# jacobkrantz/VLN-CE

Measured on AMD Instinct MI355X. Metric: policy-steps/sec (fwd+bwd), higher is better.
Workload: dtype f32

## Files before the change

### include/vlnce_hip.h

```cpp
#ifndef VLNCE_HIP_H
#define VLNCE_HIP_H

#include <stddef.h>
#include <stdint.h>

#ifdef __cplusplus
extern "C" {
#endif

typedef void* vlnce_stream_t;

enum { VLNCE_ACT_NONE = 0, VLNCE_ACT_RELU = 1, VLNCE_ACT_SIGMOID = 2, VLNCE_ACT_TANH = 3 };

int vlnce_version(void);
int vlnce_option_count(void);
int vlnce_option_index(const char* name);
const char* vlnce_last_error(void);

int vlnce_set_option(const char* name, int value);
int vlnce_get_option(const char* name, int* value);
int vlnce_option_default(const char* name, int* value);

typedef struct {
  int N, H, W, Cin;
  int Cout, KH, KW;
  int stride, pad;
  int Ho, Wo;
  int ldx, ldy;
} vlnce_conv_desc;

typedef struct {
  const float* in_scale;
  const float* in_shift;
  const float* in_center;
  int in_relu;
  const float* x2;
  const float* in2_scale;
  const float* in2_shift;
  const float* in2_center;
  float* side_out;
  const void* w_split;
  const void* w_frag;
  const int* options;
  int w_format;
} vlnce_prologue;

#define VLNCE_BN_SHARDS 16
typedef struct {
  double* acc;
  void* workspace;
  long workspace_bytes;
} vlnce_bn_sums;

typedef struct {
  const float* scale;
  const float* shift;
  const float* residual;
  int ldr;
  int act;
  int accumulate;
  float* stat_partial;
  const vlnce_bn_sums* bn;
} vlnce_epilogue;

long vlnce_conv2d_bn_workspace_bytes(const vlnce_conv_desc* d);
int vlnce_bn_finalize_sums(double* acc, int M, int C, const float* gamma, const float* beta,
                           float eps, float momentum, float* running_mean, float* running_var,
                           float* scale_out, float* shift_out, float* mean_out, float* rstd_out,
                           vlnce_stream_t stream);

int vlnce_conv2d_tiles_m(const vlnce_conv_desc* d);
int vlnce_conv2d_tile_rows(const vlnce_conv_desc* d);

int vlnce_conv2d_split_weights(const float* w, void* planes, long count, int format,
                               vlnce_stream_t stream);

long vlnce_conv2d_pack_bytes(const vlnce_conv_desc* d);
int vlnce_conv2d_pack_weights(const float* w_ohwi, void* frag, const vlnce_conv_desc* d,
                              int format , vlnce_stream_t stream);

typedef struct vlnce_weight_job {
  const float* w_oihw;
  void* dst;
  int Cout, Cin, T;
  int kind;
  int transposed;
  int format;
} vlnce_weight_job;
long vlnce_weight_job_items(const vlnce_weight_job* job);
int vlnce_conv2d_prepare_weights(const vlnce_weight_job* jobs_dev, const long* first_item_dev,
                                 int njobs, long total_items, vlnce_stream_t stream);

#define VLNCE_CONV_PATH_F32 0
#define VLNCE_CONV_PATH_X3 1
#define VLNCE_CONV_PATH_P3 2
#define VLNCE_CONV_PATH_M3 3
int vlnce_conv2d_last_path(void);

#define VLNCE_CONV_KERNEL(family, format, kernel, a, b, c) \
  ((family) | ((format) << 2) | ((kernel) << 4) | ((a) << 8) | ((b) << 16) | ((c) << 24))
#define VLNCE_CONV_KERNEL_FAMILY(v) ((v) & 3)
#define VLNCE_CONV_KERNEL_FORMAT(v) (((v) >> 2) & 3)
#define VLNCE_CONV_KERNEL_KIND(v) (((v) >> 4) & 15)
#define VLNCE_CONV_KERNEL_A(v) (((v) >> 8) & 255)
#define VLNCE_CONV_KERNEL_B(v) (((v) >> 16) & 255)
#define VLNCE_CONV_KERNEL_C(v) (((v) >> 24) & 127)
#define VLNCE_CONV_KERNEL_P3 0
#define VLNCE_CONV_KERNEL_U3 1
#define VLNCE_CONV_KERNEL_S3 2
#define VLNCE_CONV_P3_DENSE 0
#define VLNCE_CONV_P3_GATHER 1
#define VLNCE_CONV_P3_DUAL 2
#define VLNCE_CONV_KERNEL_F32_BUF 0
#define VLNCE_CONV_KERNEL_F32_SPLITK 1
#define VLNCE_CONV_KERNEL_F32_V4 2
#define VLNCE_CONV_KERNEL_F32_S 3
#define VLNCE_CONV_KERNEL_F32_STEM3 4
#define VLNCE_CONV_KERNEL_F32_STEM1 5
#define VLNCE_CONV_KERNEL_F32_DUAL 6
int vlnce_conv2d_last_kernel(void);

int vlnce_conv2d_fwd(const float* x, const float* w_ohwi, float* y,
                     const vlnce_conv_desc* d, const vlnce_prologue* pro,
                     const vlnce_epilogue* epi, vlnce_stream_t stream);

int vlnce_gemm(const float* A, int lda, int transA, const float* B, int ldb, int transB,
               float* C, int ldc, int M, int N, int K,
               const vlnce_epilogue* epi, vlnce_stream_t stream);

int vlnce_linear_rows_supported(int M, int N, int K);
int vlnce_linear_rows_fwd(const float* x, int ldx, const float* w, int ldw, const float* bias,
                          int act, float* y, int ldy, int M, int N, int K, vlnce_stream_t stream);
int vlnce_linear_rows_bwd(const float* x, int ldx, const float* w, int ldw, const float* dy,
                          int lddy, const float* y, int ldy, int act, float* dx, float* dw,
                          float* db, int M, int N, int K, vlnce_stream_t stream);

int vlnce_colsum(const float* x, int ldx, int M, int N, float* out, int accumulate,
                 vlnce_stream_t stream);

size_t vlnce_bn_finalize_workspace_bytes(int tiles_m, int C);
int vlnce_bn_finalize(const float* stat_partial, int tiles_m, int tile_rows, int M, int C,
                      const float* gamma, const float* beta, float eps, float momentum,
                      float* running_mean, float* running_var,
                      float* scale_out, float* shift_out,
                      float* mean_out, float* rstd_out,
                      void* workspace, size_t workspace_bytes,
                      vlnce_stream_t stream);

int vlnce_scale_shift_act(const float* x, const float* scale, const float* shift,
                          const float* center, int rows_per_sample, const float* residual,
                          float* y, long M, int C, int act, vlnce_stream_t stream);

int vlnce_scale_shift_add_act(const float* x1, const float* scale1, const float* shift1,
                              const float* center1, const float* x2, const float* scale2,
                              const float* shift2, const float* center2, float* y, long M, int C,
                              int act, vlnce_stream_t stream);

int vlnce_gn_chunks(int HW);
int vlnce_gn_partial(const float* x, int Nimg, int HW, int C, float* partial ,
                     vlnce_stream_t stream);
int vlnce_gn_finalize(const float* partial, int Nimg, int HW, int C, int groups,
                      const float* gamma, const float* beta, float eps,
                      float* scale_out, float* shift_out,
                      float* center_out,
                      float* mean_out, float* rstd_out,
                      vlnce_stream_t stream);
int vlnce_gn_finalize_tiles(const float* stat_partial, int tile_rows, int Nimg, int HW, int C,
                            int groups, const float* gamma, const float* beta, float eps,
                            float* scale_out, float* shift_out, float* center_out,
                            float* mean_out, float* rstd_out, vlnce_stream_t stream);
int vlnce_group_norm_small(const float* x, int Nimg, int HW, int C, int groups, const float* gamma,
                           const float* beta, float eps, const float* residual, int act, float* y,
                           vlnce_stream_t stream);

int vlnce_maxpool3x3s2(const float* x, float* y, int N, int H, int W, int C, int Ho, int Wo,
                       const float* in_scale, const float* in_shift, const float* in_center,
                       int in_relu, vlnce_stream_t stream);
int vlnce_avgpool2x2(const float* x, float* y, int N, int H, int W, int C, vlnce_stream_t stream);

int vlnce_space_to_depth2(const float* x, float* y, int N, int H, int W, int C, int pad_lo,
                          int pad_hi, const float* scale, const float* shift,
                          vlnce_stream_t stream);
#define VLNCE_DT_F32 0
#define VLNCE_DT_U8 1
typedef struct {
  const void* x;
  const void* x2;
  const unsigned char* mask2;
  int dtype;
  int N, F, Hs, Ws, C;
  int y0, x0, H, W;
} vlnce_frames;
int vlnce_frames_s2d(const vlnce_frames* frames, float* y, int pad_lo, int pad_hi,
                     const float* scale, const float* shift, vlnce_stream_t stream);
int vlnce_stem7_fwd(const vlnce_frames* frames, const float* in_scale, const float* in_shift,
                    const void* w_frag, int w_format, float* y, int Cout, const vlnce_epilogue* epi,
                    vlnce_stream_t stream);
int vlnce_frames_avgpool2(const vlnce_frames* frames, float* y, vlnce_stream_t stream);
int vlnce_frames_f32(const vlnce_frames* frames, float* y, const float* scale, const float* shift,
                     vlnce_stream_t stream);
int vlnce_frames_gather(const void* const* srcs, int F, int elem_bytes, int N, int Hs, int Ws,
                        int C, int y0, int x0, int H, int W, void* out, vlnce_stream_t stream);

int vlnce_frames_resize_area(const void* x, int dtype, int NF, int Hs, int Ws, int C, int OH, int OW,
                             int y0, int x0, int H, int W, void* out, vlnce_stream_t stream);

int vlnce_adaptive_avgpool(const float* x, float* y, int N, int H, int W, int C, int OH, int OW,
                           int ldy, vlnce_stream_t stream);

int vlnce_conv2d_wgrad(const float* x, const float* dy, float* dw_ohwi, const vlnce_conv_desc* d,
                       const float* dy_pow2, int P, int accumulate, vlnce_stream_t stream);
#define VLNCE_WGRAD_PATH_F32 0
#define VLNCE_WGRAD_PATH_X6_BF16 1
#define VLNCE_WGRAD_PATH_X6_F16 2
int vlnce_conv2d_wgrad_last_path(void);
#define VLNCE_WGRAD_KERNEL(path, tm, split) ((path) | ((tm) << 4) | ((split) ? 1 << 12 : 0))
#define VLNCE_WGRAD_KERNEL_PATH(v) ((v) & 15)
#define VLNCE_WGRAD_KERNEL_TM(v) (((v) >> 4) & 255)
#define VLNCE_WGRAD_KERNEL_SPLIT(v) (((v) >> 12) & 1)
int vlnce_conv2d_wgrad_last_kernel(void);
size_t vlnce_bn_bwd_workspace_floats(long M, int C);
int vlnce_bn_bwd(const float* dy, const float* y, const float* x, const float* mean,
                 const float* rstd, const float* gamma, long M, int C, int relu,
                 int use_batch_stats, float* dx, float* dres, float* dgamma, float* dbeta,
                 float* workspace, float* pow2, int P, vlnce_stream_t stream);
size_t vlnce_gn_bwd_workspace_floats(int Nimg, int HW, int C, int groups);
int vlnce_gn_bwd(const float* dy, const float* y, const float* x, const float* mean,
                 const float* rstd, const float* gamma, int Nimg, int HW, int C, int groups,
                 int relu, float* dx, float* dres, float* dgamma, float* dbeta, float* workspace,
                 float* pow2, int P, vlnce_stream_t stream);
int vlnce_maxpool3x3s2_argmax(const float* x, float* y, uint8_t* argmax, int N, int H, int W,
                              int C, int Ho, int Wo, vlnce_stream_t stream);
int vlnce_maxpool3x3s2_bwd(const float* dy, const uint8_t* argmax, float* dx, int N, int H, int W,
                           int C, int Ho, int Wo, vlnce_stream_t stream);
int vlnce_adaptive_avgpool_bwd(const float* dy, float* dx, int N, int H, int W, int C, int OH,
                               int OW, vlnce_stream_t stream);

int vlnce_action_head_fwd(const float* x, int ldx, const float* w, const float* b, int M, int K,
                          int A, float* logits_out, int* nan_count, vlnce_stream_t stream);
int vlnce_action_head_bwd(const float* x, int ldx, const float* w, const float* logits,
                          const float* dlogits, int M, int K, int A, float* dx, float* dw,
                          float* db, vlnce_stream_t stream);

int vlnce_attn_fwd(const float* q, const float* K, int ldk, const float* V, int ldv,
                   const uint8_t* mask, int mask_mode, float scale,
                   float* out, float* attn_out, int B, int P, int Dk, int Dv,
                   vlnce_stream_t stream);
int vlnce_attn_bwd(const float* dout, const float* q, const float* K, int ldk,
                   const float* V, int ldv, const uint8_t* mask, int mask_mode, float scale,
                   const float* attn, float* dq, float* dK, int lddk, float* dV, int lddv,
                   int B, int P, int Dk, int Dv, vlnce_stream_t stream);

int vlnce_attn_fwd_shared(const float* q, const float* K, int ldk, const float* V, int ldv,
                          const uint8_t* mask, int mask_mode, float scale, const int64_t* kv_index,
                          float* out, float* attn_out, int B, int P, int Dk, int Dv,
                          vlnce_stream_t stream);
int vlnce_attn_bwd_shared(const float* dout, const float* q, const float* K, int ldk,
                          const float* V, int ldv, const uint8_t* mask, int mask_mode, float scale,
                          const int64_t* kv_index, const float* attn, float* dq, float* dK,
                          int lddk, float* dV, int lddv, int B, int P, int Dk, int Dv,
                          vlnce_stream_t stream);
int vlnce_segment_sum(const float* x, const int64_t* index, int B, int U, long row_elems,
// ... 129 lines not shown
```

### vln-ce_amd/_lib.py

```python
import collections
import ctypes as C
import os
import threading

import torch

_HERE = os.path.dirname(os.path.abspath(__file__))
LIB_PATH = os.environ.get("VLNCE_HIP_LIB") or os.path.join(_HERE, "libvlnce_hip.so")

_P = C.c_void_p
_I = C.c_int
_F = C.c_float
_L = C.c_long


def _buffer_format(explicit, *bufs):
    tags = {getattr(b, "_vlnce_fmt", None) for b in bufs if b is not None} - {None}
    if explicit:
        tags.add(int(explicit))
    if len(tags) > 1:
        raise RuntimeError(f"weight buffers / w_format disagree on the plane format: {sorted(tags)}")
    return tags.pop() if tags else 1


ConvKernel = collections.namedtuple("ConvKernel", "family kernel fmt a b c")
ConvKernel.__doc__ = """family: "f32" | "x3" | "p3" | "m3" (= conv2d_last_path()); kernel: the kernel within it
("conv_p3" | "conv_u3" | "conv_s3", "conv_m3", "conv_x3", "buf" | "splitk" | "v4" | "s" | "stem3" |
"stem1" | "dual" of igemm_kernel); fmt: plane format 1 / 2 (0: fp32); a, b, c per kernel:
  conv_p3: tile 1..6, mode "dense" | "gather" | "dual", 0      conv_u3: rows, kind 0..2, waves
  conv_s3: Cin, 0, 0      conv_m3: NT, KSPLIT, RB      conv_x3: tile 1..4, dual 0 / 1, 0
  splitk: the split factor, 0, 0"""
WgradKernel = collections.namedtuple("WgradKernel", "path tm split")

_FAMILIES = ("f32", "x3", "p3", "m3")
_KERNELS = {"f32": ("buf", "splitk", "v4", "s", "stem3", "stem1", "dual"), "x3": ("conv_x3",),
            "p3": ("conv_p3", "conv_u3", "conv_s3"), "m3": ("conv_m3",)}
_P3_MODES = ("dense", "gather", "dual")


def decode_conv_kernel(v):
    if v < 0:
        return None
    family = _FAMILIES[v & 3]
    kernel = _KERNELS[family][(v >> 4) & 15]
    a, b, c = (v >> 8) & 255, (v >> 16) & 255, (v >> 24) & 127
    if kernel == "conv_p3":
        b = _P3_MODES[b]
    return ConvKernel(family, kernel, (v >> 2) & 3, a, b, c)


def decode_wgrad_kernel(v):
    return None if v < 0 else WgradKernel(v & 15, (v >> 4) & 255, bool((v >> 12) & 1))


class ConvDesc(C.Structure):
    _fields_ = [(n, _I) for n in
                ("N", "H", "W", "Cin", "Cout", "KH", "KW", "stride", "pad", "Ho", "Wo", "ldx", "ldy")]


class WeightJob(C.Structure):
    _fields_ = [("w_oihw", _P), ("dst", _P), ("Cout", _I), ("Cin", _I), ("T", _I), ("kind", _I),
                ("transposed", _I), ("format", _I)]


class WeightPrepPlan:
    __slots__ = ("table", "first_item", "njobs", "total", "keep")


class Prologue(C.Structure):
    _fields_ = [("in_scale", _P), ("in_shift", _P), ("in_center", _P), ("in_relu", _I),
                ("x2", _P), ("in2_scale", _P), ("in2_shift", _P), ("in2_center", _P),
                ("side_out", _P), ("w_split", _P), ("w_frag", _P), ("options", _P), ("w_format", _I)]


class Frames(C.Structure):
    _fields_ = [("x", _P), ("x2", _P), ("mask2", _P), ("dtype", _I), ("N", _I), ("F", _I),
                ("Hs", _I), ("Ws", _I), ("C", _I), ("y0", _I), ("x0", _I), ("H", _I), ("W", _I)]


class BnSums(C.Structure):
    _fields_ = [("acc", _P), ("workspace", _P), ("workspace_bytes", _L)]


class TrajSensor(C.Structure):
    _fields_ = [("src", _P), ("dst", _P), ("row_stride", _L), ("c_stride", _L), ("p_stride", _L),
                ("C", _I), ("P", _I), ("src_dtype", _I), ("dst_dtype", _I)]


class Epilogue(C.Structure):
    _fields_ = [("scale", _P), ("shift", _P), ("residual", _P), ("ldr", _I), ("act", _I),
                ("accumulate", _I), ("stat_partial", _P), ("bn", C.POINTER(BnSums))]


_SIGNATURES = {
    "vlnce_version": (_I, []),
    "vlnce_last_error": (C.c_char_p, []),
    "vlnce_set_option": (_I, [C.c_char_p, _I]),
    "vlnce_get_option": (_I, [C.c_char_p, C.POINTER(_I)]),
    "vlnce_option_default": (_I, [C.c_char_p, C.POINTER(_I)]),
    "vlnce_conv2d_split_weights": (_I, [_P, _P, C.c_long, _I, _P]),
    "vlnce_conv2d_last_path": (_I, []),
    "vlnce_conv2d_wgrad_last_path": (_I, []),
    "vlnce_conv2d_last_kernel": (_I, []),
    "vlnce_conv2d_wgrad_last_kernel": (_I, []),
    "vlnce_embedding_bwd": (_I, [_P, _P, _P, _L, _I, _L, _L, _P]),
    "vlnce_conv2d_pack_bytes": (C.c_long, [C.POINTER(ConvDesc)]),
    "vlnce_conv2d_pack_weights": (_I, [_P, _P, C.POINTER(ConvDesc), _I, _P]),
    "vlnce_weight_job_items": (C.c_long, [C.POINTER(WeightJob)]),
    "vlnce_conv2d_prepare_weights": (_I, [_P, _P, _I, C.c_long, _P]),
    "vlnce_conv2d_tiles_m": (_I, [C.POINTER(ConvDesc)]),
    "vlnce_conv2d_tile_rows": (_I, [C.POINTER(ConvDesc)]),
    "vlnce_conv2d_bn_workspace_bytes": (C.c_long, [C.POINTER(ConvDesc)]),
    "vlnce_bn_finalize_sums": (_I, [_P, _I, _I, _P, _P, _F, _F, _P, _P, _P, _P, _P, _P, _P]),
    "vlnce_conv2d_fwd": (_I, [_P, _P, _P, C.POINTER(ConvDesc), C.POINTER(Prologue),
                              C.POINTER(Epilogue), _P]),
    "vlnce_gemm": (_I, [_P, _I, _I, _P, _I, _I, _P, _I, _I, _I, _I, C.POINTER(Epilogue), _P]),
    "vlnce_colsum": (_I, [_P, _I, _I, _I, _P, _I, _P]),
    "vlnce_bn_finalize_workspace_bytes": (C.c_size_t, [_I, _I]),
    "vlnce_bn_finalize": (_I, [_P, _I, _I, _I, _I, _P, _P, _F, _F, _P, _P, _P, _P, _P, _P, _P,
                               C.c_size_t, _P]),
    "vlnce_scale_shift_act": (_I, [_P, _P, _P, _P, _I, _P, _P, _L, _I, _I, _P]),
    "vlnce_gn_chunks": (_I, [_I]),
    "vlnce_gn_partial": (_I, [_P, _I, _I, _I, _P, _P]),
    "vlnce_gn_finalize": (_I, [_P, _I, _I, _I, _I, _P, _P, _F, _P, _P, _P, _P, _P, _P]),
    "vlnce_gn_finalize_tiles": (_I, [_P, _I, _I, _I, _I, _I, _P, _P, _F, _P, _P, _P, _P, _P, _P]),
    "vlnce_maxpool3x3s2": (_I, [_P, _P, _I, _I, _I, _I, _I, _I, _P, _P, _P, _I, _P]),
    "vlnce_scale_shift_add_act": (_I, [_P, _P, _P, _P, _P, _P, _P, _P, _P, _L, _I, _I, _P]),
    "vlnce_avgpool2x2": (_I, [_P, _P, _I, _I, _I, _I, _P]),
    "vlnce_ragged_pad_rows": (_I, [_P, _I, _P, _I, _I, _L, _F, _P, _P]),
    "vlnce_ragged_pad_rows_i64": (_I, [_P, _P, _I, _I, _L, _L, _P, _P]),
    "vlnce_dagger_targets": (_I, [_P, _P, _I, _I, _F, _P, _P, _P, _P]),
    "vlnce_traj_append": (_I, [C.POINTER(TrajSensor), _I, C.POINTER(_I), C.POINTER(_I), _I, _L, _P]),
    "vlnce_dagger_mix_actions": (_I, [_P, _P, _I, _P, _F, _I, _P, _P, _P]),
    "vlnce_ppo_loss": (_I, [_P, _P, _P, _P, _P, _P, _P, _P, _P, _P, _I, _F, _F, _F, _F, _F, _F, _F, _I,
                            _P, _P, _P]),
    "vlnce_ppo_returns": (_I, [_P, _P, _P, _P, _P, _I, _I, _F, _F, _I, _P]),
    "vlnce_space_to_depth2": (_I, [_P, _P, _I, _I, _I, _I, _I, _I, _P, _P, _P]),
    "vlnce_frames_s2d": (_I, [C.POINTER(Frames), _P, _I, _I, _P, _P, _P]),
    "vlnce_frames_avgpool2": (_I, [C.POINTER(Frames), _P, _P]),
    "vlnce_stem7_fwd": (_I, [C.POINTER(Frames), _P, _P, _P, _I, _P, _I, C.POINTER(Epilogue), _P]),
    "vlnce_frames_f32": (_I, [C.POINTER(Frames), _P, _P, _P, _P]),
    "vlnce_frames_gather": (_I, [_P, _I, _I, _I, _I, _I, _I, _I, _I, _I, _I, _P, _P]),
    "vlnce_frames_resize_area": (_I, [_P] + [_I] * 11 + [_P, _P]),
    "vlnce_adaptive_avgpool": (_I, [_P, _P, _I, _I, _I, _I, _I, _I, _I, _P]),
    "vlnce_attn_fwd": (_I, [_P, _P, _I, _P, _I, _P, _I, _F, _P, _P, _I, _I, _I, _I, _P]),
    "vlnce_attn_bwd": (_I, [_P, _P, _P, _I, _P, _I, _P, _I, _F, _P, _P, _P, _I, _P, _I,
                            _I, _I, _I, _I, _P]),
    "vlnce_rowzero_mask": (_I, [_P, _I, _L, _I, _P, _P]),
    "vlnce_attn_fwd_shared": (_I, [_P, _P, _I, _P, _I, _P, _I, _F, _P, _P, _P, _I, _I, _I, _I, _P]),
    "vlnce_attn_bwd_shared": (_I, [_P, _P, _P, _I, _P, _I, _P, _I, _F, _P, _P, _P, _P, _I, _P, _I,
                                   _I, _I, _I, _I, _P]),
    "vlnce_segment_sum": (_I, [_P, _P, _I, _I, _L, _P, _P]),
    "vlnce_action_head_fwd": (_I, [_P, _I, _P, _P, _I, _I, _I, _P, _P, _P]),
    "vlnce_action_head_bwd": (_I, [_P, _I, _P, _P, _P, _I, _I, _I, _P, _P, _P, _P]),
    "vlnce_gru_gates_fwd": (_I, [_P, _P, _P, _P, _P, _P, _P, _I, _I, _P]),
    "vlnce_gru_gates_bwd": (_I, [_P, _P, _P, _P, _P, _P, _P, _P, _I, _I, _P]),
    "vlnce_lstm_gates_fwd": (_I, [_P, _P, _P, _P, _P, _P, _P, _I, _I, _P]),
    "vlnce_lstm_gates_bwd": (_I, [_P, _P, _P, _P, _P, _P, _P, _P, _I, _I, _P]),
    "vlnce_mean_rows": (_I, [_P, _P, _I, _I, _I, _P]),
    "vlnce_mask_rows": (_I, [_P, _P, _P, _I, _I, _P]),
    "vlnce_conv2d_wgrad": (_I, [_P, _P, _P, C.POINTER(ConvDesc), _P, _I, _I, _P]),
    "vlnce_bn_bwd": (_I, [_P, _P, _P, _P, _P, _P, _L, _I, _I, _I, _P, _P, _P, _P, _P, _P, _I, _P]),
    "vlnce_bn_bwd_workspace_floats": (C.c_size_t, [_L, _I]),
    "vlnce_gn_bwd_workspace_floats": (C.c_size_t, [_I, _I, _I, _I]),
    "vlnce_gn_bwd": (_I, [_P, _P, _P, _P, _P, _P, _I, _I, _I, _I, _I, _P, _P, _P, _P, _P, _P, _I, _P]),
    "vlnce_maxpool3x3s2_argmax": (_I, [_P, _P, _P, _I, _I, _I, _I, _I, _I, _P]),
    "vlnce_maxpool3x3s2_bwd": (_I, [_P, _P, _P, _I, _I, _I, _I, _I, _I, _P]),
    "vlnce_adaptive_avgpool_bwd": (_I, [_P, _P, _I, _I, _I, _I, _I, _I, _P]),
    "vlnce_rnn_seq_supported": (_I, [_I, _I]),
    "vlnce_rnn_seq_fwd": (_I, [_I, _I, _P, _P, _P, _P, _P, _P, _P, _P, _I, _I, _I, _P]),
    "vlnce_rnn_seq_bwd": (_I, [_I, _I, _P, _P, _P, _P, _P, _P, _P, _P, _P, _I, _I, _I, _P]),
    "vlnce_option_count": (_I, []),
    "vlnce_option_index": (_I, [C.c_char_p]),
    "vlnce_linear_rows_supported": (_I, [_I, _I, _I]),
    "vlnce_linear_rows_fwd": (_I, [_P, _I, _P, _I, _P, _I, _P, _I, _I, _I, _I, _P]),
    "vlnce_linear_rows_bwd": (_I, [_P, _I, _P, _I, _P, _I, _P, _I, _I, _P, _P, _P, _I, _I, _I, _P]),
    "vlnce_rnn_seq_fwd2": (_I, [_I, _I, _P, _P, _P, _P, _P, _P, _L, _L, _P, _P, _P, _I, _I, _I, _P]),
    "vlnce_rnn_seq_bwd2": (_I, [_I, _I, _P, _P, _P, _P, _P, _P, _L, _L, _P, _P, _P, _P, _I, _I, _I, _P]),
    "vlnce_rnn_seq_wgrad": (_I, [_I, _I, _I, _P, _P, _P, _P, _I, _I, _P, _P, _P, _P, _P, _P, _I, _I, _I, _P]),
    "vlnce_group_norm_small": (_I, [_P, _I, _I, _I, _I, _P, _P, _F, _P, _I, _P, _P]),
    "vlnce_gru_rollout_supported": (_I, [_I, _I]),
    "vlnce_gru_rollout_workspace_bytes": (C.c_long, [_I, _I]),
    "vlnce_gru_rollout_fwd": (_I, [_P, _P, _P, _P, _P, _P, _P, _P, _P, _P, _I, _I, _I, _P]),
    "vlnce_gru_rollout_bwd": (_I, [_P, _P, _P, _P, _P, _P, _P, _P, _P, _P, _P, _I, _I, _I, _P]),
    "vlnce_lstm_rollout_supported": (_I, [_I, _I]),
    "vlnce_lstm_rollout_workspace_bytes": (C.c_long, [_I, _I]),
    "vlnce_lstm_rollout_fwd": (_I, [_P, _P, _P, _P, _P, _P, _P, _P, _P, _P, _P, _I, _I, _I, _P]),
    "vlnce_lstm_rollout_bwd": (_I, [_P, _P, _P, _P, _P, _P, _P, _P, _P, _P, _P, _P, _P, _I, _I, _I, _P]),
    "vlnce_rnn_step_supported": (_I, [_I, _I, _I]),
    "vlnce_rnn_step_fwd": (_I, [_I, _P, _P, _P, _P, _P, _P, _P, _P, _P, _P, _I, _I, _P]),
    "vlnce_rnn_step_bwd": (_I, [_I, _P, _P, _P, _P, _P, _P, _P, _P, _P, _P, _P, _P, _P, _I, _I, _P]),
    "vlnce_select_rows": (_I, [_P, _P, _P, _P, _I, _I, _P]),
    "vlnce_act_bwd": (_I, [_P, _P, _P, _L, _I, _P]),
}


def collapse_rows(t):
    while True:
        groups = []
        for n, st in zip(t.shape[1:], t.stride()[1:]):
            if n == 1:
                continue
            if groups and groups[-1][1] == st * n:
                groups[-1] = (groups[-1][0] * n, int(st))
            else:
                groups.append((int(n), int(st)))
        if len(groups) <= 2:
            break
        t = t.contiguous()
    row_stride = int(t.stride(0)) if t.size(0) > 1 else 0
    if not groups:
        return t, row_stride, 1, 0, 1, 0
    if len(groups) == 1:
        return t, row_stride, groups[0][0], groups[0][1], 1, 0
    return t, row_stride, groups[0][0], groups[0][1], groups[1][0], groups[1][1]


def exported_symbols():
    return sorted(_SIGNATURES)


def load_cdll(path=LIB_PATH):
    if not os.path.exists(path):
        raise RuntimeError(
            f"{path} not found: build it with `python __graft_entry__.py` (hipcc, gfx950). "
            "The VLN-CE policy path has no CPU fallback."
        )
    dll = C.CDLL(path)
    for name, (res, args) in _SIGNATURES.items():
        fn = getattr(dll, name)
        fn.restype = res
        fn.argtypes = args
    return dll


class _CallState(threading.local):
    dev = None
    restore = None


_CALL = _CallState()


def _ptr(t):
    if t is None:
        return None
    if not t.is_cuda:
        raise RuntimeError("libvlnce_hip: tensor is not on a GPU (no CPU fallback)")
    idx = t.device.index
    if _CALL.dev is None:
        _CALL.dev = idx
    elif _CALL.dev != idx:
        first, _CALL.dev = _CALL.dev, None
        raise RuntimeError(f"libvlnce_hip: tensors of one call live on cuda:{first} and "
                           f"cuda:{idx}")
    return t.data_ptr()


def _stream():
    dev, _CALL.dev = _CALL.dev, None
    if dev is None:
        return torch.cuda.current_stream().cuda_stream
    cur = torch.cuda.current_device()
    if dev != cur:
        _CALL.restore = cur
        torch.cuda.set_device(dev)
    return torch.cuda.current_stream(dev).cuda_stream


def _leave_device():
    if _CALL.restore is not None:
        cur, _CALL.restore = _CALL.restore, None
        torch.cuda.set_device(cur)


class HipLib:

    name = "hip"

    ABI = 147

    def __init__(self, path=LIB_PATH):
        self.dll = load_cdll(path)
        have = int(self.dll.vlnce_version())
        if have != self.ABI:
            raise RuntimeError(f"{path} has ABI {have}, this package binds ABI {self.ABI}: "
                               "rebuild it (python __graft_entry__.py)")

        self._conv_math = None
        self._tls = threading.local()
        self._options_from_env()

    OPTION_NAMES = ("conv_math", "p3", "p3_tile", "s3", "u3", "u3_waves", "x3_tile", "igemm_tile",
                    "igemm_nobuf", "igemm_no_splitk", "wgrad_tile", "rollout_one_xcd", "m3")

    def _options_from_env(self):
        for name in self.OPTION_NAMES:
            v = os.environ.get("VLNCE_" + name.upper())
            if v is None:
                continue
            if name == "conv_math":
                v = {"f32": 0, "0": 0, "bf16": 1, "1": 1, "f16": 2, "2": 2}.get(v.strip().lower(), v)
            elif name in ("igemm_nobuf", "igemm_no_splitk"):
                v = 0 if v in ("", "0") else 1
            try:
                v = int(v)
            except ValueError:
                import warnings
                warnings.warn(f"VLNCE_{name.upper()}={v!r} is not an integer: ignored "
                              f"(the option keeps its default)")
                continue
            self.set_option(name, v)

    def set_option(self, name, value):
        self._check(self.dll.vlnce_set_option(name.encode(), int(value)), "vlnce_set_option")
        if name == "conv_math":
            self._conv_math = int(value)

    def plane_format(self, options=None):
        v = None
        if options:
            v = options.get("conv_math")
        if v is None:
            sc = getattr(self._tls, "scoped", None)
            if sc:
                v = sc.get("conv_math")
        if v is None or v < 0:
            v = self._conv_math
            if v is None:
                v = self._conv_math = self.get_option("conv_math")
        return 2 if v == 2 else 1

    def get_option(self, name):
        v = _I(0)
        self._check(self.dll.vlnce_get_option(name.encode(), C.byref(v)), "vlnce_get_option")
        return v.value

    def option_default(self, name):
        v = _I(0)
        self._check(self.dll.vlnce_option_default(name.encode(), C.byref(v)), "vlnce_option_default")
        return v.value

    PER_LAUNCH = ("conv_math", "p3", "p3_tile", "s3", "u3", "u3_waves", "x3_tile", "m3")

    def _launch_options(self, overrides):
        if not overrides:
            return None
        arr = (C.c_int * int(self.dll.vlnce_option_count()))(*([-1] * int(self.dll.vlnce_option_count())))
        for name, v in overrides.items():
            i = int(self.dll.vlnce_option_index(name.encode()))
            if i < 0:
                raise RuntimeError(f"unknown dispatch option {name!r}")
            arr[i] = int(v)
        return arr

    def options(self, **kw):
        lib = self
        unknown = [k for k in kw if k not in self.OPTION_NAMES]
        if unknown:
            raise RuntimeError(f"unknown dispatch option(s) {unknown}")

        class _Scope:
            def __enter__(self_inner):
                self_inner.prev = getattr(lib._tls, "scoped", None)
                scoped = dict(self_inner.prev or {})
                scoped.update({k: v for k, v in kw.items() if k in lib.PER_LAUNCH})
                lib._tls.scoped = scoped or None
                self_inner.old = {k: lib.get_option(k) for k in kw if k not in lib.PER_LAUNCH}
                for k in self_inner.old:
                    lib.set_option(k, kw[k])
                return lib

            def __exit__(self_inner, *exc):
                lib._tls.scoped = self_inner.prev
                for k, v in self_inner.old.items():
                    lib.set_option(k, v)
                return False

        return _Scope()

    def _check(self, rc, what):
        _leave_device()
        if rc != 0:
            raise RuntimeError(f"{what} failed (rc={rc}): {self.dll.vlnce_last_error().decode()}")

    @staticmethod
    def _desc(g):
        return ConvDesc(*[int(g[k]) for k, _ in ConvDesc._fields_])

    def conv2d_tiles(self, g):
        d = self._desc(g)
        return self.dll.vlnce_conv2d_tiles_m(C.byref(d)), self.dll.vlnce_conv2d_tile_rows(C.byref(d))

    def conv2d_fwd(self, x, w, y, g, in_scale=None, in_shift=None, in_relu=0, scale=None,
                   shift=None, residual=None, ldr=0, act=0, accumulate=0, stat_partial=None,
                   in_center=None, x2=None, in2_scale=None, in2_shift=None, in2_center=None,
                   side_out=None, w_split=None, w_frag=None, bn=None, options=None, w_format=None):
        d = self._desc(g)
        w_format = _buffer_format(w_format, w_split, w_frag)
        opts = self._launch_options(options if options is not None
                                    else getattr(self._tls, "scoped", None))
        pro = Prologue(_ptr(in_scale), _ptr(in_shift), _ptr(in_center), int(in_relu), _ptr(x2),
                       _ptr(in2_scale), _ptr(in2_shift), _ptr(in2_center), _ptr(side_out),
                       _ptr(w_split), _ptr(w_frag),
                       C.cast(opts, C.c_void_p) if opts is not None else None, int(w_format))
        bnp = None
        if bn is not None:
            acc, ws = bn
            bnp = C.pointer(BnSums(_ptr(acc), _ptr(ws), ws.numel() * ws.element_size()))
        epi = Epilogue(_ptr(scale), _ptr(shift), _ptr(residual), int(ldr), int(act),
                       int(accumulate), _ptr(stat_partial), bnp)
        self._check(self.dll.vlnce_conv2d_fwd(_ptr(x), _ptr(w), _ptr(y), C.byref(d), C.byref(pro),
                                              C.byref(epi), _stream()), "vlnce_conv2d_fwd")

    def bn_finalize_sums(self, acc, M, gamma, beta, eps, momentum, running_mean, running_var,
                         scale_out, mean_out, shift_out=None, rstd_out=None):
        Cc = scale_out.numel()
        self._check(self.dll.vlnce_bn_finalize_sums(
            _ptr(acc), int(M), Cc, _ptr(gamma), _ptr(beta), float(eps), float(momentum),
            _ptr(running_mean), _ptr(running_var), _ptr(scale_out), _ptr(shift_out),
            _ptr(mean_out), _ptr(rstd_out), _stream()), "vlnce_bn_finalize_sums")

    def conv2d_bn_workspace_bytes(self, g):
        d = self._desc(g)
        return int(self.dll.vlnce_conv2d_bn_workspace_bytes(C.byref(d)))

    def conv2d_split_weights(self, w, planes, fmt=1):
        self._check(self.dll.vlnce_conv2d_split_weights(_ptr(w), _ptr(planes), w.numel(), int(fmt),
                                                        _stream()), "vlnce_conv2d_split_weights")

    def conv2d_last_path(self):
        return int(self.dll.vlnce_conv2d_last_path())

    def conv2d_wgrad_last_path(self):
        return int(self.dll.vlnce_conv2d_wgrad_last_path())

    def conv2d_last_kernel(self):
        return decode_conv_kernel(int(self.dll.vlnce_conv2d_last_kernel()))

    def conv2d_wgrad_last_kernel(self):
        return decode_wgrad_kernel(int(self.dll.vlnce_conv2d_wgrad_last_kernel()))

    def conv2d_pack_bytes(self, g):
        d = self._desc(g)
        return int(self.dll.vlnce_conv2d_pack_bytes(C.byref(d)))

    def conv2d_pack_weights(self, w, frag, g, fmt=1):
        d = self._desc(g)
        self._check(self.dll.vlnce_conv2d_pack_weights(_ptr(w), _ptr(frag), C.byref(d), int(fmt),
                                                       _stream()), "vlnce_conv2d_pack_weights")

    WP_F32, WP_PLANES, WP_FRAGMENTS = 0, 1, 2

    def weight_prep_plan(self, jobs):
        arr = (WeightJob * len(jobs))()
        first = [0]
        for j, (w, dst, kind, transposed, fmt) in zip(arr, jobs):
            assert w.is_cuda and w.is_contiguous() and w.dtype == torch.float32 and w.dim() == 4
            j.w_oihw, j.dst = w.data_ptr(), dst.data_ptr()
            j.Cout, j.Cin, j.T = w.size(0), w.size(1), w.size(2) * w.size(3)
            j.kind, j.transposed, j.format = int(kind), int(bool(transposed)), int(fmt or 0)
            items = int(self.dll.vlnce_weight_job_items(C.byref(j)))
            if items <= 0:
                raise ValueError(f"weight_prep_plan: job not eligible: {tuple(w.shape)} kind={kind} "
                                 f"transposed={transposed} format={fmt}")
            first.append(first[-1] + items)
        plan = WeightPrepPlan()
        dev = jobs[0][1].device
        plan.table = torch.frombuffer(bytearray(bytes(arr)), dtype=torch.uint8).to(dev)
        plan.first_item = torch.tensor(first, dtype=torch.int64).to(dev)
        plan.njobs, plan.total = len(jobs), first[-1]
        plan.keep = [(w, dst) for w, dst, *_ in jobs]
        return plan

    def conv2d_prepare_weights(self, plan):
        self._check(self.dll.vlnce_conv2d_prepare_weights(_ptr(plan.table), _ptr(plan.first_item),
                                                          plan.njobs, plan.total, _stream()),
                    "vlnce_conv2d_prepare_weights")

    def gemm(self, A, lda, transA, B, ldb, transB, Cm, ldc, M, N, K, scale=None, shift=None,
             residual=None, ldr=0, act=0, accumulate=0):
        epi = Epilogue(_ptr(scale), _ptr(shift), _ptr(residual), int(ldr), int(act),
                       int(accumulate), None)
        self._check(self.dll.vlnce_gemm(_ptr(A), lda, transA, _ptr(B), ldb, transB, _ptr(Cm), ldc,
                                        M, N, K, C.byref(epi), _stream()), "vlnce_gemm")

    def colsum(self, x, ldx, M, N, out, accumulate=0):
        self._check(self.dll.vlnce_colsum(_ptr(x), ldx, M, N, _ptr(out), accumulate, _stream()),
                    "vlnce_colsum")

    def bn_finalize_workspace_bytes(self, tiles_m, Cc):
        return int(self.dll.vlnce_bn_finalize_workspace_bytes(tiles_m, Cc))

    def bn_finalize(self, partial, tiles_m, tile_rows, M, Cc, gamma, beta, eps, momentum,
                    running_mean, running_var, scale_out, shift_out, mean_out=None, rstd_out=None,
                    workspace=None):
        wb = workspace.numel() * workspace.element_size() if workspace is not None else 0
        self._check(self.dll.vlnce_bn_finalize(
            _ptr(partial), tiles_m, tile_rows, M, Cc, _ptr(gamma), _ptr(beta), eps, momentum,
            _ptr(running_mean), _ptr(running_var), _ptr(scale_out), _ptr(shift_out),
            _ptr(mean_out), _ptr(rstd_out), _ptr(workspace), wb, _stream()), "vlnce_bn_finalize")

    def scale_shift_act(self, x, scale, shift, rows_per_sample, residual, y, M, Cc, act,
                        center=None):
        self._check(self.dll.vlnce_scale_shift_act(
            _ptr(x), _ptr(scale), _ptr(shift), _ptr(center), rows_per_sample, _ptr(residual),
            _ptr(y), M, Cc, act, _stream()), "vlnce_scale_shift_act")

    def gn_chunks(self, HW):
        return self.dll.vlnce_gn_chunks(HW)

    def gn_partial(self, x, Nimg, HW, Cc, partial):
        self._check(self.dll.vlnce_gn_partial(_ptr(x), Nimg, HW, Cc, _ptr(partial), _stream()),
                    "vlnce_gn_partial")

    def gn_finalize(self, partial, Nimg, HW, Cc, groups, gamma, beta, eps, scale_out, shift_out,
                    mean_out=None, rstd_out=None, center_out=None):
        self._check(self.dll.vlnce_gn_finalize(
            _ptr(partial), Nimg, HW, Cc, groups, _ptr(gamma), _ptr(beta), eps, _ptr(scale_out),
            _ptr(shift_out), _ptr(center_out), _ptr(mean_out), _ptr(rstd_out), _stream()),
            "vlnce_gn_finalize")

    def gn_finalize_tiles(self, partial, tile_rows, Nimg, HW, Cc, groups, gamma, beta, eps,
                          scale_out, shift_out, mean_out=None, rstd_out=None, center_out=None):
        self._check(self.dll.vlnce_gn_finalize_tiles(
            _ptr(partial), tile_rows, Nimg, HW, Cc, groups, _ptr(gamma), _ptr(beta), eps,
            _ptr(scale_out), _ptr(shift_out), _ptr(center_out), _ptr(mean_out), _ptr(rstd_out),
            _stream()), "vlnce_gn_finalize_tiles")

    def maxpool3x3s2(self, x, y, N, H, W, Cc, Ho, Wo, in_scale=None, in_shift=None, in_relu=0,
                     in_center=None):
        self._check(self.dll.vlnce_maxpool3x3s2(_ptr(x), _ptr(y), N, H, W, Cc, Ho, Wo,
                                                _ptr(in_scale), _ptr(in_shift), _ptr(in_center),
                                                int(in_relu), _stream()), "vlnce_maxpool3x3s2")

    def scale_shift_add_act(self, x1, s1, t1, x2, s2, t2, y, M, Cc, act, c1=None, c2=None):
        self._check(self.dll.vlnce_scale_shift_add_act(
            _ptr(x1), _ptr(s1), _ptr(t1), _ptr(c1), _ptr(x2), _ptr(s2), _ptr(t2), _ptr(c2),
            _ptr(y), M, Cc, act, _stream()), "vlnce_scale_shift_add_act")

    _SRC = {torch.float32: 0, torch.float16: 1, torch.int64: 2}

    def ragged_pad_rows(self, src, offsets, B, Tmax, D, fill, dst):
        assert offsets.dtype == torch.int32 and dst.dtype == torch.float32
        self._check(self.dll.vlnce_ragged_pad_rows(
            _ptr(src), self._SRC[src.dtype], _ptr(offsets), B, Tmax, D, float(fill),
            _ptr(dst), _stream()), "vlnce_ragged_pad_rows")

    def ragged_pad_rows_i64(self, src, offsets, B, Tmax, D, fill, dst):
        assert src.dtype == torch.int64 and dst.dtype == torch.int64
        self._check(self.dll.vlnce_ragged_pad_rows_i64(
            _ptr(src), _ptr(offsets), B, Tmax, D, int(fill), _ptr(dst), _stream()),
            "vlnce_ragged_pad_rows_i64")

    def dagger_targets(self, oracle, offsets, B, Tmax, coef, corrected, weights, masks):
        self._check(self.dll.vlnce_dagger_targets(
            _ptr(oracle), _ptr(offsets), B, Tmax, float(coef), _ptr(corrected),
            _ptr(weights), _ptr(masks), _stream()), "vlnce_dagger_targets")

    _TRAJ = {torch.float32: 0, torch.float16: 1, torch.int64: 2, torch.uint8: 3}
    TRAJ_MAX_SENSORS, TRAJ_MAX_ROWS = 8, 128

    def traj_append(self, sources, arenas, slots, steps):
        n = len(slots)
# ... 386 lines not shown
```

### vln-ce_amd/csrc/api.cpp

```cpp
#include <stdarg.h>
#include <stdio.h>
#include <string.h>

#include <atomic>

#include "common_opts.h"

static thread_local char g_err[512] = "";

void vlnce_set_error(const char* fmt, ...) {
  va_list ap;
  va_start(ap, fmt);
  vsnprintf(g_err, sizeof(g_err), fmt, ap);
  va_end(ap);
}

extern "C" const char* vlnce_last_error(void) { return g_err; }
extern "C" int vlnce_version(void) { return 147; }

namespace {
struct OptDef {
  const char* name;
  int def;
};
const OptDef kOpts[VLNCE_OPT_COUNT] = {
    {"conv_math", 2},   {"p3", 2},          {"p3_tile", 0},         {"s3", 1},
    {"u3", 1},          {"u3_waves", 8},    {"x3_tile", 0},         {"igemm_tile", 0},
    {"igemm_nobuf", 0}, {"igemm_no_splitk", 0}, {"wgrad_tile", 64}, {"rollout_one_xcd", 0},
    {"m3", 1},
};
std::atomic<int> g_opt[VLNCE_OPT_COUNT] = {
    {2}, {2}, {0}, {1}, {1}, {8}, {0}, {0}, {0}, {0}, {64}, {0}, {1},
};
int opt_index(const char* name) {
  if (name)
    for (int i = 0; i < VLNCE_OPT_COUNT; ++i)
      if (strcmp(name, kOpts[i].name) == 0) return i;
  return -1;
}
}

namespace {
thread_local const int* t_call_opts = nullptr;
}
VlnceOptScope::VlnceOptScope(const int* per_call) : prev(t_call_opts) { t_call_opts = per_call; }
VlnceOptScope::~VlnceOptScope() { t_call_opts = prev; }

int vlnce_opt(int id) {
  if (t_call_opts && t_call_opts[id] >= 0) return t_call_opts[id];
  return g_opt[id].load(std::memory_order_relaxed);
}

extern "C" int vlnce_option_count(void) { return VLNCE_OPT_COUNT; }

extern "C" int vlnce_option_index(const char* name) { return opt_index(name); }

extern "C" int vlnce_set_option(const char* name, int value) {
  const int i = opt_index(name);
  if (i < 0) {
    vlnce_set_error("vlnce_set_option: unknown option '%s'", name ? name : "(null)");
    return 1;
  }
  g_opt[i].store(value, std::memory_order_relaxed);
  return 0;
}

extern "C" int vlnce_get_option(const char* name, int* value) {
  const int i = opt_index(name);
  if (i < 0 || !value) {
    vlnce_set_error("vlnce_get_option: unknown option '%s'", name ? name : "(null)");
    return 1;
  }
  *value = g_opt[i].load(std::memory_order_relaxed);
  return 0;
}

extern "C" int vlnce_option_default(const char* name, int* value) {
  const int i = opt_index(name);
  if (i < 0 || !value) {
    vlnce_set_error("vlnce_option_default: unknown option '%s'", name ? name : "(null)");
    return 1;
  }
  *value = kOpts[i].def;
  return 0;
}
```

### vln-ce_amd/csrc/common_opts.h

```cpp
#pragma once
#include "../../include/vlnce_hip.h"

void vlnce_set_error(const char* fmt, ...);

enum {
  VLNCE_OPT_CONV_MATH,
  VLNCE_OPT_P3,
  VLNCE_OPT_P3_TILE,
  VLNCE_OPT_S3,
  VLNCE_OPT_U3,
  VLNCE_OPT_U3_WAVES,
  VLNCE_OPT_X3_TILE,
  VLNCE_OPT_IGEMM_TILE,
  VLNCE_OPT_IGEMM_NOBUF,
  VLNCE_OPT_IGEMM_NO_SPLITK,
  VLNCE_OPT_WGRAD_TILE,
  VLNCE_OPT_ROLLOUT_ONE_XCD,
  VLNCE_OPT_M3,
  VLNCE_OPT_COUNT
};
int vlnce_opt(int id);

struct VlnceOptScope {
  explicit VlnceOptScope(const int* per_call);
  ~VlnceOptScope();
  const int* prev;
};
```

### vln-ce_amd/csrc/conv_s3.hip

```cpp
#include "igemm_shared.h"

using namespace vlnce_detail;

namespace vlnce_detail {
namespace {

template <int NCC, int MATH>
__global__ __launch_bounds__(512) void conv_s3_kernel(IgemmParams p) {
#if defined(__HIP_DEVICE_COMPILE__)
  typedef Planes<MATH> PL;
  constexpr int P3_ROW = PL::ROW, NA = PL::NA, NP = PL::NP;
  constexpr int BM = 64, MT = 2, KS = NCC * 2;
  constexpr int CBUF = BM * P3_ROW;
  constexpr int PBUF = NCC * CBUF;
  constexpr int SPS = 32 / KS;
  extern __shared__ __attribute__((aligned(16))) char xsm[];

  const int tid = threadIdx.x;
  const int lane = tid & 63;
  const int wave = __builtin_amdgcn_readfirstlane(tid >> 6);
  const int half = lane >> 5;
  const int l31 = lane & 31;
  const int trow = tid >> 3;
  const int lk4 = (tid & 7) * 4;

  const int n0 = ((int)blockIdx.x % p.tiles_n) * 256;
  const int wg = (int)blockIdx.x / p.tiles_n, nwg = (int)gridDim.x / p.tiles_n;
  const int my_tiles = (p.tiles_m - wg + nwg - 1) / nwg;

  const __amdgpu_buffer_rsrc_t rsrc_a = __builtin_amdgcn_make_buffer_rsrc(
      const_cast<char*>(reinterpret_cast<const char*>(p.A)), 0, (int)p.a_bytes, 0x00020000);
  const __amdgpu_buffer_rsrc_t rsrc_b = __builtin_amdgcn_make_buffer_rsrc(
      const_cast<char*>(reinterpret_cast<const char*>(p.Bfrag)), 0, (int)((long)p.N * p.K * 6),
      0x00020000);
  const __amdgpu_buffer_rsrc_t rsrc_c = __builtin_amdgcn_make_buffer_rsrc(
      reinterpret_cast<char*>(p.C), 0, (int)p.c_bytes, 0x00020000);
  const float relu_floor = p.in_relu ? 0.f : -__builtin_huge_valf();
  const bool relu_out = p.act == VLNCE_ACT_RELU;

  bf16x8 bres[KS][3];
  {
    const int vb = (n0 / 32 + wave) * KS * 3072 + lane * 16;
#pragma unroll
    for (int ks = 0; ks < KS; ++ks)
#pragma unroll
      for (int q = 0; q < 3; ++q)
        bres[ks][q] = __builtin_bit_cast(
            bf16x8, __builtin_amdgcn_raw_buffer_load_b128(rsrc_b, vb + q * 1024, ks * 3072, 0));
  }
  float* const vlds = reinterpret_cast<float*>(xsm + 2 * PBUF);
  if (tid < 8) {
    const f32x4 zero4 = {0.f, 0.f, 0.f, 0.f}, one4 = {1.f, 1.f, 1.f, 1.f};
#pragma unroll
    for (int c = 0; c < NCC; ++c) {
      f32x4 s_ = one4, t_ = zero4, c_ = zero4;
      if (p.in_scale != nullptr) {
        s_ = ldg4(p.in_scale + c * 32 + lk4);
        t_ = ldg4(p.in_shift + c * 32 + lk4);
        if (p.in_center) c_ = ldg4(p.in_center + c * 32 + lk4);
      }
      *reinterpret_cast<f32x4*>(vlds + c * 32 + lk4) = s_;
      *reinterpret_cast<f32x4*>(vlds + NCC * 32 + c * 32 + lk4) = t_;
      *reinterpret_cast<f32x4*>(vlds + 2 * NCC * 32 + c * 32 + lk4) = c_;
    }
  }
  __syncthreads();
  const int col = n0 + wave * 32 + l31;
  const float e_sc = (p.scale ? p.scale[col] : 1.f) * PL::POST;
  const float e_sh = p.shift ? p.shift[col] : 0.f;

  constexpr int RING = NCC > 2 ? 1 : 2;
  f32x4 raw[RING][NCC];
  auto load_raw = [&](f32x4 (&r)[NCC], int round) {
    const int m = (wg + round * nwg) * BM + trow;
    const int vo = (round < my_tiles && m < p.M) ? (m * p.lda + lk4) * 4 : BUF_OOB;
#pragma unroll
    for (int c = 0; c < NCC; ++c)
      r[c] = __builtin_bit_cast(f32x4, __builtin_amdgcn_raw_buffer_load_b128(rsrc_a, vo, c * 128, 0));
  };
#pragma unroll
  for (int k = 0; k < RING; ++k) load_raw(raw[k], k);
  f32x16 acc[2][MT];
#pragma unroll
  for (int b = 0; b < 2; ++b)
#pragma unroll
    for (int i = 0; i < MT; ++i)
#pragma unroll
      for (int r = 0; r < 16; ++r) acc[b][i][r] = 0.f;
  const int a_off = l31 * P3_ROW + half * 16;

  WaveBn<1> wbn;
  wave_bn_reset(wbn);
  auto stats = [&](const f32x16 (&a)[MT], int m0) {
    if (p.bn.acc != nullptr) {
      wave_bn_tile<MT, 1>(reinterpret_cast<const f32x16(&)[MT][1]>(a), wbn, p.bn.acc, n0 + wave * 32,
                          p.N, p.M - m0, half, l31, PL::POST);
    } else if (p.stat_partial != nullptr) {
#pragma unroll
      for (int i = 0; i < MT; ++i)
        wave_stats_block<1>(reinterpret_cast<const f32x16(&)[1]>(a[i]), p.stat_partial,
                            m0 / 32 + i, p.M - (m0 + i * 32), n0 + wave * 32, p.N, half, l31, PL::POST);
    }
  };
  auto stores = [&](f32x16 (&a)[MT], int m0, int first, int count) {
    const int rows_left = p.M - (m0 + 4 * half);
    const int e_voff = (int)((((long)(m0 + 4 * half)) * p.ldc + col) * 4);
#pragma unroll
    for (int k = first; k < first + count; ++k) {
      const int i = k >> 4, r2 = k & 15;
      const int rw = i * 32 + (r2 & 3) + 8 * (r2 >> 2);
      const float lin = a[i][r2] * e_sc + e_sh;
      const float v = relu_out ? (lin > 0.f ? lin : 0.f) : lin;
      __builtin_amdgcn_raw_buffer_store_b32(__builtin_bit_cast(unsigned, v), rsrc_c,
                                            rw < rows_left ? e_voff : BUF_OOB, rw * p.ldc * 4, 0);
      a[i][r2] = 0.f;
    }
  };

  auto tile = [&](int round, f32x4 (&r)[NCC], f32x16 (&cur)[MT], f32x16 (&prv)[MT]) {
    const int m0 = (wg + round * nwg) * BM;
    const int m0_prev = (wg + (round - 1) * nwg) * BM;
    const bool has_prev = round > 0;
    char* const pb = xsm + (round & 1) * PBUF;
    const bool row_ok = m0 + trow < p.M;
#pragma unroll
    for (int c = 0; c < NCC; ++c) {
      f32x4 v = r[c];
      const f32x4 s_ = *reinterpret_cast<const f32x4*>(vlds + c * 32 + lk4);
      const f32x4 t_ = *reinterpret_cast<const f32x4*>(vlds + NCC * 32 + c * 32 + lk4);
      const f32x4 c_ = *reinterpret_cast<const f32x4*>(vlds + 2 * NCC * 32 + c * 32 + lk4);
#pragma unroll
      for (int e = 0; e < 4; ++e) {
        v[e] = fmaxf(fmaf(v[e] - c_[e], s_[e], t_[e]), relu_floor);
        v[e] = row_ok ? v[e] : 0.f;
      }
      p3_split_store<MATH>(v, pb + c * CBUF + trow * P3_ROW + lk4 * 2);
    }
    load_raw(r, round + RING);
    asm volatile("s_waitcnt lgkmcnt(0)" ::: "memory");
    __builtin_amdgcn_s_barrier();
    if (has_prev) stats(prv, m0_prev);
#pragma unroll
    for (int c = 0; c < NCC; ++c)
#pragma unroll
      for (int s2 = 0; s2 < 2; ++s2) {
        bf16x8 f[MT][NA];
#pragma unroll
        for (int i = 0; i < MT; ++i)
#pragma unroll
          for (int q = 0; q < NA; ++q)
            f[i][q] = *reinterpret_cast<const bf16x8*>(pb + c * CBUF + a_off + i * 32 * P3_ROW +
                                                       q * 64 + s2 * 32);
#pragma unroll
        for (int q = 0; q < NP; ++q)
#pragma unroll
          for (int i = 0; i < MT; ++i)
            cur[i] = plane_mfma<MATH>(f[i][PL::PA[q]], bres[c * 2 + s2][PL::PB[q]], cur[i]);
        stores(prv, has_prev ? m0_prev : p.M, (c * 2 + s2) * SPS, SPS);
        if constexpr (MATH == MATH_F16X3) {
#pragma unroll
          for (int g = 0; g < 2; ++g) {
            if constexpr (SPS == 8) {
              __builtin_amdgcn_sched_group_barrier(0x008, 1, 0);
              __builtin_amdgcn_sched_group_barrier(0x040, 1, 0);
              __builtin_amdgcn_sched_group_barrier(0x008, 1, 0);
              __builtin_amdgcn_sched_group_barrier(0x040, 2, 0);
              __builtin_amdgcn_sched_group_barrier(0x008, 1, 0);
              __builtin_amdgcn_sched_group_barrier(0x040, 1, 0);
            } else {
              __builtin_amdgcn_sched_group_barrier(0x008, 3, 0);
              __builtin_amdgcn_sched_group_barrier(0x040, 2, 0);
            }
          }
        } else {
#pragma unroll
          for (int g = 0; g < 4; ++g) {
            if constexpr (SPS == 8) {
              __builtin_amdgcn_sched_group_barrier(0x008, 2, 0);
              __builtin_amdgcn_sched_group_barrier(0x040, 1, 0);
              __builtin_amdgcn_sched_group_barrier(0x008, 1, 0);
              __builtin_amdgcn_sched_group_barrier(0x040, 1, 0);
            } else {
              __builtin_amdgcn_sched_group_barrier(0x008, 3, 0);
              __builtin_amdgcn_sched_group_barrier(0x040, 1, 0);
            }
          }
        }
      }
  };
  if (my_tiles <= 0) return;
  tile(0, raw[0], acc[0], acc[1]);
  if (1 < my_tiles) tile(1, raw[RING - 1], acc[1], acc[0]);
  for (int round = 2; round < my_tiles; round += 2) {
    tile(round, raw[0], acc[0], acc[1]);
    if (round + 1 < my_tiles) tile(round + 1, raw[RING - 1], acc[1], acc[0]);
  }
  {
    const int m0 = (wg + (my_tiles - 1) * nwg) * BM;
    if ((my_tiles - 1) & 1) {
      stats(acc[1], m0);
      if (p.bn.acc != nullptr) wave_bn_flush(wbn, p.bn.acc, p.N, half, l31);
      stores(acc[1], m0, 0, 32);
    } else {
      stats(acc[0], m0);
      if (p.bn.acc != nullptr) wave_bn_flush(wbn, p.bn.acc, p.N, half, l31);
      stores(acc[0], m0, 0, 32);
    }
  }
#endif
}

template <int NCC, int MATH>
int launch_s3(const IgemmParams& p, hipStream_t stream) {
  constexpr int smem_bytes = 2 * NCC * 64 * Planes<MATH>::ROW + 3 * NCC * 32 * 4;
  auto kern = conv_s3_kernel<NCC, MATH>;
  static bool attr_set = false;
  if (!attr_set) {
    hipError_t e = hipFuncSetAttribute(reinterpret_cast<const void*>(kern),
                                       hipFuncAttributeMaxDynamicSharedMemorySize, smem_bytes);
    if (e != hipSuccess) {
      vlnce_set_error("conv_s3: hipFuncSetAttribute failed: %s", hipGetErrorString(e));
      return 2;
    }
    attr_set = true;
  }
  IgemmParams q = p;
  q.tiles_m = ceil_div(p.M, 64);
  q.tiles_n = p.N / 256;
  q.splitk = 1;
  const int cus = x3_cus();
  long grid = (long)q.tiles_m * q.tiles_n;
  if (grid > cus) grid = cus - cus % q.tiles_n;
  hipLaunchKernelGGL(kern, dim3((unsigned)grid), dim3(512), smem_bytes, stream, q);
  VLNCE_CHECK_LAUNCH("conv_s3");
  return 0;
}

}

int s3_launch(const IgemmParams& p, hipStream_t stream) {
  note_conv_kernel(VLNCE_CONV_KERNEL(VLNCE_CONV_PATH_P3, p.math, VLNCE_CONV_KERNEL_S3, p.Cin == 64 ? 64 : 128, 0, 0));
  if (p.math == MATH_F16X3)
    return p.Cin == 64 ? launch_s3<2, MATH_F16X3>(p, stream) : launch_s3<4, MATH_F16X3>(p, stream);
  return p.Cin == 64 ? launch_s3<2, MATH_BF16X6>(p, stream) : launch_s3<4, MATH_BF16X6>(p, stream);
}

}
```

### vln-ce_amd/csrc/igemm.hip

```cpp
#include "igemm_shared.h"

using namespace vlnce_detail;

namespace {


template <int BM, int BN, int WM, int WN, int AMODE, int BMODE, int CIN_C = 0, int KW_C = 0,
          int DUAL = 0>
__global__ __launch_bounds__(256, 2) void igemm_kernel(IgemmParams p) {
  static_assert(!DUAL || AMODE == A_BUF, "dual-input prologue: buffer-loader path only");
  constexpr int WTM = BM / WM;
  constexpr int WTN = BN / WN;
  constexpr int MT = WTM / 32;
  constexpr int NT = WTN / 32;
  constexpr bool A_KMAJOR = AMODE == A_TRANS;
  constexpr bool B_KMAJOR = BMODE == B_KN || BMODE == B_IM2COL;
  constexpr int LDT_A = BM + 8, LDT_B = BN + 8;
  constexpr int A_TILE = BM * LDP;
  constexpr int B_TILE = BN * LDP;
  static_assert(BK * LDT_A <= A_TILE && BK * LDT_B <= B_TILE, "k-major LDS image");
  constexpr int STAGE = A_TILE + B_TILE;
  static_assert(WM * WN == 4, "4 waves");
  static_assert(MT >= 1 && NT >= 1, "tile");

// ... 944 lines not shown
      const long long c = clock64() - d_c0, w = wall_clock64() - d_w0;
      printf("x3 tiles %d KT %d: first K-tile after %lld cycles; total %lld cycles = %lld ticks of 100 MHz "
             "(%.2f GHz); waiting for producers %lld\n", my_tiles, KT, d_c1 - d_c0, c, w,
             (double)c / (double)w * 0.1, d_wait);
    }
#endif
  }
#endif
}

__global__ __launch_bounds__(256) void rows_stats_kernel(const float* __restrict__ y, int ldc, int M,
                                                         int N, int rows,
                                                         float* __restrict__ partial) {
  const int col = blockIdx.y * 64 + (threadIdx.x & 63);
  const int blk = blockIdx.x * 4 + (threadIdx.x >> 6);
  const int r0 = blk * rows;
  if (col >= N || r0 >= M) return;
  const int n = min(rows, M - r0);
  const float* q = y + (long)r0 * ldc + col;
  float v[32];
  float s = 0.f;
#pragma unroll
  for (int i = 0; i < 32; ++i) {
    v[i] = i < n ? q[(long)i * ldc] : 0.f;
    s += v[i];
  }
  const float mean = s / (float)n;
  float m2 = 0.f;
#pragma unroll
  for (int i = 0; i < 32; ++i) {
    const float d = v[i] - mean;
    if (i < n) m2 += d * d;
  }
  float* dst = partial + ((long)blk * N + col) * 2;
  dst[0] = s;
  dst[1] = m2;
}

__global__ __launch_bounds__(256) void bias_act_kernel(float* __restrict__ c, int ldc, int M, int N,
                                                       const float* __restrict__ shift, int act) {
  const long total = (long)M * N;
  for (long i = (long)blockIdx.x * blockDim.x + threadIdx.x; i < total;
       i += (long)gridDim.x * blockDim.x) {
    const long row = i / N;
    const int col = (int)(i - row * N);
    float* q = c + row * ldc + col;
    *q = apply_act(*q + (shift ? shift[col] : 0.f), act);
  }
}

template <int BM, int BN, int WM, int WN, int AMODE, int BMODE, int CIN_C = 0, int KW_C = 0,
          int DUAL = 0>
int launch(const IgemmParams& p, hipStream_t stream) {
  constexpr int smem_bytes = 2 * (BM + BN) * LDP * (int)sizeof(float);
  static_assert(BM * (BN + 4) * (int)sizeof(float) <= smem_bytes, "epilogue tile must fit");
  auto kern = igemm_kernel<BM, BN, WM, WN, AMODE, BMODE, CIN_C, KW_C, DUAL>;
  static bool attr_set = false;
  if (!attr_set) {
    hipError_t e = hipFuncSetAttribute(reinterpret_cast<const void*>(kern),
                                       hipFuncAttributeMaxDynamicSharedMemorySize, smem_bytes);
    if (e != hipSuccess) {
      vlnce_set_error("igemm: hipFuncSetAttribute failed: %s", hipGetErrorString(e));
      return 2;
    }
    attr_set = true;
  }
  IgemmParams q = p;
  q.tiles_m = ceil_div(p.M, BM);
  q.tiles_n = ceil_div(p.N, BN);
  if (q.splitk < 1) q.splitk = 1;
  const long nwg = (long)q.tiles_m * q.tiles_n;
  if (nwg <= 0 || nwg > 0x7fffffffL) {
    vlnce_set_error("igemm: bad grid %ld", nwg);
    return 1;
  }
  hipLaunchKernelGGL(kern, dim3((unsigned)nwg, (unsigned)q.splitk), dim3(256), smem_bytes, stream,
                     q);
  VLNCE_CHECK_LAUNCH("igemm");
  return 0;
}

struct TileChoice {
  int bm, bn;
};
TileChoice choose_tile(long M, int N) {
  const int force = vlnce_opt(VLNCE_OPT_IGEMM_TILE);
  if (force == 1) return {128, 128};
  if (force == 2) return {128, 64};
  if (force == 3) return {64, 64};
  const long want = 512;
  auto tiles = [&](int bm, int bn) { return (long)ceil_div(M, bm) * ceil_div(N, bn); };
  if (N > 64 && M > 64 && tiles(128, 128) >= want) return {128, 128};
  if (N > 64 && M > 64 && tiles(128, 64) >= want) return {128, 64};
  return {64, 64};
}

template <int AMODE, int BMODE>
int dispatch_tiles(const IgemmParams& p, hipStream_t s) {
  const TileChoice t = choose_tile(p.M, p.N);
  if (t.bm == 128 && t.bn == 128) return launch<128, 128, 2, 2, AMODE, BMODE>(p, s);
  if (t.bm == 128 && t.bn == 64) return launch<128, 64, 2, 2, AMODE, BMODE>(p, s);
  return launch<64, 64, 2, 2, AMODE, BMODE>(p, s);
}
int dispatch_dual(const IgemmParams& p, hipStream_t s) {
  const TileChoice t = choose_tile(p.M, p.N);
  if (t.bm == 128 && t.bn == 128) return launch<128, 128, 2, 2, A_BUF, B_BUF, 0, 0, 1>(p, s);
  if (t.bm == 128 && t.bn == 64) return launch<128, 64, 2, 2, A_BUF, B_BUF, 0, 0, 1>(p, s);
  return launch<64, 64, 2, 2, A_BUF, B_BUF, 0, 0, 1>(p, s);
}
template <int AMODE, int BMODE>
int dispatch_small(const IgemmParams& p, hipStream_t s) {
  return launch<64, 64, 2, 2, AMODE, BMODE>(p, s);
}
bool buf_ok(const IgemmParams& p) {
  const bool off = vlnce_opt(VLNCE_OPT_IGEMM_NOBUF) != 0;
  const long bias = ((long)p.pad * p.W + p.pad) * p.lda * 4;
  return !off && (p.Cin % 32 == 0) && (p.K % 32 == 0) && (p.lda % 4 == 0) && (p.ldb % 4 == 0) &&
         p.KH * p.KW <= 32 && p.a_bytes + bias < 0x7fffffffL && p.b_bytes < 0x7fffffffL;
}
template <int CIN_C>
int dispatch_stem(const IgemmParams& p, hipStream_t s) {
  const TileChoice t = choose_tile(p.M, p.N);
  if (t.bm == 128) return launch<128, 64, 2, 2, A_IM2COL_S, B_NK_S, CIN_C, 7>(p, s);
  return launch<64, 64, 2, 2, A_IM2COL_S, B_NK_S, CIN_C, 7>(p, s);
}

int choose_splitk(const IgemmParams& p, bool long_reduction_form = false) {
  const bool off = vlnce_opt(VLNCE_OPT_IGEMM_NO_SPLITK) != 0;
  if (off) return 1;
  const long tiles = (long)ceil_div(p.M, 64) * ceil_div(p.N, 64);
  const int KT = ceil_div(p.K, BK);
  if (long_reduction_form && KT >= 32 && tiles >= 128 && tiles < 1024) {
    long s = (1024 + tiles - 1) / tiles;
    if (s > KT / 4) s = KT / 4;
    return s < 2 ? 1 : (int)s;
  }
  if (tiles >= 128 || KT < 8) return 1;
  long s = (256 + tiles - 1) / tiles;
  if (s > KT / 2) s = KT / 2;
  if (s > 64) s = 64;
  return s < 2 ? 1 : (int)s;
}

void fill_epilogue(IgemmParams& p, const vlnce_epilogue* e) {
  p.scale = e ? e->scale : nullptr;
  p.shift = e ? e->shift : nullptr;
  p.residual = e ? e->residual : nullptr;
  p.ldr = e ? e->ldr : 0;
  p.act = e ? e->act : 0;
  p.accumulate = e ? e->accumulate : 0;
  p.stat_partial = e ? e->stat_partial : nullptr;
  p.bn = vlnce_bn_sums{};
  if (e && e->bn) p.bn = *e->bn;
}

bool aligned16(const void* q) { return (reinterpret_cast<uintptr_t>(q) & 15) == 0; }

template <int BM, int BN, int WM, int WN, int DUAL, int MATH>
int launch_x3(const IgemmParams& p, hipStream_t stream) {
  constexpr int smem_bytes = 2 * (Planes<MATH>::NA * BM + 3 * BN) * X3_PITCH + 16;
  constexpr int threads = (WM * WN + X3_PRODUCERS) * 64;
  auto kern = conv_x3_kernel<BM, BN, WM, WN, DUAL, MATH>;
  static bool attr_set = false;
  if (!attr_set) {
    hipError_t e = hipFuncSetAttribute(reinterpret_cast<const void*>(kern),
                                       hipFuncAttributeMaxDynamicSharedMemorySize, smem_bytes);
    if (e != hipSuccess) {
      vlnce_set_error("conv_x3: hipFuncSetAttribute failed: %s", hipGetErrorString(e));
      return 2;
    }
    attr_set = true;
  }
  IgemmParams q = p;
  q.tiles_m = ceil_div(p.M, BM);
  q.tiles_n = ceil_div(p.N, BN);
  q.splitk = 1;
  const long nwg = (long)q.tiles_m * q.tiles_n;
  if (nwg <= 0 || nwg > 0x7fffffffL) {
    vlnce_set_error("conv_x3: bad grid %ld", nwg);
    return 1;
  }
  const int cus = x3_cus();
  const unsigned grid = nwg <= cus ? (unsigned)nwg : (unsigned)cus;
  hipLaunchKernelGGL(kern, dim3(grid), dim3(threads), smem_bytes, stream, q);
  VLNCE_CHECK_LAUNCH("conv_x3");
  return 0;
}

struct X3Plan {
  int bm, bn;
};
bool x3_plan(const IgemmParams& p, X3Plan* out) {
  if (!conv_math() || !p.Bsplit || !buf_ok(p) || p.splitk > 1) return false;
  if (p.accumulate || p.c_bytes >= 0x7fffffffL) return false;
  if (p.residual && (p.ldr != p.ldc || p.stat_partial || p.bn.acc)) return false;
  const int force = vlnce_opt(VLNCE_OPT_X3_TILE);
  const X3Plan cand[4] = {{128, 128}, {64, 128}, {128, 64}, {64, 64}};
  if (force >= 1 && force <= 4) {
    *out = cand[force - 1];
    return true;
  }
  const int cus = x3_cus();
  double best = 0.0;
  for (const X3Plan& c : cand) {
    if (c.bn == 128 && p.N <= 64) continue;
    const long tiles = (long)ceil_div(p.M, c.bm) * ceil_div(p.N, c.bn);
    const long rounds = (tiles + cus - 1) / cus;
    const double eff = (double)tiles / (double)(rounds * cus);
    if (eff >= 0.8) {
      *out = c;
      return true;
    }
    if (eff > best) {
      best = eff;
      *out = c;
    }
  }
  return best >= 0.4;
}
template <int DUAL, int MATH>
int dispatch_x3_(const IgemmParams& p, const X3Plan& t, hipStream_t s) {
  const int tile = t.bm == 128 ? (t.bn == 128 ? 1 : 3) : (t.bn == 128 ? 2 : 4);
  note_conv_kernel(VLNCE_CONV_KERNEL(VLNCE_CONV_PATH_X3, MATH, 0, tile, DUAL, 0));
  if (t.bm == 128 && t.bn == 128) return launch_x3<128, 128, 2, 4, DUAL, MATH>(p, s);
  if (t.bm == 64 && t.bn == 128) return launch_x3<64, 128, 2, 4, DUAL, MATH>(p, s);
  if (t.bm == 128 && t.bn == 64) return launch_x3<128, 64, 4, 2, DUAL, MATH>(p, s);
  return launch_x3<64, 64, 2, 2, DUAL, MATH>(p, s);
}
template <int DUAL>
int dispatch_x3(const IgemmParams& p, const X3Plan& t, hipStream_t s) {
  return p.math == MATH_F16X3 ? dispatch_x3_<DUAL, MATH_F16X3>(p, t, s)
                              : dispatch_x3_<DUAL, MATH_BF16X6>(p, t, s);
}

}

static int stat_rows_for(const vlnce_conv_desc* d) {
  const int hw = d->Ho * d->Wo;
  return hw % 32 == 0 ? 32 : 16;
}

extern "C" int vlnce_conv2d_tile_rows(const vlnce_conv_desc* d) { return stat_rows_for(d); }

extern "C" int vlnce_conv2d_tiles_m(const vlnce_conv_desc* d) {
  const long M = (long)d->N * d->Ho * d->Wo;
  return ceil_div(M, stat_rows_for(d));
}

template <int MATH>
__global__ __launch_bounds__(256) void split_weights_kernel(const float* __restrict__ w,
                                                            unsigned short* __restrict__ planes,
                                                            long count) {
  for (long i = blockIdx.x * 256L + threadIdx.x; i < count; i += gridDim.x * 256L) {
    unsigned short o[3];
    split_weight<MATH>(w[i], o);
#pragma unroll
    for (int q = 0; q < 3; ++q) planes[q * count + i] = o[q];
  }
}

extern "C" int vlnce_conv2d_split_weights(const float* w, void* planes, long count, int format,
                                          vlnce_stream_t stream) {
  VLNCE_CHECK_ARG(w && planes && count > 0, "conv2d_split_weights: bad argument");
  VLNCE_CHECK_ARG(format == MATH_BF16X6 || format == MATH_F16X3,
                  "conv2d_split_weights: format must be 1 (three bf16 planes) or 2 (fp16 planes)");
  const long blocks = (count + 255) / 256;
  hipLaunchKernelGGL(format == MATH_F16X3 ? split_weights_kernel<MATH_F16X3>
                                          : split_weights_kernel<MATH_BF16X6>,
                     dim3((unsigned)(blocks > 4096 ? 4096 : blocks)),
                     dim3(256), 0, reinterpret_cast<hipStream_t>(stream), w,
                     reinterpret_cast<unsigned short*>(planes), count);
  VLNCE_CHECK_LAUNCH("conv2d_split_weights");
  return 0;
}

__global__ __launch_bounds__(256) void bn_sums_finalize_kernel(
    double* __restrict__ acc, int M, int N, const float* __restrict__ gamma,
    const float* __restrict__ beta, float eps, float momentum, float* running_mean,
    float* running_var, float* scale_out, float* shift_out, float* mean_out, float* rstd_out) {
  const int c = blockIdx.x * 256 + threadIdx.x;
  if (c >= N) return;
  double S = 0.0, Q = 0.0;
#pragma unroll
  for (int k = 0; k < VLNCE_BN_SHARDS; ++k) {
    double* q = acc + ((long)k * N + c) * 2;
    S += q[0];
    Q += q[1];
    q[0] = 0.0;
    q[1] = 0.0;
  }
  const double mean = S / (double)M;
  double m2 = Q - S * mean;
  if (m2 < 0.0) m2 = 0.0;
  const double var = m2 / (double)M;
  const float rstd = (float)(1.0 / sqrt(var + (double)eps));
  const float g = gamma ? gamma[c] : 1.f;
  const float sc = g * rstd;
  scale_out[c] = sc;
  if (shift_out) shift_out[c] = (beta ? beta[c] : 0.f) - (float)mean * sc;
  if (mean_out) mean_out[c] = (float)mean;
  if (rstd_out) rstd_out[c] = rstd;
  if (running_mean) {
    const double unbiased = M > 1 ? m2 / (double)(M - 1) : var;
    running_mean[c] = (1.f - momentum) * running_mean[c] + momentum * (float)mean;
    running_var[c] = (1.f - momentum) * running_var[c] + momentum * (float)unbiased;
  }
}

__global__ __launch_bounds__(256) void bn_partials_to_sums_kernel(const float* __restrict__ partial,
                                                                  int tiles_m, int tile_rows, int M,
                                                                  int N, double* __restrict__ acc) {
  const int c = blockIdx.y * 64 + (threadIdx.x & 63);
  const int t0 = (blockIdx.x * 4 + (threadIdx.x >> 6)) * 32;
  if (c >= N || t0 >= tiles_m) return;
  double S = 0.0, Q = 0.0;
  for (int t = t0; t < min(t0 + 32, tiles_m); ++t) {
    const float2 v = *reinterpret_cast<const float2*>(partial + ((long)t * N + c) * 2);
    const int nt = min(tile_rows, M - t * tile_rows);
    S += (double)v.x;
    Q += (double)v.y + (double)v.x * (double)v.x / (double)nt;
  }
  double* q = acc + ((long)(blockIdx.x % VLNCE_BN_SHARDS) * N + c) * 2;
  unsafeAtomicAdd(q, S);
  unsafeAtomicAdd(q + 1, Q);
}

extern "C" long vlnce_conv2d_bn_workspace_bytes(const vlnce_conv_desc* d) {
  if (!d || d->Cout <= 0) return 0;
  return (((long)vlnce_conv2d_tiles_m(d) * d->Cout * 2 * 4) + 255) / 256 * 256;
}

extern "C" int vlnce_bn_finalize_sums(double* acc, int M, int C, const float* gamma, const float* beta,
                                      float eps, float momentum, float* running_mean,
                                      float* running_var, float* scale_out, float* shift_out,
                                      float* mean_out, float* rstd_out, vlnce_stream_t stream) {
  VLNCE_CHECK_ARG(acc && scale_out && M > 0 && C > 0, "bn_finalize_sums: bad argument");
  VLNCE_CHECK_ARG((running_mean == nullptr) == (running_var == nullptr),
                  "bn_finalize_sums: running stats must come together");
  hipLaunchKernelGGL(bn_sums_finalize_kernel, dim3(ceil_div(C, 256)), dim3(256), 0,
                     reinterpret_cast<hipStream_t>(stream), acc, M, C, gamma, beta, eps, momentum,
                     running_mean, running_var, scale_out, shift_out, mean_out, rstd_out);
  VLNCE_CHECK_LAUNCH("bn_finalize_sums");
  return 0;
}

static thread_local int g_last_path = -1;
extern "C" int vlnce_conv2d_last_path(void) { return g_last_path; }
static thread_local int g_last_kernel = -1;
extern "C" int vlnce_conv2d_last_kernel(void) { return g_last_kernel; }
void vlnce_detail::note_conv_kernel(int value) { g_last_kernel = value; }
static void note_f32_kernel(int kernel, int a = 0) {
  g_last_kernel = VLNCE_CONV_KERNEL(VLNCE_CONV_PATH_F32, 0, kernel, a, 0, 0);
}

extern "C" int vlnce_conv2d_fwd(const float* x, const float* w, float* y, const vlnce_conv_desc* d,
                                const vlnce_prologue* pro, const vlnce_epilogue* epi,
                                vlnce_stream_t stream) {
  VLNCE_CHECK_ARG(x && w && y && d, "conv2d_fwd: null argument");
  VLNCE_CHECK_ARG(d->N > 0 && d->H > 0 && d->W > 0 && d->Cin > 0 && d->Cout > 0,
                  "conv2d_fwd: bad shape");
  const VlnceOptScope opt_scope(pro ? pro->options : nullptr);
  VLNCE_CHECK_ARG(d->H < 32768 && d->W < 32768, "conv2d_fwd: H/W must be < 32768");
  const int ho = (d->H + 2 * d->pad - d->KH) / d->stride + 1;
  const int wo = (d->W + 2 * d->pad - d->KW) / d->stride + 1;
  VLNCE_CHECK_ARG(ho == d->Ho && wo == d->Wo, "conv2d_fwd: Ho/Wo mismatch (%d,%d) vs (%d,%d)", ho,
                  wo, d->Ho, d->Wo);
  const long M = (long)d->N * d->Ho * d->Wo;
  VLNCE_CHECK_ARG(M < 0x7fffffffL && (long)d->N * d->H * d->W < 0x7fffffffL,
                  "conv2d_fwd: too many pixels for 32-bit row indices");
  IgemmParams p{};
  p.A = x;
  p.B = w;
  p.C = y;
  p.M = (int)M;
  p.N = d->Cout;
  p.K = d->KH * d->KW * d->Cin;
  p.H = d->H;
  p.W = d->W;
  p.Cin = d->Cin;
  p.KH = d->KH;
  p.KW = d->KW;
  p.stride = d->stride;
  p.pad = d->pad;
  p.Ho = d->Ho;
  p.Wo = d->Wo;
  p.lda = d->ldx ? d->ldx : d->Cin;
  p.ldb = p.K;
  p.ldc = d->ldy ? d->ldy : d->Cout;
  p.in_scale = pro ? pro->in_scale : nullptr;
  p.in_shift = pro ? pro->in_shift : nullptr;
  p.in_center = pro ? pro->in_center : nullptr;
  p.in_relu = pro ? pro->in_relu : 0;
  p.A2 = pro ? pro->x2 : nullptr;
  p.in2_scale = pro ? pro->in2_scale : nullptr;
  p.in2_shift = pro ? pro->in2_shift : nullptr;
  p.in2_center = pro ? pro->in2_center : nullptr;
  p.side_out = pro ? pro->side_out : nullptr;
  p.Bsplit = pro ? pro->w_split : nullptr;
  p.Bfrag = pro ? pro->w_frag : nullptr;
  p.math = (pro && pro->w_format) ? pro->w_format : MATH_BF16X6;
  VLNCE_CHECK_ARG(p.math == MATH_BF16X6 || p.math == MATH_F16X3,
                  "conv2d_fwd: w_format must be 0 / 1 (three bf16 planes) or 2 (fp16 planes)");
  VLNCE_CHECK_ARG((p.in_scale == nullptr) == (p.in_shift == nullptr),
                  "conv2d_fwd: in_scale and in_shift must come together");
  fill_epilogue(p, epi);
  const vlnce_bn_sums* const bnf = epi ? epi->bn : nullptr;
  if (bnf != nullptr) {
    VLNCE_CHECK_ARG(bnf->acc != nullptr, "conv2d_fwd: bn needs acc");
    VLNCE_CHECK_ARG(!p.stat_partial && !p.scale && !p.shift && !p.residual && !p.act && !p.accumulate,
                    "conv2d_fwd: bn excludes stat_partial / scale / shift / residual / act / accumulate");
    VLNCE_CHECK_ARG(bnf->workspace && bnf->workspace_bytes >= vlnce_conv2d_bn_workspace_bytes(d) &&
                        aligned16(bnf->workspace),
                    "conv2d_fwd: bn workspace too small (vlnce_conv2d_bn_workspace_bytes)");
  }
  auto bn_to_partials = [&]() {
    if (bnf != nullptr) {
      p.bn = vlnce_bn_sums{};
      p.stat_partial = static_cast<float*>(bnf->workspace);
    }
  };
  auto bn_sums_behind = [&](int rc) -> int { return rc; };
  auto bn_finalize_behind = [&](int rc) -> int {
    if (rc != 0 || bnf == nullptr) return rc;
    const int tiles = vlnce_conv2d_tiles_m(d);
    hipLaunchKernelGGL(bn_partials_to_sums_kernel, dim3(ceil_div(tiles, 128), ceil_div(d->Cout, 64)),
                       dim3(256), 0, reinterpret_cast<hipStream_t>(stream),
                       static_cast<const float*>(bnf->workspace), tiles, stat_rows_for(d), (int)M,
                       d->Cout, bnf->acc);
    VLNCE_CHECK_LAUNCH("conv2d_fwd bn moments -> sums");
    return 0;
  };
  const bool v4 = (d->Cin % 4 == 0) && (p.lda % 4 == 0) && aligned16(x) && aligned16(w) &&
                  (!p.in_scale || (aligned16(p.in_scale) && aligned16(p.in_shift))) &&
                  (!p.in_center || aligned16(p.in_center));
  p.splitk = 1;
  p.a_bytes = (((long)d->N * d->H * d->W - 1) * p.lda + d->Cin) * 4;
  p.b_bytes = (long)d->Cout * p.K * 4;
  p.c_bytes = ((M - 1) * p.ldc + d->Cout) * 4;
  p.stat_rows = stat_rows_for(d);
  hipStream_t s = reinterpret_cast<hipStream_t>(stream);
  g_last_path = VLNCE_CONV_PATH_F32;
  if (p.A2 != nullptr || p.side_out != nullptr) {
    VLNCE_CHECK_ARG(p.A2 && p.in_scale && d->KH == 1 && d->KW == 1 && d->stride == 1 &&
                        d->pad == 0 && v4 && buf_ok(p) && aligned16(p.A2) &&
                        (!p.side_out || aligned16(p.side_out)) &&
                        ((p.in2_scale == nullptr) == (p.in2_shift == nullptr)) &&
                        (!p.in2_scale || (aligned16(p.in2_scale) && aligned16(p.in2_shift))) &&
                        (!p.in2_center || (p.in2_scale && aligned16(p.in2_center))),
                    "conv2d_fwd: the dual-input prologue needs x2 + in_scale on a 1x1/stride-1/"
                    "pad-0 convolution with Cin %% 32 == 0 and 16-byte aligned operands");
    g_last_path = VLNCE_CONV_PATH_P3;
    if (const int rc = p3_try_launch(p, s); rc >= 0) return bn_sums_behind(rc);
    g_last_path = VLNCE_CONV_PATH_X3;
    if (X3Plan t; x3_plan(p, &t)) return bn_sums_behind(dispatch_x3<1>(p, t, s));
    g_last_path = VLNCE_CONV_PATH_F32;
    note_f32_kernel(VLNCE_CONV_KERNEL_F32_DUAL);
    bn_to_partials();
    return bn_finalize_behind(dispatch_dual(p, s));
  }
  if (v4 && buf_ok(p)) {
    g_last_path = VLNCE_CONV_PATH_M3;
    if (const int rc = m3_try_launch(p, s); rc >= 0) return bn_sums_behind(rc);
    g_last_path = VLNCE_CONV_PATH_F32;
    const int sk = (!p.accumulate && p.ldc == p.N && p.stat_rows <= 32 &&
                    ((p.scale && p.shift) || (!p.scale && !p.residual)))
                       ? choose_splitk(p)
                       : 1;
    if (sk > 1) {
      bn_to_partials();
      const float* scale = p.scale;
      const float* shift = p.shift;
      const float* residual = p.residual;
      float* stat_partial = p.stat_partial;
      const int act = p.act, ldr = p.ldr;
      p.scale = p.shift = p.residual = nullptr;
      p.stat_partial = nullptr;
      p.act = 0;
      p.splitk = sk;
      note_f32_kernel(VLNCE_CONV_KERNEL_F32_SPLITK, sk);
      vlnce_zero(y, M, p.N, p.ldc, s);
      if (int rc = dispatch_small<A_BUF, B_BUF>(p, s)) return rc;
      if (stat_partial) {
        const int nblk = ceil_div((int)M, p.stat_rows);
        hipLaunchKernelGGL(rows_stats_kernel, dim3(ceil_div(nblk, 4), ceil_div(p.N, 64)), dim3(256),
                           0, s, y, p.ldc, (int)M, p.N, p.stat_rows, stat_partial);
        VLNCE_CHECK_LAUNCH("conv2d_fwd split-K statistics");
      }
      if (bnf != nullptr) return bn_finalize_behind(0);
      if (scale) {
        VLNCE_CHECK_ARG(!residual || ldr == p.N, "conv2d_fwd: split-K needs a contiguous residual");
        return vlnce_scale_shift_act(y, scale, shift, nullptr, 0, residual, y, M, p.N, act, stream);
      }
      if (shift || act) {
        const long work = M * p.N;
        const int grid = (int)((work + 255) / 256 > 2048 ? 2048 : (work + 255) / 256);
        hipLaunchKernelGGL(bias_act_kernel, dim3(grid), dim3(256), 0, s, y, p.ldc, (int)M, p.N, shift, act);
        VLNCE_CHECK_LAUNCH("conv2d_fwd bias/act");
      }
      return 0;
    }
    g_last_path = VLNCE_CONV_PATH_P3;
    if (const int rc = p3_try_launch(p, s); rc >= 0) return bn_sums_behind(rc);
    g_last_path = VLNCE_CONV_PATH_X3;
    if (X3Plan t; x3_plan(p, &t)) return bn_sums_behind(dispatch_x3<0>(p, t, s));
    g_last_path = VLNCE_CONV_PATH_F32;
    note_f32_kernel(VLNCE_CONV_KERNEL_F32_BUF);
    bn_to_partials();
    return bn_finalize_behind(dispatch_tiles<A_BUF, B_BUF>(p, s));
  }
  bn_to_partials();
  note_f32_kernel(v4 ? VLNCE_CONV_KERNEL_F32_V4
                  : d->KW == 7 && d->Cin == 3 ? VLNCE_CONV_KERNEL_F32_STEM3
                  : d->KW == 7 && d->Cin == 1 ? VLNCE_CONV_KERNEL_F32_STEM1
                                              : VLNCE_CONV_KERNEL_F32_S);
  if (v4) return bn_finalize_behind(dispatch_tiles<A_IM2COL_V4, B_NK_V4>(p, s));
  if (d->KW == 7 && d->Cin == 3) return bn_finalize_behind(dispatch_stem<3>(p, s));
  if (d->KW == 7 && d->Cin == 1) return bn_finalize_behind(dispatch_stem<1>(p, s));
  return bn_finalize_behind(dispatch_tiles<A_IM2COL_S, B_NK_S>(p, s));
}

extern "C" int vlnce_gemm(const float* A, int lda, int transA, const float* B, int ldb, int transB,
                          float* C, int ldc, int M, int N, int K, const vlnce_epilogue* epi,
                          vlnce_stream_t stream) {
  VLNCE_CHECK_ARG(A && B && C, "gemm: null argument");
  VLNCE_CHECK_ARG(M > 0 && N > 0 && K > 0, "gemm: bad shape %d %d %d", M, N, K);
  VLNCE_CHECK_ARG(!(epi && epi->stat_partial), "gemm: stat_partial is a conv-only option");
  IgemmParams p{};
  p.A = A;
  p.B = B;
  p.C = C;
  p.M = M;
  p.N = N;
  p.K = K;
  VLNCE_CHECK_ARG((long)M < 32767L * 1024L, "gemm: M too large");
  p.W = M < 1024 ? M : 1024;
  p.H = ceil_div(M, p.W);
  p.Cin = K;
  p.KH = p.KW = 1;
  p.stride = 1;
  p.pad = 0;
  p.Ho = p.H;
  p.Wo = p.W;
  p.lda = lda;
  p.ldb = ldb;
  p.ldc = ldc;
  fill_epilogue(p, epi);
  hipStream_t s = reinterpret_cast<hipStream_t>(stream);
  p.splitk = 1;
  const bool plain = !p.scale && !p.residual && !(p.accumulate && p.act);
  if (plain) p.splitk = choose_splitk(p, transA != 0);
  const float* bias2 = nullptr;
  int act2 = 0;
  if (p.splitk > 1) {
    bias2 = p.shift;
    act2 = p.act;
    p.shift = nullptr;
    p.act = 0;
    if (!p.accumulate) vlnce_zero(C, M, N, ldc, s);
    p.accumulate = 0;
  }
  int rc;
  if (!transA) {
    const bool av4 = (K % 4 == 0) && (lda % 4 == 0) && aligned16(A);
    if (!transB) {
      const bool bv4 = (K % 4 == 0) && (ldb % 4 == 0) && aligned16(B);
      p.a_bytes = (((long)M - 1) * lda + K) * 4;
      p.b_bytes = (((long)N - 1) * ldb + K) * 4;
      if (av4 && bv4 && buf_ok(p))
        rc = p.splitk > 1 ? dispatch_small<A_BUF, B_BUF>(p, s) : dispatch_tiles<A_BUF, B_BUF>(p, s);
      else if (av4 && bv4)
        rc = p.splitk > 1 ? dispatch_small<A_IM2COL_V4, B_NK_V4>(p, s)
                          : dispatch_tiles<A_IM2COL_V4, B_NK_V4>(p, s);
      else
        rc = dispatch_small<A_IM2COL_S, B_NK_S>(p, s);
    } else {
      VLNCE_CHECK_ARG(aligned16(B), "gemm: B must be 16-byte aligned");
      if (av4)
        rc = p.splitk > 1 ? dispatch_small<A_IM2COL_V4, B_KN>(p, s)
                          : dispatch_tiles<A_IM2COL_V4, B_KN>(p, s);
      else
        rc = dispatch_small<A_IM2COL_S, B_KN>(p, s);
    }
  } else {
    VLNCE_CHECK_ARG(transB, "gemm: transA requires transB (only A^T * B^T-stored form is built)");
    VLNCE_CHECK_ARG(aligned16(A) && aligned16(B), "gemm: operands must be 16-byte aligned");
    rc = p.splitk > 1 ? dispatch_small<A_TRANS, B_KN>(p, s) : dispatch_tiles<A_TRANS, B_KN>(p, s);
  }
  if (rc != 0) return rc;
  if (p.splitk > 1 && (bias2 || act2)) {
    const long work = (long)M * N;
    const int grid = (int)((work + 255) / 256 > 2048 ? 2048 : (work + 255) / 256);
    hipLaunchKernelGGL(bias_act_kernel, dim3(grid), dim3(256), 0, s, C, ldc, M, N, bias2, act2);
    VLNCE_CHECK_LAUNCH("gemm bias/act");
  }
// ... 70 lines not shown
```

### vln-ce_amd/csrc/igemm_shared.h

```cpp
#pragma once
#include "common.h"
#include <stdlib.h>
#include <type_traits>

namespace vlnce_detail {

constexpr int BK = 32;
constexpr int LDP = 36;

enum { A_IM2COL_V4 = 0, A_IM2COL_S = 1, A_TRANS = 2, A_BUF = 3 };
enum { B_NK_V4 = 0, B_NK_S = 1, B_KN = 2, B_BUF = 3, B_IM2COL = 4 };

typedef unsigned int u32x4 __attribute__((ext_vector_type(4)));
typedef unsigned u32x2 __attribute__((ext_vector_type(2)));
constexpr int BUF_OOB = (int)0x80000000;

#ifdef VLNCE_DBG_TIME
#define DBG_T(...) __VA_ARGS__
#else
#define DBG_T(...)
#endif

struct IgemmParams {
  const float* A;
  const float* B;
  float* C;
  int M, N, K;
  int H, W, Cin, KH, KW, stride, pad, Ho, Wo;
  int lda, ldb, ldc;
  const float* in_scale;
  const float* in_shift;
  const float* in_center;
  int in_relu;
  const float* A2;
  const float* in2_scale;
  const float* in2_shift;
  const float* in2_center;
  float* side_out;
  const void* Bsplit;
  const void* Bfrag;
  int math;
  int p3_rows;
  const float* scale;
  const float* shift;
  const float* residual;
  int ldr;
  int act;
  int accumulate;
  float* stat_partial;
  vlnce_bn_sums bn;
  int tiles_m, tiles_n;
  int splitk;
  int stat_rows;
  long a_bytes, b_bytes, c_bytes;
};

__device__ __forceinline__ f32x4 ldg4(const float* p) { return *reinterpret_cast<const f32x4*>(p); }

template <int MT, int NT>
__device__ __forceinline__ void wave_stats(const f32x16 (&acc)[MT][NT], float* stat_partial,
                                           int part_row, int rows_left, int rows_full, int col0,
                                           int N, int half, int l31, float post = 1.f) {
  const int rows_valid = min(rows_full, rows_left);
#pragma unroll
  for (int j = 0; j < NT; ++j) {
    float s = 0.f;
#pragma unroll
    for (int i = 0; i < MT; ++i)
#pragma unroll
      for (int r = 0; r < 16; ++r) {
        const int row = i * 32 + (r & 3) + 8 * (r >> 2) + 4 * half;
        if (row < rows_valid) s += acc[i][j][r];
      }
    s += __shfl_xor(s, 32, 64);
    const float mean = rows_valid > 0 ? s / (float)rows_valid : 0.f;
    float m2 = 0.f;
#pragma unroll
    for (int i = 0; i < MT; ++i)
#pragma unroll
      for (int r = 0; r < 16; ++r) {
        const int row = i * 32 + (r & 3) + 8 * (r >> 2) + 4 * half;
        const float d = acc[i][j][r] - mean;
        if (row < rows_valid) m2 += d * d;
      }
    m2 += __shfl_xor(m2, 32, 64);
    const int col = col0 + j * 32 + l31;
    if (half == 0 && col < N && rows_left > 0) {
      float* dst = stat_partial + ((long)part_row * N + col) * 2;
      dst[0] = s * post;
      dst[1] = m2 * post * post;
    }
  }
}

template <int MT, int NT>
__device__ __forceinline__ void wave_stats_fine(const f32x16 (&acc)[MT][NT], float* stat_partial,
                                                int rows, int row0, int M, int col0, int N,
                                                int half, int l31, float post = 1.f) {
  const int nblk = MT * 32 / rows;
  for (int b = 0; b < nblk; ++b) {
    const int r_first = b * rows;
    const int left = M - (row0 + r_first);
    const int valid = min(rows, left);
#pragma unroll
    for (int j = 0; j < NT; ++j) {
      float s = 0.f;
#pragma unroll
      for (int i = 0; i < MT; ++i)
#pragma unroll
        for (int r = 0; r < 16; ++r) {
          const int row = i * 32 + (r & 3) + 8 * (r >> 2) + 4 * half;
          if (row >= r_first && row < r_first + valid) s += acc[i][j][r];
        }
      s += __shfl_xor(s, 32, 64);
      const float mean = valid > 0 ? s / (float)valid : 0.f;
      float m2 = 0.f;
#pragma unroll
      for (int i = 0; i < MT; ++i)
#pragma unroll
        for (int r = 0; r < 16; ++r) {
          const int row = i * 32 + (r & 3) + 8 * (r >> 2) + 4 * half;
          const float d = acc[i][j][r] - mean;
          if (row >= r_first && row < r_first + valid) m2 += d * d;
        }
      m2 += __shfl_xor(m2, 32, 64);
      const int col = col0 + j * 32 + l31;
      if (half == 0 && col < N && left > 0) {
        float* dst = stat_partial + ((long)((row0 + r_first) / rows) * N + col) * 2;
        dst[0] = s * post;
        dst[1] = m2 * post * post;
      }
    }
  }
}

template <int NT>
__device__ __forceinline__ void wave_stats_block(const f32x16 (&acc)[NT], float* stat_partial,
                                                 int part_row, int rows_left, int col0, int N,
                                                 int half, int l31, float post = 1.f) {
  const int rows_valid = min(32, rows_left);
#pragma unroll
  for (int j = 0; j < NT; ++j) {
    float s = 0.f;
#pragma unroll
    for (int r = 0; r < 16; ++r)
      if ((r & 3) + 8 * (r >> 2) + 4 * half < rows_valid) s += acc[j][r];
    s += __shfl_xor(s, 32, 64);
    const float mean = rows_valid > 0 ? s / (float)rows_valid : 0.f;
    float m2 = 0.f;
#pragma unroll
    for (int r = 0; r < 16; ++r) {
      const float d = acc[j][r] - mean;
      if ((r & 3) + 8 * (r >> 2) + 4 * half < rows_valid) m2 += d * d;
    }
    m2 += __shfl_xor(m2, 32, 64);
    const int col = col0 + j * 32 + l31;
    if (half == 0 && col < N && rows_left > 0) {
      float* dst = stat_partial + ((long)part_row * N + col) * 2;
      dst[0] = s * post;
      dst[1] = m2 * post * post;
    }
  }
}

template <int NT>
struct WaveBn {
  double s[NT], q[NT];
  int col0;
};
template <int NT>
__device__ __forceinline__ void wave_bn_reset(WaveBn<NT>& w) {
#pragma unroll
  for (int j = 0; j < NT; ++j) w.s[j] = w.q[j] = 0.0;
  w.col0 = -1;
}
template <int NT>
__device__ __forceinline__ void wave_bn_flush(WaveBn<NT>& w, double* acc, int N, int half, int l31) {
  acc += (long)(blockIdx.x % VLNCE_BN_SHARDS) * N * 2;
  if (w.col0 >= 0 && half == 0) {
#pragma unroll
    for (int j = 0; j < NT; ++j) {
      const int col = w.col0 + j * 32 + l31;
      if (col < N) {
        unsafeAtomicAdd(acc + 2 * col, w.s[j]);
        unsafeAtomicAdd(acc + 2 * col + 1, w.q[j]);
      }
    }
  }
  wave_bn_reset(w);
}
template <int NT>
__device__ __forceinline__ void wave_bn_block(const f32x16 (&acc)[NT], WaveBn<NT>& w, int rows_left,
                                              int half, float post = 1.f) {
  const int rows_valid = min(32, rows_left);
  if (rows_valid <= 0) return;
  const double inv_n = 1.0 / (double)rows_valid;
#pragma unroll
  for (int j = 0; j < NT; ++j) {
    float s = 0.f;
#pragma unroll
    for (int r = 0; r < 16; ++r)
      if ((r & 3) + 8 * (r >> 2) + 4 * half < rows_valid) s += acc[j][r];
    s += __shfl_xor(s, 32, 64);
    const float mean = s / (float)rows_valid;
    float m2 = 0.f;
#pragma unroll
    for (int r = 0; r < 16; ++r) {
// ... 38 lines not shown
#pragma unroll
      for (int r = 0; r < 16; ++r) {
        const int rw = i * 32 + (r & 3) + 8 * (r >> 2);
#pragma unroll
        for (int j = 0; j < NT; ++j) {
          const float v = apply_act(acc[i][j][r] * e_sc[j] + e_sh[j] + rv[j][r], act);
          __builtin_amdgcn_raw_buffer_store_b32(__builtin_bit_cast(unsigned, v), rsrc_c,
                                                rw < rows_left ? e_voff[j] : BUF_OOB, rw * ldc * 4, 0);
          if (clear) acc[i][j][r] = 0.f;
        }
      }
    }
    return;
  }
#pragma unroll
  for (int i = 0; i < MT; ++i)
#pragma unroll
    for (int r = 0; r < 16; ++r) {
      const int rw = i * 32 + (r & 3) + 8 * (r >> 2);
#pragma unroll
      for (int j = 0; j < NT; ++j) {
        const float v = apply_act(acc[i][j][r] * e_sc[j] + e_sh[j], act);
        __builtin_amdgcn_raw_buffer_store_b32(__builtin_bit_cast(unsigned, v), rsrc_c,
                                              rw < rows_left ? e_voff[j] : BUF_OOB, rw * ldc * 4, 0);
        if (clear) acc[i][j][r] = 0.f;
      }
    }
}

typedef __bf16 bf16x8 __attribute__((ext_vector_type(8)));
typedef _Float16 f16x8 __attribute__((ext_vector_type(8)));

enum { MATH_F32 = 0, MATH_BF16X6 = 1, MATH_F16X3 = 2 };
template <int MATH>
struct Planes;
template <>
struct Planes<MATH_BF16X6> {
  static constexpr int NA = 3, NB = 3, NP = 6;
  static constexpr int ROW = 208;
  static constexpr float POST = 1.f;
  static constexpr int PA[6] = {2, 1, 0, 1, 0, 0};
  static constexpr int PB[6] = {0, 1, 2, 0, 1, 0};
};
template <>
struct Planes<MATH_F16X3> {
  static constexpr int NA = 2, NB = 3, NP = 3;
  static constexpr int ROW = 144;
  static constexpr float POST = 1.f / 2048.f;
  static constexpr int PA[6] = {1, 0, 0, 0, 0, 0};
  static constexpr int PB[6] = {2, 1, 0, 0, 0, 0};
};
template <int MATH>
__device__ __forceinline__ f32x16 plane_mfma(bf16x8 a, bf16x8 b, f32x16 c) {
  if constexpr (MATH == MATH_F16X3)
    return __builtin_amdgcn_mfma_f32_32x32x16_f16(__builtin_bit_cast(f16x8, a),
                                                  __builtin_bit_cast(f16x8, b), c, 0, 0, 0);
  else
    return __builtin_amdgcn_mfma_f32_32x32x16_bf16(a, b, c, 0, 0, 0);
}
template <int MATH>
__device__ __forceinline__ void split_pair(float v0, float v1, unsigned (&w)[Planes<MATH>::NA]) {
  typedef float f32x2_ __attribute__((ext_vector_type(2)));
  if constexpr (MATH == MATH_F16X3) {
    typedef _Float16 f16x2_ __attribute__((ext_vector_type(2)));
    const f32x2_ v = {v0, v1};
    const f16x2_ h = __builtin_convertvector(v, f16x2_);
    w[0] = __builtin_bit_cast(unsigned, h);
    const f32x2_ r = {(v0 - (float)h[0]) * 2048.f, (v1 - (float)h[1]) * 2048.f};
    w[1] = __builtin_bit_cast(unsigned, __builtin_convertvector(r, f16x2_));
  } else {
    typedef __bf16 bf16x2_ __attribute__((ext_vector_type(2)));
    f32x2_ v = {v0, v1};
#pragma unroll
    for (int q = 0; q < 3; ++q) {
      const unsigned hb = __builtin_bit_cast(unsigned, __builtin_convertvector(v, bf16x2_));
      w[q] = hb;
      if (q < 2) {
        v[0] -= __builtin_bit_cast(float, hb << 16);
        v[1] -= __builtin_bit_cast(float, hb & 0xffff0000u);
      }
    }
  }
}
template <int MATH>
__device__ __forceinline__ void p3_split_store(f32x4 x, char* row_ptr) {
  constexpr int NA = Planes<MATH>::NA;
  unsigned w0[NA], w1[NA];
  split_pair<MATH>(x[0], x[1], w0);
  split_pair<MATH>(x[2], x[3], w1);
#pragma unroll
  for (int q = 0; q < NA; ++q) *reinterpret_cast<u32x2*>(row_ptr + q * 64) = u32x2{w0[q], w1[q]};
}
template <int MATH>
__device__ __forceinline__ void split_weight(float v, unsigned short (&o)[3]) {
  if constexpr (MATH == MATH_F16X3) {
    const _Float16 h = (_Float16)v;
    o[0] = __builtin_bit_cast(unsigned short, (_Float16)((float)h * 2048.f));
    o[1] = __builtin_bit_cast(unsigned short, (_Float16)((v - (float)h) * 2048.f));
    o[2] = __builtin_bit_cast(unsigned short, h);
  } else {
#pragma unroll
    for (int q = 0; q < 3; ++q) {
      const __bf16 hb = (__bf16)v;
      o[q] = __builtin_bit_cast(unsigned short, hb);
      v -= (float)hb;
    }
  }
}

__device__ __forceinline__ int x3_peek(const int* flag) {
  return __hip_atomic_load(flag, __ATOMIC_RELAXED, __HIP_MEMORY_SCOPE_WORKGROUP);
}
__device__ __forceinline__ void x3_wait(const int* flag, int seen, int need) {
  while (seen < need) {
    __builtin_amdgcn_s_sleep(1);
    seen = x3_peek(flag);
  }
  asm volatile("" ::: "memory");
}
__device__ __forceinline__ void x3_signal(int* flag) {
  typedef __attribute__((address_space(3))) int lds_int;
  const unsigned addr = (unsigned)(__UINTPTR_TYPE__)(lds_int*)flag;
  asm volatile("ds_add_u32 %0, %1" ::"v"(addr), "v"(1) : "memory");
}

static inline int x3_cus() {
  static const int cus = [] {
    int dev = 0, n = 256;
    if (hipGetDevice(&dev) != hipSuccess ||
        hipDeviceGetAttribute(&n, hipDeviceAttributeMultiprocessorCount, dev) != hipSuccess)
      n = 256;
    return n >= 8 ? (n / 8) * 8 : 8;
  }();
  return cus;
}

static inline int x3_lds_max() {
  static const int v = [] {
    int dev = 0, n = 0;
    if (hipGetDevice(&dev) != hipSuccess ||
        hipDeviceGetAttribute(&n, hipDeviceAttributeMaxSharedMemoryPerBlock, dev) != hipSuccess || n <= 0)
      n = 65536;
    return n;
  }();
  return v;
}

static inline int conv_math() { return vlnce_opt(VLNCE_OPT_CONV_MATH) != 0; }

int p3_try_launch(const IgemmParams& p, hipStream_t stream);
constexpr int U3_MAX_CIN = 4096;
int u3_launch(const IgemmParams& p, int bm, int dual_kind, int waves, hipStream_t stream);
int s3_launch(const IgemmParams& p, hipStream_t stream);
int m3_try_launch(const IgemmParams& p, hipStream_t stream);
int wgrad_x6_try_launch(const float* x, const float* dy, float* dw, const vlnce_conv_desc* d,
                        const float* dy_up, const float* dy_down, int accumulate,
                        hipStream_t stream);

void note_conv_kernel(int value);
void note_wgrad_kernel(int tm, bool split);

}
```

### vln-ce_amd/encoders/resnet_encoders.py

```python
import os
import warnings
from collections import OrderedDict

import numpy as np
import torch
import torch.nn as nn

from .. import ops
from ..config import Box, Dict
from ..streams import DropsGraphsOnApply, capture_guard, wait_ready
from . import trunk_backward as tb


class _WeightCache:

    def __init__(self):
        self._packed = {}
        self._folded = {}
        self._prep = None
        self._convs = None

    @staticmethod
    def _key(*ts):
        return tuple((t.data_ptr(), t._version, t.device) for t in ts)

    def conv(self, conv):
        k = self._key(conv.weight)
        hit = self._packed.get(id(conv))
        if hit is None or hit[0] != k:
            w = conv.weight.detach().permute(0, 2, 3, 1).contiguous()
            if not conv.weight.requires_grad:
                ops.check_weight_range(w)
            hit = (k, w)
            self._packed[id(conv)] = hit
        return hit[1]

    def prepare_trainable(self, trunk):
        if self._convs is None:
            self._convs = [m for m in trunk.modules() if isinstance(m, nn.Conv2d)]
        convs = [c for c in self._convs if c.weight.is_cuda and c.weight.is_contiguous()
                 and c.weight.size(0) % 32 == 0 and c.weight.size(1) % 32 == 0]
        if not convs or os.environ.get("VLNCE_WEIGHT_PREP", "1") == "0":
            return
        lib = ops.L()
        fmt = ops.plane_format()
        gfmt = ops.GRAD_PLANES if fmt == ops.PLANES_F16X3 else ops.PLANES_BF16X6
        sig = (fmt, gfmt) + tuple((id(c), c.weight.data_ptr()) for c in convs)
        st = self._prep
        if st is None or st["sig"] != sig:
            st = dict(sig=sig, key=None, rows=[], plan=None)
            jobs = []
            for c in convs:
                p = c.weight
                Cout, Cin, KH, KW = p.shape
                dev = p.device

                def i16(*shape):
                    return torch.empty(shape, device=dev, dtype=torch.int16)
                row = dict(conv=c,
                           w=(torch.empty((Cout, KH, KW, Cin), device=dev) if KH * KW > 1 else None),
                           split=i16(3, p.numel()), frag=i16(p.numel() * 3),
                           wt=torch.empty((Cin, KH, KW, Cout), device=dev),
                           split_t=i16(3, p.numel()), frag_t=i16(p.numel() * 3))
                row["split"]._vlnce_fmt = row["frag"]._vlnce_fmt = fmt
                row["split_t"]._vlnce_fmt = row["frag_t"]._vlnce_fmt = gfmt
                if row["w"] is not None:
                    jobs.append((p, row["w"], lib.WP_F32, 0, 0))
                jobs += [(p, row["split"], lib.WP_PLANES, 0, fmt),
                         (p, row["frag"], lib.WP_FRAGMENTS, 0, fmt),
                         (p, row["wt"], lib.WP_F32, 1, 0),
                         (p, row["split_t"], lib.WP_PLANES, 1, gfmt),
                         (p, row["frag_t"], lib.WP_FRAGMENTS, 1, gfmt)]
                st["rows"].append(row)
            st["plan"] = lib.weight_prep_plan(jobs)
            self._prep = st
        key = tuple(c.weight._version for c in convs)
        if st["key"] == key:
            return
        lib.conv2d_prepare_weights(st["plan"])
        st["key"] = key
        for row in st["rows"]:
            c = row["conv"]
            w = row["w"] if row["w"] is not None else c.weight.detach().permute(0, 2, 3, 1)
            wt = row["wt"]
            w.__dict__["_vlnce_split"] = {fmt: (w._version, row["split"])}
            w.__dict__["_vlnce_frag"] = {fmt: (w._version, row["frag"])}
            wt.__dict__["_vlnce_split"] = {gfmt: (wt._version, row["split_t"])}
            wt.__dict__["_vlnce_frag"] = {gfmt: (wt._version, row["frag_t"])}
            w._vlnce_dgrad = wt
            self._packed[id(c)] = (self._key(c.weight), w)

    def stem_s2d(self, conv):
        k = self._key(conv.weight)
        hit = self._packed.get(("s2d", id(conv)))
        if hit is None or hit[0] != k:
            hit = (k, ops.stem_weight_s2d(self.conv(conv)))
            self._packed[("s2d", id(conv))] = hit
        return hit[1]

    def stem7(self, conv):
        fmt = ops.plane_format(None, self.conv(conv))
        k = self._key(conv.weight) + (fmt,)
        hit = self._packed.get(("stem7", id(conv)))
        if hit is None or hit[0] != k:
            hit = (k, ops.stem7_pack_weights(self.conv(conv), fmt))
            self._packed[("stem7", id(conv))] = hit
        return hit[1], fmt

    def bn_eval(self, bn, gen=0):
        k = self._key(bn.weight, bn.bias, bn.running_mean, bn.running_var) + (gen,)
        hit = self._folded.get(id(bn))
        if hit is None or hit[0] != k:
            scale = bn.weight.detach() / torch.sqrt(bn.running_var + bn.eps)
            shift = bn.bias.detach() - bn.running_mean * scale
            hit = (k, scale.contiguous(), shift.contiguous())
            self._folded[id(bn)] = hit
        return hit[1], hit[2]


class _GraphRunner:

    MAX_GRAPHS = 6

    def __init__(self, fn):
        self.fn = fn
        self.entries = OrderedDict()

    @staticmethod
    def enabled():
        return os.environ.get("VLNCE_HIP_GRAPHS", "1") != "0"

    def captured(self, key):
        return not self.enabled() or isinstance(self.entries.get(key), list)

    @staticmethod
    def _parts(x):
        return tuple(x) if isinstance(x, (tuple, list)) else (x,)

    def __call__(self, x, key):
        parts = self._parts(x)
        probe = parts[0]
        if (not self.enabled() or not probe.is_cuda or torch.cuda.is_current_stream_capturing()):
            return self.fn(x)
        ent = self.entries.get(key)
        if ent is None:
            while len(self.entries) >= self.MAX_GRAPHS:
                self.entries.popitem(last=False)
            self.entries[key] = "seen"
            return self.fn(x)
        self.entries.move_to_end(key)
        cur = torch.cuda.current_stream(probe.device)
        if ent == "seen":
            static_in = tuple(None if t is None else t.clone() for t in parts)
            graph = torch.cuda.CUDAGraph()
            with capture_guard(), torch.cuda.graph(graph):
                static_out = self.fn(static_in if isinstance(x, (tuple, list)) else static_in[0])
            ent = [graph, static_in, static_out, None]
            self.entries[key] = ent
        else:
            if ent[3] is not None:
                cur.wait_event(ent[3])
            for dst, src in zip(ent[1], parts):
                if dst is not None:
                    dst.copy_(src)
        ent[0].replay()
        out = ent[2].clone()
        ent[3] = torch.cuda.Event()
        ent[3].record(cur)
        return out


def _stem_is_s2d(conv, H, W=None):
    if W is None:
        H, W = H.size(1), H.size(2)
    return (conv.kernel_size == (7, 7) and conv.stride == (2, 2) and conv.padding == (3, 3)
            and H % 2 == 0 and W % 2 == 0 and os.environ.get("VLNCE_STEM_S2D", "1") != "0")


def _as_nhwc(t_nchw_logical):
    return t_nchw_logical.permute(0, 2, 3, 1).contiguous()


def _grid_embedding_nhwc(emb, b, h, w):
    e = emb.weight.view(1, emb.embedding_dim, h, w).permute(0, 2, 3, 1)
    return e.expand(b, h, w, emb.embedding_dim)


def _c3(cin, cout, stride=1):
    return nn.Conv2d(cin, cout, 3, stride=stride, padding=1, bias=False)


def _c1(cin, cout, stride=1):
    return nn.Conv2d(cin, cout, 1, stride=stride, bias=False)


class BasicBlock(nn.Module):
    expansion = 1

    def __init__(self, inplanes, planes, stride=1, downsample=None):
        super().__init__()
        self.conv1 = _c3(inplanes, planes, stride)
        self.bn1 = nn.BatchNorm2d(planes)
        self.relu = nn.ReLU(inplace=True)
        self.conv2 = _c3(planes, planes)
        self.bn2 = nn.BatchNorm2d(planes)
        self.downsample = downsample
        self.stride = stride

    def stages(self):
        return [(self.conv1, self.bn1), (self.conv2, self.bn2)]


class Bottleneck(nn.Module):
    expansion = 4

    def __init__(self, inplanes, planes, stride=1, downsample=None):
        super().__init__()
        self.conv1 = _c1(inplanes, planes)
        self.bn1 = nn.BatchNorm2d(planes)
        self.conv2 = _c3(planes, planes, stride)
        self.bn2 = nn.BatchNorm2d(planes)
        self.conv3 = _c1(planes, planes * 4)
        self.bn3 = nn.BatchNorm2d(planes * 4)
        self.relu = nn.ReLU(inplace=True)
        self.downsample = downsample
        self.stride = stride

    def stages(self):
        return [(self.conv1, self.bn1), (self.conv2, self.bn2), (self.conv3, self.bn3)]


class _GlobalAvgPool(nn.Module):
    out_hw = (1, 1)


class SpatialAvgPool(nn.Module):
    out_hw = (4, 4)


class HipResNetTrunk(DropsGraphsOnApply, nn.Sequential):

    def __init__(self, block, layers):
        inplanes = 64
        mods = [nn.Conv2d(3, 64, 7, stride=2, padding=3, bias=False), nn.BatchNorm2d(64),
                nn.ReLU(inplace=True), nn.MaxPool2d(kernel_size=3, stride=2, padding=1)]
        for planes, n, stride in zip((64, 128, 256, 512), layers, (1, 2, 2, 2)):
            down = None
            if stride != 1 or inplanes != planes * block.expansion:
                down = nn.Sequential(_c1(inplanes, planes * block.expansion, stride),
                                     nn.BatchNorm2d(planes * block.expansion))
            blocks = [block(inplanes, planes, stride, down)]
            inplanes = planes * block.expansion
            blocks += [block(inplanes, planes) for _ in range(1, n)]
            mods.append(nn.Sequential(*blocks))
        mods.append(_GlobalAvgPool())
        super().__init__(*mods)
        self.final_channels = inplanes
        for m in self.modules():
            if isinstance(m, nn.Conv2d):
                nn.init.kaiming_normal_(m.weight, mode="fan_out", nonlinearity="relu")
        self._cache = _WeightCache()
        self.input_scale = None
        self._bn_gen = 0
        self._graphs = _GraphRunner(self._forward_impl)
        self._norms = [m for m in self.modules() if isinstance(m, nn.BatchNorm2d)]

    def _conv_bn_eval(self, x, conv, bn, relu, residual=None, prologue=None, s2d=False):
        pro = {} if prologue is None else dict(in_scale=prologue[0], in_shift=prologue[1])
        scale, shift = self._cache.bn_eval(bn, self._bn_gen)
        w, stride, pad = ((self._cache.stem_s2d(conv), 1, 0) if s2d else
                          (self._cache.conv(conv), conv.stride[0], conv.padding[0]))
        return ops.conv2d_nhwc(x, w, stride, pad, scale=scale, shift=shift, residual=residual,
                               act=ops.ACT_RELU if relu else ops.ACT_NONE, **pro)

    def _conv_stats(self, x, conv, bn, touched, prologue=None, in_relu=False, s2d=False,
                    dual=None):
        pro = {}
        if prologue is not None:
            pro = dict(in_scale=prologue[0], in_shift=prologue[1], in_relu=in_relu,
                       in_center=prologue[2] if len(prologue) > 2 else None)
        if dual is not None:
            x2, p2, side = dual
            pro.update(x2=x2, side_out=side)
            if p2 is not None:
                pro.update(in2_scale=p2[0], in2_shift=p2[1], in2_center=p2[2])
        w, stride, pad = ((self._cache.stem_s2d(conv), 1, 0) if s2d else
                          (self._cache.conv(conv), conv.stride[0], conv.padding[0]))
        assert bn.momentum is not None
        if os.environ.get("VLNCE_BN_FUSED", "1") == "0":
            y, stats = ops.conv2d_nhwc(x, w, stride, pad, want_stats=True, **pro)
            pend = ops.bn_finalize(stats, y.numel() // y.size(-1), bn.weight, bn.bias, bn.eps,
                                   bn.momentum, bn.running_mean, bn.running_var)
            touched.append(bn.num_batches_tracked)
            return y, pend
        y, pend = ops.conv2d_bn_train(x, w, stride, pad, bn, **pro)
        touched.append(bn.num_batches_tracked)
        return y, pend

    @staticmethod
    def _materialise(pending):
        raw, pend, skip, pskip = pending
        if pskip is not None:
            return ops.scale_shift_add_act(raw, pend[0], pend[1], skip, pskip[0], pskip[1],
                                           act=ops.ACT_RELU, out=raw, c1=pend[2], c2=pskip[2])
        return ops.scale_shift_act(raw, pend[0], pend[1], center=pend[2], residual=skip,
                                   act=ops.ACT_RELU, out=raw)

    @staticmethod
    def _takes_pending(blk, pending):
        conv = blk.stages()[0][0]
        return (conv.kernel_size == (1, 1) and conv.stride == (1, 1) and conv.padding == (0, 0)
                and conv.in_channels % 32 == 0 and pending[0].numel() * 4 < (1 << 31)
                and os.environ.get("VLNCE_FUSE_BLOCK_END", "1") != "0")

    def _block_train(self, x, pending, blk, touched):
        st = blk.stages()
        if pending is not None and self._takes_pending(blk, pending):
            raw3, pend3, skip, pskip = pending
            x = torch.empty_like(raw3)
            raw, pend = self._conv_stats(raw3, st[0][0], st[0][1], touched, prologue=pend3,
                                         in_relu=True, dual=(skip, pskip, x))
        else:
            if pending is not None:
                x = self._materialise(pending)
            raw, pend = self._conv_stats(x, st[0][0], st[0][1], touched)
        for conv, bn in st[1:]:
            raw, pend = self._conv_stats(raw, conv, bn, touched, prologue=pend, in_relu=True)
        if blk.downsample is not None:
            rd, pd = self._conv_stats(x, blk.downsample[0], blk.downsample[1], touched)
            return raw, pend, rd, pd
        return raw, pend, x, None

    def _block_eval(self, x, blk):
        identity = x
        if blk.downsample is not None:
            identity = self._conv_bn_eval(x, blk.downsample[0], blk.downsample[1], False)
        st = blk.stages()
        for conv, bn in st[:-1]:
            x = self._conv_bn_eval(x, conv, bn, True)
        return self._conv_bn_eval(x, st[-1][0], st[-1][1], True, residual=identity)

    def forward(self, x_nhwc_raw):
        if torch.is_grad_enabled() and any(p.requires_grad for p in self._plist()):
            x = ops.frames_f32(ops.frames(x_nhwc_raw))
            return tb.TrunkFn.apply(self, x, *tb.trainable_params(self)).permute(0, 3, 1, 2)
        key, train = self._graph_key(ops.frames_signature(x_nhwc_raw))
        y = self._graphs(x_nhwc_raw, key)
        if train:
            self._bn_gen += 1
        return y.permute(0, 3, 1, 2)

    def _graph_key(self, signature):
        modes = tuple(m.training for m in self._norms)
        if any(modes) and not all(modes):
            raise NotImplementedError("mixed train/eval BatchNorm modes inside one trunk")
        key = (signature, modes[0], tuple(p._version for p in self._plist(checked=False)),
               id(self.input_scale[0]), len(self._modules),
               0 if modes[0] else self._bn_gen, ops.plane_format())
        return key, modes[0]

    def graph_ready(self, x):
        return self._graphs.captured(self._graph_key(ops.frames_signature(x))[0])

    def _forward_impl(self, x):
        with torch.no_grad():
            kids = list(self.children())
            train = kids[1].training
            touched = []
            fr = ops.frames(x)
            s2d = _stem_is_s2d(kids[0], fr["H"], fr["W"])
            pro = self.input_scale
            stem7 = (s2d and fr["C"] == 3 and kids[0].out_channels in (32, 64)
                     and os.environ.get("VLNCE_STEM7", "1") != "0")
            if stem7:
                wf, wfmt = self._cache.stem7(kids[0])
                if train:
                    bn = kids[1]
                    acc = ops._bn_state(bn)
                    raw = ops.stem7(fr, wf, kids[0].out_channels, pro[0], pro[1], bn_acc=acc,
                                    w_format=wfmt)
                    pend = ops.bn_finalize_sums(acc, raw.numel() // raw.size(-1), bn)
                    touched.append(bn.num_batches_tracked)
                    x = ops.maxpool3x3s2(raw, pend[0], pend[1], in_relu=True, in_center=pend[2])
                else:
                    sc, sh = self._cache.bn_eval(kids[1], self._bn_gen)
                    x = ops.stem7(fr, wf, kids[0].out_channels, pro[0], pro[1], scale=sc, shift=sh,
                                  act=ops.ACT_RELU, w_format=wfmt)
                    x = ops.maxpool3x3s2(x)
            else:
                if s2d:
                    x = ops.frames_s2d(fr, 2, 1, self.input_scale[0], self.input_scale[1])
                    pro = None
                else:
                    x = ops.frames_f32(fr)
                if train:
                    raw, pend = self._conv_stats(x, kids[0], kids[1], touched, prologue=pro, s2d=s2d)
                    x = ops.maxpool3x3s2(raw, pend[0], pend[1], in_relu=True, in_center=pend[2])
                else:
                    x = self._conv_bn_eval(x, kids[0], kids[1], True, prologue=pro, s2d=s2d)
                    x = ops.maxpool3x3s2(x)
            pending = None
            for stage in kids[4:8]:
                for blk in stage:
                    if train:
                        pending = self._block_train(x, pending, blk, touched)
                        x = None
                    else:
                        x = self._block_eval(x, blk)
            if pending is not None:
                x = self._materialise(pending)
            for pool in kids[8:]:
                x = ops.adaptive_avgpool(x, *pool.out_hw)
            if touched:
                torch._foreach_add_(touched, 1)
        return x


    def run_recording(self, x):
        kids = list(self.children())
        self._cache.prepare_trainable(self)
        sc, sh = self.input_scale
        x = ops.scale_shift_act(x, sc, sh)
        blocks = [(None if blk.downsample is None else tuple(blk.downsample), blk.stages())
                  for stage in kids[4:8] for blk in stage]
        x, tape, touched = tb.record(x, self._cache.conv, (kids[0], kids[1]), blocks,
                                     [("avgpool", pool.out_hw) for pool in kids[8:]])
        if touched:
            torch._foreach_add_(touched, 1)
        if any(m.training for m in self._norms):
            self._bn_gen += 1
        return x, tape


_TV_CHILD_INDEX = {"conv1": "0", "bn1": "1", "layer1": "4", "layer2": "5", "layer3": "6",
                   "layer4": "7"}


def torchvision_trunk_state_dict(sd):
    out = {}
    for k, v in sd.items():
        head, _, rest = k.partition(".")
        if head == "fc":
            continue
        out[(_TV_CHILD_INDEX.get(head, head) + "." + rest) if rest else k] = v
    return out


class TorchVisionResNet(nn.Module):

    def __init__(self, output_size, resnet_version="resnet50", normalize_visual_inputs=False,
                 trainable=False, spatial_output=False, single_spatial_filter=True,
                 pretrained_weights=None):
        super().__init__()
        self.normalize_visual_inputs = normalize_visual_inputs
        self.spatial_output = spatial_output
        if resnet_version == "resnet50":
            self.cnn = HipResNetTrunk(Bottleneck, [3, 4, 6, 3])
        elif resnet_version == "resnet18":
            self.cnn = HipResNetTrunk(BasicBlock, [2, 2, 2, 2])
        else:
            raise ValueError(resnet_version)
        self.resnet_layer_size = self.cnn.final_channels
        pretrained_weights = pretrained_weights or os.environ.get("VLNCE_TORCHVISION_WEIGHTS")
        if pretrained_weights and pretrained_weights != "NONE":
            self.load_torchvision_weights(pretrained_weights)
        elif not trainable:
            warnings.warn(
                f"TorchVisionResNet({resnet_version}): the frozen RGB trunk is RANDOMLY initialised "
                "(the reference uses ImageNet weights, pretrained=True).  Set "
                "MODEL.RGB_ENCODER.pretrained_weights / VLNCE_TORCHVISION_WEIGHTS to a torchvision "
                "state_dict, or restore a full policy checkpoint before training.", stacklevel=2)
        for p in self.cnn.parameters():
            p.requires_grad_(trainable)
        self.cnn.train(trainable)
        if not spatial_output:
            self.output_shape = (output_size,)
            self.fc = nn.Sequential(nn.Flatten(), nn.Linear(self.resnet_layer_size, output_size),
                                    nn.ReLU())
        else:
            if single_spatial_filter:
                del self.cnn[8]
            self.cnn.avgpool = SpatialAvgPool()
            self.spatial_embeddings = nn.Embedding(4 * 4, 64)
            self.output_shape = (self.resnet_layer_size + 64, 4, 4)
        self._in_cache = None

    def load_torchvision_weights(self, path_or_state_dict):
        sd = path_or_state_dict
        if not isinstance(sd, dict):
            sd = torch.load(sd, map_location="cpu", weights_only=True)
        sd = sd.get("state_dict", sd)
        self.cnn.load_state_dict(torchvision_trunk_state_dict(sd), strict=True)

    def _input_transform(self, device):
        if self._in_cache is None or self._in_cache[0].device != device:
            if self.normalize_visual_inputs:
                mean = torch.tensor([0.485, 0.456, 0.406], device=device)
                std = torch.tensor([0.229, 0.224, 0.225], device=device)
                sc, sh = 1.0 / (255.0 * std), -mean / std
            else:
                sc = torch.full((3,), 1.0 / 255.0, device=device)
                sh = torch.zeros(3, device=device)
            self._in_cache = (sc.contiguous(), sh.contiguous())
        return self._in_cache

    def trunk_features(self, observations):
        rgb = observations["rgb"]
        self.cnn.input_scale = self._input_transform(_GraphRunner._parts(rgb)[0].device)
        return self.cnn(rgb)

    def trunk_parameters(self):
        return self.cnn._plist()

    def trunk_ready(self, observations):
        self.cnn.input_scale = self._input_transform(_GraphRunner._parts(observations["rgb"])[0].device)
        return self.cnn.graph_ready(observations["rgb"])

    def forward(self, observations):
        if "rgb_features" in observations:
            feats = wait_ready(observations["rgb_features"], observations, "rgb_features")
        else:
            feats = self.trunk_features(observations)
        if not self.spatial_output:
            return ops.linear(feats.reshape(feats.size(0), -1), self.fc[1].weight, self.fc[1].bias,
                              ops.ACT_RELU)
        b, _, h, w = feats.shape
        x = torch.cat([_as_nhwc(feats), _grid_embedding_nhwc(self.spatial_embeddings, b, h, w)],
                      dim=3)
        return x.permute(0, 3, 1, 2)


class TorchVisionResNet50(TorchVisionResNet):
    def __init__(self, *args, **kwargs):
        super().__init__(*args, resnet_version="resnet50", **kwargs)


class TorchVisionResNet18(TorchVisionResNet):
    def __init__(self, *args, **kwargs):
        super().__init__(*args, resnet_version="resnet18", **kwargs)


class _GNBlock(nn.Module):
    def stages(self):
        mods = [m for m in self.convs if not isinstance(m, nn.ReLU)]
        return list(zip(mods[0::2], mods[1::2]))


class GNBasicBlock(_GNBlock):
    expansion = 1

    def __init__(self, inplanes, planes, ngroups, stride=1, downsample=None):
        super().__init__()
        self.convs = nn.Sequential(_c3(inplanes, planes, stride), nn.GroupNorm(ngroups, planes),
                                   nn.ReLU(True), _c3(planes, planes),
                                   nn.GroupNorm(ngroups, planes))
        self.downsample = downsample
        self.relu = nn.ReLU(True)


class GNBottleneck(_GNBlock):
    expansion = 4
# ... 188 lines not shown
```

### vln-ce_amd/ops.py

```python
import os

import torch
import torch.nn.functional as F
from torch.autograd import Function

from . import _lib

ACT_NONE, ACT_RELU, ACT_SIGMOID, ACT_TANH = 0, 1, 2, 3


def L():
    return _lib.get_lib()


def _f32c(t):
    if t.dtype != torch.float32:
        t = t.float()
    return t if t.is_contiguous() else t.contiguous()


def _rows2d(t):
    if t.dim() != 2 or t.stride(1) != 1 or (t.size(0) > 1 and t.stride(0) < t.size(1)):
        t = t.reshape(-1, t.size(-1)).contiguous()
    ld = t.stride(0) if t.size(0) > 1 else t.size(1)
    return t, ld


PLANES_BF16X6, PLANES_F16X3 = 1, 2


def plane_format(w_format=None, w=None):
    if w_format:
        return int(w_format)
    forced = getattr(w, "_vlnce_force_fmt", None) if w is not None else None
    return forced or L().plane_format()


GRAD_PLANES = (PLANES_BF16X6 if os.environ.get("VLNCE_GRAD_PLANES", "f16") in ("bf16", "1")
               else PLANES_F16X3)
_ZEROS = {}


def zeros_vec(device, n):
    z = _ZEROS.get(device)
    if z is None or z.numel() < n:
        z = torch.zeros(max(4096, n), device=device, dtype=torch.float32)
        _ZEROS[device] = z
    return z[:n]


F16_PLANES_MAX_WEIGHT = 16.0


def check_weight_range(w_ohwi):
    if w_ohwi.is_cuda and not torch.cuda.is_current_stream_capturing():
        w_ohwi._vlnce_force_fmt = (PLANES_BF16X6 if float(w_ohwi.abs().max()) >= F16_PLANES_MAX_WEIGHT
                                   else None)
    return w_ohwi


def split_weights(w_ohwi, fmt=None):
    if not w_ohwi.is_cuda or w_ohwi.shape[-1] % 32 != 0 or w_ohwi.dtype != torch.float32:
        return None
    fmt = plane_format(fmt)
    cache = w_ohwi.__dict__.setdefault("_vlnce_split", {})
    hit = cache.get(fmt)
    if hit is None or hit[0] != w_ohwi._version:
        planes = torch.empty((3, w_ohwi.numel()), device=w_ohwi.device, dtype=torch.int16)
        L().conv2d_split_weights(w_ohwi, planes, fmt)
        planes._vlnce_fmt = fmt
        hit = (w_ohwi._version, planes)
        cache[fmt] = hit
    return hit[1]


def pack_weights(w_ohwi, fmt=None):
    if (not w_ohwi.is_cuda or w_ohwi.dtype != torch.float32 or w_ohwi.shape[-1] % 32 != 0
            or w_ohwi.shape[0] % 32 != 0):
        return None
    fmt = plane_format(fmt)
    cache = w_ohwi.__dict__.setdefault("_vlnce_frag", {})
    hit = cache.get(fmt)
    if hit is None or hit[0] != w_ohwi._version:
        Cout, KH, KW, Cin = w_ohwi.shape
        g = dict(N=1, H=KH, W=KW, Cin=Cin, Cout=Cout, KH=KH, KW=KW, stride=1, pad=0, Ho=1, Wo=1,
                 ldx=Cin, ldy=Cout)
        nbytes = L().conv2d_pack_bytes(g)
        if nbytes <= 0:
            return None
        frag = torch.empty((nbytes // 2,), device=w_ohwi.device, dtype=torch.int16)
        L().conv2d_pack_weights(w_ohwi, frag, g, fmt)
        frag._vlnce_fmt = fmt
        hit = (w_ohwi._version, frag)
        cache[fmt] = hit
    return hit[1]


def conv_geometry(x, w, stride, pad, ldx=None):
    N, H, W, Cin = x.shape
    Cout, KH, KW, Cin2 = w.shape
    assert Cin == Cin2, (x.shape, w.shape)
    Ho = (H + 2 * pad - KH) // stride + 1
    Wo = (W + 2 * pad - KW) // stride + 1
    return dict(N=N, H=H, W=W, Cin=Cin, Cout=Cout, KH=KH, KW=KW, stride=stride, pad=pad,
                Ho=Ho, Wo=Wo, ldx=ldx or Cin, ldy=Cout)


def conv2d_nhwc(x, w_ohwi, stride, pad, *, in_scale=None, in_shift=None, in_center=None,
                in_relu=False, scale=None, shift=None, residual=None, act=ACT_NONE,
                want_stats=False, x2=None, in2_scale=None, in2_shift=None, in2_center=None,
                side_out=None, w_format=None):
    assert x.is_contiguous() and w_ohwi.is_contiguous()
    g = conv_geometry(x, w_ohwi, stride, pad)
    y = torch.empty((g["N"], g["Ho"], g["Wo"], g["Cout"]), device=x.device, dtype=torch.float32)
    stats = None
    partial = None
    if want_stats:
        tiles_m, tile_rows = L().conv2d_tiles(g)
        partial = torch.empty((tiles_m, g["Cout"], 2), device=x.device, dtype=torch.float32)
        stats = (partial, tiles_m, tile_rows)
    if residual is not None:
        assert residual.is_contiguous() and residual.shape == y.shape
    dual = {}
    if x2 is not None:
        assert x2.is_contiguous() and x2.shape == x.shape
        assert side_out is None or (side_out.is_contiguous() and side_out.shape == x.shape)
        dual = dict(x2=x2, in2_scale=in2_scale, in2_shift=in2_shift, in2_center=in2_center,
                    side_out=side_out)
    fmt = plane_format(w_format, w_ohwi)
    L().conv2d_fwd(x, w_ohwi, y, g, in_scale=in_scale, in_shift=in_shift, in_center=in_center,
                   in_relu=int(in_relu), **dual, scale=scale, shift=shift, residual=residual, ldr=g["Cout"], act=act,
                   stat_partial=partial, w_split=split_weights(w_ohwi, fmt),
                   w_frag=pack_weights(w_ohwi, fmt), w_format=fmt)
    return (y, stats) if want_stats else y


BN_SHARDS = 16


def _bn_state(bn):
    w = bn.weight
    acc = bn.__dict__.get("_vlnce_acc")
    if acc is None or acc.device != w.device or acc.size(1) != w.numel():
        acc = torch.zeros((BN_SHARDS, w.numel(), 2), device=w.device, dtype=torch.float64)
        bn.__dict__["_vlnce_acc"] = acc
    return acc


def conv2d_bn_sums(x, w_ohwi, stride, pad, acc, **pro):
    assert x.is_contiguous() and w_ohwi.is_contiguous()
    g = conv_geometry(x, w_ohwi, stride, pad)
    y = torch.empty((g["N"], g["Ho"], g["Wo"], g["Cout"]), device=x.device, dtype=torch.float32)
    lib = L()
    ws = torch.empty(max(lib.conv2d_bn_workspace_bytes(g), 16), device=x.device, dtype=torch.uint8)
    if pro.get("x2") is not None:
        assert pro["x2"].is_contiguous() and pro["x2"].shape == x.shape
    if "in_relu" in pro:
        pro = dict(pro, in_relu=int(pro["in_relu"]))
    fmt = plane_format(None, w_ohwi)
    lib.conv2d_fwd(x, w_ohwi, y, g, **pro, ldr=g["Cout"], w_split=split_weights(w_ohwi, fmt),
                   w_frag=pack_weights(w_ohwi, fmt), bn=(acc, ws), w_format=fmt)
    return y


def bn_finalize_sums(acc, M, bn):
    Cc = bn.weight.numel()
    scale = torch.empty(Cc, device=acc.device, dtype=torch.float32)
    mean = torch.empty_like(scale)
    L().bn_finalize_sums(acc, M, bn.weight.detach(), bn.bias.detach(), bn.eps, bn.momentum,
                         bn.running_mean, bn.running_var, scale, mean)
    return scale, bn.bias.detach(), mean


def conv2d_bn_train(x, w_ohwi, stride, pad, bn, **pro):
    assert bn.momentum is not None
    acc = _bn_state(bn)
    try:
        y = conv2d_bn_sums(x, w_ohwi, stride, pad, acc, **pro)
        return y, bn_finalize_sums(acc, y.numel() // y.size(-1), bn)
    except Exception:
        if not (acc.is_cuda and torch.cuda.is_current_stream_capturing()):
            acc.zero_()
        raise


def bn_finalize(stats, M, gamma, beta, eps, momentum, running_mean, running_var):
    partial, tiles_m, tile_rows = stats
    Cc = partial.size(1)
    scale = torch.empty(Cc, device=partial.device, dtype=torch.float32)
    folded = torch.empty_like(scale)
    mean = torch.empty_like(scale)
    lib = L()
    wb = lib.bn_finalize_workspace_bytes(tiles_m, Cc)
    ws = torch.empty(wb // 8, device=partial.device, dtype=torch.float64) if wb else None
    lib.bn_finalize(partial, tiles_m, tile_rows, M, Cc, gamma, beta, float(eps), float(momentum),
                    running_mean, running_var, scale, folded, mean, None, workspace=ws)
    return scale, beta.detach(), mean


def scale_shift_act(x, scale, shift, *, center=None, rows_per_sample=0, residual=None,
                    act=ACT_NONE, out=None):
    assert x.is_contiguous()
    Cc = x.size(-1)
    M = x.numel() // Cc
    y = out if out is not None else torch.empty_like(x)
    L().scale_shift_act(x, scale, shift, rows_per_sample, residual, y, M, Cc, act, center=center)
    return y


GN_SMALL_ELEMENTS = 1 << 20


def _gn_small(x):
    return (x.is_cuda and x.numel() <= GN_SMALL_ELEMENTS
            and os.environ.get("VLNCE_GN_SMALL", "1") != "0")


def group_norm_act(x, groups, gamma, beta, eps, *, residual=None, act=ACT_NONE):
    assert x.is_contiguous()
    N, H, W, Cc = x.shape
    HW = H * W
    lib = L()
    if _gn_small(x):
        y = torch.empty_like(x)
        lib.group_norm_small(x, N, HW, Cc, groups, gamma, beta, float(eps), residual, act, y)
        return y
    chunks = lib.gn_chunks(HW)
    partial = torch.empty((N, chunks, Cc, 2), device=x.device, dtype=torch.float32)
    lib.gn_partial(x, N, HW, Cc, partial)
    scale = torch.empty((N, Cc), device=x.device, dtype=torch.float32)
    shift = torch.empty_like(scale)
    center = torch.empty_like(scale)
    lib.gn_finalize(partial, N, HW, Cc, groups, gamma, beta, float(eps), scale, shift,
                    center_out=center)
    return scale_shift_act(x, scale, shift, center=center, rows_per_sample=HW, residual=residual,
                           act=act)


def conv_group_norm_act(x, w_ohwi, stride, pad, groups, gamma, beta, eps, *, residual=None,
                        act=ACT_NONE):
    g = conv_geometry(x, w_ohwi, stride, pad)
    if x.is_cuda and g["N"] * g["Ho"] * g["Wo"] * g["Cout"] <= GN_SMALL_ELEMENTS and \
            os.environ.get("VLNCE_GN_SMALL", "1") != "0":
        return group_norm_act(conv2d_nhwc(x, w_ohwi, stride, pad), groups, gamma, beta, eps,
                              residual=residual, act=act)
    y, stats = conv2d_nhwc(x, w_ohwi, stride, pad, want_stats=True)
    partial, _tiles_m, tile_rows = stats
    N, Ho, Wo, Cc = y.shape
    HW = Ho * Wo
    if HW % tile_rows != 0:
        return group_norm_act(y, groups, gamma, beta, eps, residual=residual, act=act)
    scale = torch.empty((N, Cc), device=y.device, dtype=torch.float32)
    shift = torch.empty_like(scale)
    center = torch.empty_like(scale)
    L().gn_finalize_tiles(partial, tile_rows, N, HW, Cc, groups, gamma, beta, float(eps), scale,
                          shift, center_out=center)
    return scale_shift_act(y, scale, shift, center=center, rows_per_sample=HW, residual=residual,
                           act=act)


def maxpool3x3s2(x, in_scale=None, in_shift=None, in_relu=False, in_center=None):
    N, H, W, Cc = x.shape
    Ho, Wo = (H + 2 - 3) // 2 + 1, (W + 2 - 3) // 2 + 1
    y = torch.empty((N, Ho, Wo, Cc), device=x.device, dtype=torch.float32)
    L().maxpool3x3s2(x, y, N, H, W, Cc, Ho, Wo, in_scale, in_shift, int(in_relu),
                     in_center=in_center)
    return y


def scale_shift_add_act(x1, s1, t1, x2, s2, t2, act=ACT_NONE, out=None, c1=None, c2=None):
    assert x1.is_contiguous() and x2.is_contiguous() and x1.shape == x2.shape
    Cc = x1.size(-1)
    y = out if out is not None else torch.empty_like(x1)
    L().scale_shift_add_act(x1, s1, t1, x2, s2, t2, y, x1.numel() // Cc, Cc, act, c1=c1, c2=c2)
    return y


def space_to_depth2(x, pad_lo, pad_hi, scale=None, shift=None):
    assert x.is_contiguous()
    N, H, W, Cc = x.shape
    y = torch.empty((N, H // 2 + pad_lo + pad_hi, W // 2 + pad_lo + pad_hi, 4 * Cc),
                    device=x.device, dtype=torch.float32)
    L().space_to_depth2(x, y, N, H, W, Cc, pad_lo, pad_hi, scale, shift)
    return y


def stem_weight_s2d(w_ohwi):
    Cout, KH, KW, Cc = w_ohwi.shape
    assert KH == 7 and KW == 7
    w8 = torch.zeros((Cout, 8, 8, Cc), device=w_ohwi.device, dtype=w_ohwi.dtype)
    w8[:, 1:, 1:] = w_ohwi
    return (w8.view(Cout, 4, 2, 4, 2, Cc).permute(0, 1, 3, 2, 4, 5)
            .reshape(Cout, 4, 4, 4 * Cc).contiguous())


def _frame_view(t):
    if t.dtype not in (torch.uint8, torch.float32):
        t = t.float()
    imgs = t.numel() // (t.size(-3) * t.size(-2) * t.size(-1)) if t.numel() else 0
    H, W, Cc = t.shape[-3:]
    if t.is_contiguous():
        return t.reshape(imgs, H, W, Cc), H, W, 0, 0
    t4 = None
    if t.dim() == 4:
        t4 = t
    elif t.dim() == 5 and t.stride(0) == t.size(1) * t.stride(1):
        t4 = torch.as_strided(t, (imgs, H, W, Cc), t.stride()[1:], t.storage_offset())
    if t4 is not None and imgs > 1 and t4.stride(3) == 1 and t4.stride(2) == Cc:
        sN, sH = t4.stride(0), t4.stride(1)
        if sH % Cc == 0 and sH > 0 and sN > 0 and sN % sH == 0:
            Ws, Hs = sH // Cc, sN // sH
            off = t4.storage_offset() % sN
            y0, rem = divmod(off, sH)
            if rem % Cc == 0 and y0 + H <= Hs and rem // Cc + W <= Ws:
                x0 = rem // Cc
                try:
                    base = torch.as_strided(t4, (imgs, Hs, Ws, Cc), (sN, sH, Cc, 1),
                                            t4.storage_offset() - off)
                    return base, Hs, Ws, y0, x0
                except RuntimeError:
                    pass
    return t.contiguous().reshape(imgs, H, W, Cc), H, W, 0, 0


def frames(x):
    x2 = mask2 = None
    if isinstance(x, (tuple, list)):
        x, x2, mask2 = x
    F_ = x.size(1) if x.dim() == 5 else 1
    N = x.size(0)
    base, Hs, Ws, y0, x0 = _frame_view(x)
    H, W, Cc = x.shape[-3:]
# ... 773 lines not shown
```

Baseline: 7909.

## Regenerate bottleneck conv3 output inside next block's conv1 instead of storing it

Adds a conv_r3 kernel that recomputes the last 1x1 conv of a bottleneck block (with its BN/ReLU prologue) from the preceding activation inside the next block's first conv, fused with the skip add. The original last conv then runs in a statistics-only mode that only accumulates BN sums and never writes its output. The aim is to avoid writing and re-reading the large expanded-channel activation. In exchange it repeats that conv's FLOPs, and selection is gated by a measured-shape table and row-count threshold, defaulting on via the new r3 option.

New measurement: 8116, median of 6. +2.6%, better.

```diff
diff --git a/include/vlnce_hip.h b/include/vlnce_hip.h
--- a/include/vlnce_hip.h
+++ b/include/vlnce_hip.h
@@ -28,6 +28,16 @@
   int Ho, Wo;
   int ldx, ldy;
 } vlnce_conv_desc;
+
+typedef struct {
+  const float* x;
+  int Cin, ldx;
+  const void* w_frag;
+  const float* in_scale;
+  const float* in_shift;
+  const float* in_center;
+  int in_relu;
+} vlnce_regen;
 
 typedef struct {
   const float* in_scale;
@@ -43,6 +53,7 @@
   const void* w_frag;
   const int* options;
   int w_format;
+  const vlnce_regen* regen;
 } vlnce_prologue;
 
 #define VLNCE_BN_SHARDS 16
@@ -61,6 +72,7 @@
   int accumulate;
   float* stat_partial;
   const vlnce_bn_sums* bn;
+  int stats_only;
 } vlnce_epilogue;
 
 long vlnce_conv2d_bn_workspace_bytes(const vlnce_conv_desc* d);
@@ -108,6 +120,7 @@
 #define VLNCE_CONV_KERNEL_P3 0
 #define VLNCE_CONV_KERNEL_U3 1
 #define VLNCE_CONV_KERNEL_S3 2
+#define VLNCE_CONV_KERNEL_R3 3
 #define VLNCE_CONV_P3_DENSE 0
 #define VLNCE_CONV_P3_GATHER 1
 #define VLNCE_CONV_P3_DUAL 2
diff --git a/vln-ce_amd/_lib.py b/vln-ce_amd/_lib.py
--- a/vln-ce_amd/_lib.py
+++ b/vln-ce_amd/_lib.py
@@ -28,13 +28,14 @@
 ("conv_p3" | "conv_u3" | "conv_s3", "conv_m3", "conv_x3", "buf" | "splitk" | "v4" | "s" | "stem3" |
 "stem1" | "dual" of igemm_kernel); fmt: plane format 1 / 2 (0: fp32); a, b, c per kernel:
   conv_p3: tile 1..6, mode "dense" | "gather" | "dual", 0      conv_u3: rows, kind 0..2, waves
-  conv_s3: Cin, 0, 0      conv_m3: NT, KSPLIT, RB      conv_x3: tile 1..4, dual 0 / 1, 0
+  conv_s3: Cin, 1 = statistics only, 0      conv_r3: regenerated Cin, Cout / 32, skip kind 1 / 2
+  conv_m3: NT, KSPLIT, RB      conv_x3: tile 1..4, dual 0 / 1, 0
   splitk: the split factor, 0, 0"""
 WgradKernel = collections.namedtuple("WgradKernel", "path tm split")
 
 _FAMILIES = ("f32", "x3", "p3", "m3")
 _KERNELS = {"f32": ("buf", "splitk", "v4", "s", "stem3", "stem1", "dual"), "x3": ("conv_x3",),
-            "p3": ("conv_p3", "conv_u3", "conv_s3"), "m3": ("conv_m3",)}
+            "p3": ("conv_p3", "conv_u3", "conv_s3", "conv_r3"), "m3": ("conv_m3",)}
 _P3_MODES = ("dense", "gather", "dual")
 
 
@@ -70,7 +71,13 @@
 class Prologue(C.Structure):
     _fields_ = [("in_scale", _P), ("in_shift", _P), ("in_center", _P), ("in_relu", _I),
                 ("x2", _P), ("in2_scale", _P), ("in2_shift", _P), ("in2_center", _P),
-                ("side_out", _P), ("w_split", _P), ("w_frag", _P), ("options", _P), ("w_format", _I)]
+                ("side_out", _P), ("w_split", _P), ("w_frag", _P), ("options", _P), ("w_format", _I),
+                ("regen", _P)]
+
+
+class Regen(C.Structure):
+    _fields_ = [("x", _P), ("Cin", _I), ("ldx", _I), ("w_frag", _P), ("in_scale", _P), ("in_shift", _P),
+                ("in_center", _P), ("in_relu", _I)]
 
 
 class Frames(C.Structure):
@@ -89,7 +96,8 @@
 
 class Epilogue(C.Structure):
     _fields_ = [("scale", _P), ("shift", _P), ("residual", _P), ("ldr", _I), ("act", _I),
-                ("accumulate", _I), ("stat_partial", _P), ("bn", C.POINTER(BnSums))]
+                ("accumulate", _I), ("stat_partial", _P), ("bn", C.POINTER(BnSums)),
+                ("stats_only", _I)]
 
 
 _SIGNATURES = {
@@ -278,7 +286,7 @@
 
     name = "hip"
 
-    ABI = 147
+    ABI = 148
 
     def __init__(self, path=LIB_PATH):
         self.dll = load_cdll(path)
@@ -292,7 +300,8 @@
         self._options_from_env()
 
     OPTION_NAMES = ("conv_math", "p3", "p3_tile", "s3", "u3", "u3_waves", "x3_tile", "igemm_tile",
-                    "igemm_nobuf", "igemm_no_splitk", "wgrad_tile", "rollout_one_xcd", "m3")
+                    "igemm_nobuf", "igemm_no_splitk", "wgrad_tile", "rollout_one_xcd", "m3", "r3",
+                    "s3_wgs")
 
     def _options_from_env(self):
         for name in self.OPTION_NAMES:
@@ -331,6 +340,12 @@
                 v = self._conv_math = self.get_option("conv_math")
         return 2 if v == 2 else 1
 
+    def effective_option(self, name):
+        sc = getattr(self._tls, "scoped", None)
+        if sc and sc.get(name, -1) >= 0:
+            return int(sc[name])
+        return self.get_option(name)
+
     def get_option(self, name):
         v = _I(0)
         self._check(self.dll.vlnce_get_option(name.encode(), C.byref(v)), "vlnce_get_option")
@@ -341,7 +356,7 @@
         self._check(self.dll.vlnce_option_default(name.encode(), C.byref(v)), "vlnce_option_default")
         return v.value
 
-    PER_LAUNCH = ("conv_math", "p3", "p3_tile", "s3", "u3", "u3_waves", "x3_tile", "m3")
+    PER_LAUNCH = ("conv_math", "p3", "p3_tile", "s3", "u3", "u3_waves", "x3_tile", "m3", "r3", "s3_wgs")
 
     def _launch_options(self, overrides):
         if not overrides:
@@ -395,21 +410,29 @@
     def conv2d_fwd(self, x, w, y, g, in_scale=None, in_shift=None, in_relu=0, scale=None,
                    shift=None, residual=None, ldr=0, act=0, accumulate=0, stat_partial=None,
                    in_center=None, x2=None, in2_scale=None, in2_shift=None, in2_center=None,
-                   side_out=None, w_split=None, w_frag=None, bn=None, options=None, w_format=None):
+                   side_out=None, w_split=None, w_frag=None, bn=None, options=None, w_format=None,
+                   stats_only=False, regen=None):
         d = self._desc(g)
-        w_format = _buffer_format(w_format, w_split, w_frag)
+        w_format = _buffer_format(w_format, w_split, w_frag, regen["w_frag"] if regen else None)
+        rg = None
+        if regen is not None:
+            rx = regen["x"]
+            rg = Regen(_ptr(rx), rx.size(-1), rx.size(-1), _ptr(regen["w_frag"]),
+                       _ptr(regen.get("in_scale")), _ptr(regen.get("in_shift")),
+                       _ptr(regen.get("in_center")), int(regen.get("in_relu", 0)))
         opts = self._launch_options(options if options is not None
                                     else getattr(self._tls, "scoped", None))
         pro = Prologue(_ptr(in_scale), _ptr(in_shift), _ptr(in_center), int(in_relu), _ptr(x2),
                        _ptr(in2_scale), _ptr(in2_shift), _ptr(in2_center), _ptr(side_out),
                        _ptr(w_split), _ptr(w_frag),
-                       C.cast(opts, C.c_void_p) if opts is not None else None, int(w_format))
+                       C.cast(opts, C.c_void_p) if opts is not None else None, int(w_format),
+                       C.cast(C.pointer(rg), C.c_void_p) if rg is not None else None)
         bnp = None
         if bn is not None:
             acc, ws = bn
             bnp = C.pointer(BnSums(_ptr(acc), _ptr(ws), ws.numel() * ws.element_size()))
         epi = Epilogue(_ptr(scale), _ptr(shift), _ptr(residual), int(ldr), int(act),
-                       int(accumulate), _ptr(stat_partial), bnp)
+                       int(accumulate), _ptr(stat_partial), bnp, int(bool(stats_only)))
         self._check(self.dll.vlnce_conv2d_fwd(_ptr(x), _ptr(w), _ptr(y), C.byref(d), C.byref(pro),
                                               C.byref(epi), _stream()), "vlnce_conv2d_fwd")
 
diff --git a/vln-ce_amd/csrc/api.cpp b/vln-ce_amd/csrc/api.cpp
--- a/vln-ce_amd/csrc/api.cpp
+++ b/vln-ce_amd/csrc/api.cpp
@@ -16,7 +16,7 @@
 }
 
 extern "C" const char* vlnce_last_error(void) { return g_err; }
-extern "C" int vlnce_version(void) { return 147; }
+extern "C" int vlnce_version(void) { return 148; }
 
 namespace {
 struct OptDef {
@@ -27,10 +27,10 @@
     {"conv_math", 2},   {"p3", 2},          {"p3_tile", 0},         {"s3", 1},
     {"u3", 1},          {"u3_waves", 8},    {"x3_tile", 0},         {"igemm_tile", 0},
     {"igemm_nobuf", 0}, {"igemm_no_splitk", 0}, {"wgrad_tile", 64}, {"rollout_one_xcd", 0},
-    {"m3", 1},
+    {"m3", 1},          {"r3", 1},          {"s3_wgs", 0},
 };
 std::atomic<int> g_opt[VLNCE_OPT_COUNT] = {
-    {2}, {2}, {0}, {1}, {1}, {8}, {0}, {0}, {0}, {0}, {64}, {0}, {1},
+    {2}, {2}, {0}, {1}, {1}, {8}, {0}, {0}, {0}, {0}, {64}, {0}, {1}, {1}, {0},
 };
 int opt_index(const char* name) {
   if (name)
diff --git a/vln-ce_amd/csrc/common_opts.h b/vln-ce_amd/csrc/common_opts.h
--- a/vln-ce_amd/csrc/common_opts.h
+++ b/vln-ce_amd/csrc/common_opts.h
@@ -17,6 +17,8 @@
   VLNCE_OPT_WGRAD_TILE,
   VLNCE_OPT_ROLLOUT_ONE_XCD,
   VLNCE_OPT_M3,
+  VLNCE_OPT_R3,
+  VLNCE_OPT_S3_WGS,
   VLNCE_OPT_COUNT
 };
 int vlnce_opt(int id);
diff --git a/vln-ce_amd/csrc/conv_r3.hip b/vln-ce_amd/csrc/conv_r3.hip
--- /dev/null
+++ b/vln-ce_amd/csrc/conv_r3.hip
@@ -0,0 +1,373 @@
+#include "igemm_shared.h"
+
+using namespace vlnce_detail;
+
+namespace vlnce_detail {
+namespace {
+
+__device__ __forceinline__ float swap_odd_even(float v) {
+  return __builtin_bit_cast(
+      float, __builtin_amdgcn_update_dpp(0, __builtin_bit_cast(int, v), 0xB1, 0xF, 0xF, true));
+}
+
+template <int NCC, int N2B, int SKIP, int MATH>
+__global__ __launch_bounds__(512) void conv_r3_kernel(IgemmParams p, RegenParams g) {
+#if defined(__HIP_DEVICE_COMPILE__)
+  typedef Planes<MATH> PL;
+  constexpr int ROW = PL::ROW, NA = PL::NA, NP = PL::NP;
+  constexpr int BM = 64, MT = 2;
+  constexpr int KS1 = NCC * 2;
+  constexpr int NPASS = NCC / 2;
+  constexpr int KS2 = NCC * 8;
+  constexpr int CBUF = BM * ROW;
+  constexpr int P1 = NCC * CBUF;
+  constexpr int YB = 8 * CBUF;
+  constexpr int MT2 = N2B == 8 ? 2 : 1;
+  constexpr int AHEAD = (NCC == 2 && MATH == MATH_F16X3) ? 3 : 2;
+  constexpr bool EARLY_B2 = NCC == 2;
+  constexpr int AH1 = NCC == 2 ? 4 : 2;
+  constexpr bool FENCE_SLABS = NCC == 4 || MATH == MATH_BF16X6;
+  extern __shared__ __attribute__((aligned(16))) char xsm[];
+
+  const int tid = threadIdx.x;
+  const int lane = tid & 63;
+  const int wave = __builtin_amdgcn_readfirstlane(tid >> 6);
+  const int half = lane >> 5;
+  const int l31 = lane & 31;
+  const int trow = tid >> 3;
+  const int lk4 = (tid & 7) * 4;
+  const int wg = (int)blockIdx.x, nwg = (int)gridDim.x;
+  const int my_tiles = (p.tiles_m - wg + nwg - 1) / nwg;
+  if (my_tiles <= 0) return;
+
+  const __amdgpu_buffer_rsrc_t rsrc_a = __builtin_amdgcn_make_buffer_rsrc(
+      const_cast<char*>(reinterpret_cast<const char*>(g.x)), 0, (int)g.x_bytes, 0x00020000);
+  const __amdgpu_buffer_rsrc_t rsrc_b1 = __builtin_amdgcn_make_buffer_rsrc(
+      const_cast<char*>(reinterpret_cast<const char*>(g.w_frag)), 0, NCC * 128 * NCC * 32 * 6, 0x00020000);
+  const __amdgpu_buffer_rsrc_t rsrc_s = __builtin_amdgcn_make_buffer_rsrc(
+      const_cast<char*>(reinterpret_cast<const char*>(p.A2)), 0, (int)p.a_bytes, 0x00020000);
+  const __amdgpu_buffer_rsrc_t rsrc_y = __builtin_amdgcn_make_buffer_rsrc(
+      reinterpret_cast<char*>(p.side_out), 0, (int)p.a_bytes, 0x00020000);
+  const __amdgpu_buffer_rsrc_t rsrc_b2 = __builtin_amdgcn_make_buffer_rsrc(
+      const_cast<char*>(reinterpret_cast<const char*>(p.Bfrag)), 0, N2B * 32 * NCC * 128 * 6, 0x00020000);
+  const __amdgpu_buffer_rsrc_t rsrc_c = __builtin_amdgcn_make_buffer_rsrc(
+      reinterpret_cast<char*>(p.C), 0, (int)p.c_bytes, 0x00020000);
+  const float relu2 = g.relu ? 0.f : -__builtin_huge_valf();
+  const float relu3 = p.in_relu ? 0.f : -__builtin_huge_valf();
+
+  bf16x8 bres[AH1][3];
+  auto load_b1 = [&](bf16x8 (&f)[3], int pass, int ks) {
+    const int vb = (pass * 8 + wave) * KS1 * 3072 + lane * 16;
+#pragma unroll
+    for (int q = 0; q < 3; ++q)
+      f[q] = __builtin_bit_cast(
+          bf16x8, __builtin_amdgcn_raw_buffer_load_b128(rsrc_b1, vb + q * 1024, ks * 3072, 0));
+  };
+  auto preload_b1 = [&](int pass) {
+#pragma unroll
+    for (int k = 0; k < AH1; ++k) load_b1(bres[k], pass, k);
+  };
+  preload_b1(0);
+  float* const vlds = reinterpret_cast<float*>(xsm + P1 + YB);
+  if (tid < 8) {
+    const f32x4 zero4 = {0.f, 0.f, 0.f, 0.f}, one4 = {1.f, 1.f, 1.f, 1.f};
+#pragma unroll
+    for (int c = 0; c < NCC; ++c) {
+      f32x4 s_ = one4, t_ = zero4, c_ = zero4;
+      if (g.scale != nullptr) {
+        s_ = ldg4(g.scale + c * 32 + lk4);
+        t_ = ldg4(g.shift + c * 32 + lk4);
+        if (g.center) c_ = ldg4(g.center + c * 32 + lk4);
+      }
+      *reinterpret_cast<f32x4*>(vlds + c * 32 + lk4) = s_;
+      *reinterpret_cast<f32x4*>(vlds + NCC * 32 + c * 32 + lk4) = t_;
+      *reinterpret_cast<f32x4*>(vlds + 2 * NCC * 32 + c * 32 + lk4) = c_;
+    }
+  }
+  __syncthreads();
+  float s3[NPASS], t3[NPASS], c3[NPASS], s2[NPASS], c2[NPASS];
+#pragma unroll
+  for (int ps = 0; ps < NPASS; ++ps) {
+    const int col = ps * 256 + wave * 32 + l31;
+    s3[ps] = p.in_scale[col];
+    t3[ps] = p.in_shift[col];
+    c3[ps] = p.in_center ? p.in_center[col] : 0.f;
+    s2[ps] = c2[ps] = 0.f;
+    if constexpr (SKIP == 2) {
+      s2[ps] = p.in2_scale[col];
+      t3[ps] = t3[ps] + p.in2_shift[col];
+      c2[ps] = p.in2_center ? p.in2_center[col] : 0.f;
+    }
+  }
+
+  f32x4 raw[NCC];
+  auto load_raw = [&](int round) {
+    const int m = (wg + round * nwg) * BM + trow;
+    const int vo = (round < my_tiles && m < p.M) ? (m * g.ldx + lk4) * 4 : BUF_OOB;
+#pragma unroll
+    for (int c = 0; c < NCC; ++c)
+      raw[c] = __builtin_bit_cast(f32x4, __builtin_amdgcn_raw_buffer_load_b128(rsrc_a, vo, c * 128, 0));
+  };
+  float sk[MT][16];
+  auto load_skip = [&](int round, int pass) {
+    const int m0 = (wg + round * nwg) * BM;
+    const int rows_left = p.M - (m0 + 4 * half);
+    const int voff = round < my_tiles
+                         ? (int)((((long)(m0 + 4 * half)) * p.lda + pass * 256 + wave * 32 + l31) * 4)
+                         : BUF_OOB;
+#pragma unroll
+    for (int i = 0; i < MT; ++i)
+#pragma unroll
+      for (int r = 0; r < 16; ++r) {
+        const int rw = i * 32 + (r & 3) + 8 * (r >> 2);
+        sk[i][r] = __builtin_bit_cast(float, __builtin_amdgcn_raw_buffer_load_b32(
+                                                 rsrc_s, rw < rows_left ? voff : BUF_OOB, rw * p.lda * 4, 0));
+        if ((r & 7) == 7) __builtin_amdgcn_sched_barrier(0);
+      }
+  };
+  load_raw(0);
+  load_skip(0, 0);
+
+  const bool active2 = N2B == 2 ? wave < 4 : true;
+  const int cb = wave % N2B;
+  const int rb = N2B == 8 ? 0 : (wave / N2B) & 1;
+  const int vb2 = cb * KS2 * 3072 + lane * 16;
+  bf16x8 fb[AHEAD][3];
+  auto load_b2 = [&](bf16x8 (&f)[3], int slab) {
+#pragma unroll
+    for (int q = 0; q < 3; ++q)
+      f[q] = __builtin_bit_cast(
+          bf16x8, __builtin_amdgcn_raw_buffer_load_b128(rsrc_b2, vb2 + q * 1024, slab * 3072, 0));
+  };
+  auto preload_b2 = [&](int ps) {
+    if (active2) {
+#pragma unroll
+      for (int k = 0; k < AHEAD; ++k) load_b2(fb[k], ps * 16 + k);
+    }
+  };
+  if constexpr (EARLY_B2) preload_b2(0);
+  WaveBn<1> wbn;
+  wave_bn_reset(wbn);
+  const int a_off = l31 * ROW + half * 16;
+  char* const ypatch = xsm + P1;
+  const bool odd = (l31 & 1) != 0;
+
+  for (int round = 0; round < my_tiles; ++round) {
+    const int m0 = (wg + round * nwg) * BM;
+    {
+      const bool row_ok = m0 + trow < p.M;
+#pragma unroll
+      for (int c = 0; c < NCC; ++c) {
+        f32x4 v = raw[c];
+        const f32x4 s_ = *reinterpret_cast<const f32x4*>(vlds + c * 32 + lk4);
+        const f32x4 t_ = *reinterpret_cast<const f32x4*>(vlds + NCC * 32 + c * 32 + lk4);
+        const f32x4 c_ = *reinterpret_cast<const f32x4*>(vlds + 2 * NCC * 32 + c * 32 + lk4);
+#pragma unroll
+        for (int e = 0; e < 4; ++e) {
+          v[e] = fmaxf(fmaf(v[e] - c_[e], s_[e], t_[e]), relu2);
+          v[e] = row_ok ? v[e] : 0.f;
+        }
+        p3_split_store<MATH>(v, xsm + c * CBUF + trow * ROW + lk4 * 2);
+      }
+      load_raw(round + 1);
+    }
+    asm volatile("s_waitcnt lgkmcnt(0)" ::: "memory");
+    __builtin_amdgcn_s_barrier();
+
+    f32x16 acc2[MT2];
+#pragma unroll
+    for (int i = 0; i < MT2; ++i)
+#pragma unroll
+      for (int r = 0; r < 16; ++r) acc2[i][r] = 0.f;
+    const int rows_left = p.M - (m0 + 4 * half);
+
+#pragma unroll
+    for (int ps = 0; ps < NPASS; ++ps) {
+      f32x16 acc[MT];
+#pragma unroll
+      for (int i = 0; i < MT; ++i)
+#pragma unroll
+        for (int r = 0; r < 16; ++r) acc[i][r] = 0.f;
+#pragma unroll
+      for (int c = 0; c < NCC; ++c)
+#pragma unroll
+        for (int h = 0; h < 2; ++h) {
+          bf16x8 f[MT][NA];
+#pragma unroll
+          for (int i = 0; i < MT; ++i)
+#pragma unroll
+            for (int q = 0; q < NA; ++q)
+              f[i][q] = *reinterpret_cast<const bf16x8*>(xsm + c * CBUF + a_off + i * 32 * ROW + q * 64 +
+                                                         h * 32);
+#pragma unroll
+          for (int q = 0; q < NP; ++q)
+#pragma unroll
+            for (int i = 0; i < MT; ++i)
+              acc[i] = plane_mfma<MATH>(f[i][PL::PA[q]], bres[(c * 2 + h) % AH1][PL::PB[q]], acc[i]);
+          if (c * 2 + h + AH1 < KS1) load_b1(bres[(c * 2 + h) % AH1], ps, c * 2 + h + AH1);
+          if constexpr (FENCE_SLABS) __builtin_amdgcn_sched_barrier(0);
+        }
+      __builtin_amdgcn_sched_barrier(0);
+      float yv[MT][16];
+      {
+        char* const yb = ypatch + wave * CBUF + half * 4 * ROW + (l31 >> 1) * 4 + (odd ? ROW : 0);
+#pragma unroll
+        for (int i = 0; i < MT; ++i)
+#pragma unroll
+          for (int r = 0; r < 16; ++r) {
+            const int rw = i * 32 + (r & 3) + 8 * (r >> 2);
+            const float raw3 = fmaf(acc[i][r], PL::POST, 0.f);
+            float v;
+            if constexpr (SKIP == 2)
+              v = fmaxf(fmaf(raw3 - c3[ps], s3[ps], fmaf(sk[i][r] - c2[ps], s2[ps], t3[ps])), relu3);
+            else
+              v = fmaxf(fmaf(raw3 - c3[ps], s3[ps], t3[ps]) + sk[i][r], relu3);
+            yv[i][r] = rw < rows_left ? v : 0.f;
+          }
+#pragma unroll
+        for (int i = 0; i < MT; ++i)
+#pragma unroll
+          for (int j = 0; j < 8; ++j) {
+            const int rw = i * 32 + ((2 * j) & 3) + 8 * ((2 * j) >> 2);
+            const float v0 = yv[i][2 * j], v1 = yv[i][2 * j + 1];
+            const float got = swap_odd_even(odd ? v0 : v1);
+            unsigned w[NA];
+            split_pair<MATH>(odd ? got : v0, odd ? v1 : got, w);
+#pragma unroll
+            for (int q = 0; q < NA; ++q) *reinterpret_cast<unsigned*>(yb + rw * ROW + q * 64) = w[q];
+            if ((j & 3) == 3) __builtin_amdgcn_sched_barrier(0);
+          }
+      }
+      asm volatile("s_waitcnt lgkmcnt(0)" ::: "memory");
+      __builtin_amdgcn_s_barrier();
+      if constexpr (!EARLY_B2) preload_b2(ps);
+      if (active2) {
+#pragma unroll
+        for (int c = 0; c < 8; ++c)
+#pragma unroll
+          for (int h = 0; h < 2; ++h) {
+            const int sl = c * 2 + h;
+            bf16x8 f[MT2][NA];
+#pragma unroll
+            for (int i = 0; i < MT2; ++i)
+#pragma unroll
+              for (int q = 0; q < NA; ++q)
+                f[i][q] = *reinterpret_cast<const bf16x8*>(ypatch + c * CBUF + a_off +
+                                                           (rb + i) * 32 * ROW + q * 64 + h * 32);
+#pragma unroll
+            for (int q = 0; q < NP; ++q)
+#pragma unroll
+              for (int i = 0; i < MT2; ++i)
+                acc2[i] = plane_mfma<MATH>(f[i][PL::PA[q]], fb[sl % AHEAD][PL::PB[q]], acc2[i]);
+            if (sl + AHEAD < 16) load_b2(fb[sl % AHEAD], ps * 16 + sl + AHEAD);
+            if constexpr (FENCE_SLABS) __builtin_amdgcn_sched_barrier(0);
+          }
+      }
+      __builtin_amdgcn_sched_barrier(0);
+      {
+        const int y_voff = (int)((((long)(m0 + 4 * half)) * p.lda + ps * 256 + wave * 32 + l31) * 4);
+        if constexpr (NPASS > 1) preload_b1((ps + 1) % NPASS);
+        if constexpr (EARLY_B2) preload_b2((ps + 1) % NPASS);
+        if (ps + 1 < NPASS) load_skip(round, ps + 1);
+        else load_skip(round + 1, 0);
+#pragma unroll
+        for (int i = 0; i < MT; ++i)
+#pragma unroll
+          for (int r = 0; r < 16; ++r) {
+            const int rw = i * 32 + (r & 3) + 8 * (r >> 2);
+            __builtin_amdgcn_raw_buffer_store_b32(__builtin_bit_cast(unsigned, yv[i][r]), rsrc_y,
+                                                  rw < rows_left ? y_voff : BUF_OOB, rw * p.lda * 4, 0);
+            if ((r & 7) == 7) __builtin_amdgcn_sched_barrier(0);
+          }
+      }
+      if (ps + 1 < NPASS) {
+        asm volatile("s_waitcnt lgkmcnt(0)" ::: "memory");
+        __builtin_amdgcn_s_barrier();
+      }
+    }
+    __builtin_amdgcn_sched_barrier(0);
+    if (active2) {
+      const int r0 = m0 + rb * 32;
+      if (p.bn.acc != nullptr) {
+        wave_bn_tile<MT2, 1>(reinterpret_cast<const f32x16(&)[MT2][1]>(acc2), wbn, p.bn.acc, cb * 32,
+                             p.N, p.M - r0, half, l31, PL::POST);
+      } else if (p.stat_partial != nullptr) {
+#pragma unroll
+        for (int i = 0; i < MT2; ++i)
+          wave_stats_block<1>(reinterpret_cast<const f32x16(&)[1]>(acc2[i]), p.stat_partial,
+                              r0 / 32 + i, p.M - (r0 + i * 32), cb * 32, p.N, half, l31, PL::POST);
+      }
+      const int rows_left2 = p.M - (r0 + 4 * half);
+      const int e_voff = (int)((((long)(r0 + 4 * half)) * p.ldc + cb * 32 + l31) * 4);
+#pragma unroll
+      for (int i = 0; i < MT2; ++i)
+#pragma unroll
+        for (int r = 0; r < 16; ++r) {
+          const int rw = i * 32 + (r & 3) + 8 * (r >> 2);
+          const float v = fmaf(acc2[i][r], PL::POST, 0.f);
+          __builtin_amdgcn_raw_buffer_store_b32(__builtin_bit_cast(unsigned, v), rsrc_c,
+                                                rw < rows_left2 ? e_voff : BUF_OOB, rw * p.ldc * 4, 0);
+          if ((r & 7) == 7) __builtin_amdgcn_sched_barrier(0);
+        }
+    }
+  }
+  if (p.bn.acc != nullptr) wave_bn_flush(wbn, p.bn.acc, p.N, half, l31);
+#endif
+}
+
+template <int NCC, int N2B, int SKIP, int MATH>
+int launch_r3(const IgemmParams& p, const RegenParams& g, hipStream_t stream) {
+  constexpr int smem_bytes = (NCC + 8) * 64 * Planes<MATH>::ROW + 3 * NCC * 32 * 4;
+  if (smem_bytes > x3_lds_max()) {
+    vlnce_set_error("conv_r3: %d bytes of LDS per workgroup, the device allows %d", smem_bytes, x3_lds_max());
+    return 1;
+  }
+  auto kern = conv_r3_kernel<NCC, N2B, SKIP, MATH>;
+  static bool attr_set = false;
+  if (!attr_set) {
+    hipError_t e = hipFuncSetAttribute(reinterpret_cast<const void*>(kern),
+                                       hipFuncAttributeMaxDynamicSharedMemorySize, smem_bytes);
+    if (e != hipSuccess) {
+      vlnce_set_error("conv_r3: hipFuncSetAttribute failed: %s", hipGetErrorString(e));
+      return 2;
+    }
+    attr_set = true;
+  }
+  IgemmParams q = p;
+  q.tiles_m = ceil_div(p.M, 64);
+  q.tiles_n = 1;
+  q.splitk = 1;
+  long grid = q.tiles_m;
+  if (grid > x3_cus()) grid = x3_cus();
+  if (const int cap = vlnce_opt(VLNCE_OPT_S3_WGS); cap > 0 && grid > cap) grid = cap;
+  hipLaunchKernelGGL(kern, dim3((unsigned)grid), dim3(512), smem_bytes, stream, q, g);
+  VLNCE_CHECK_LAUNCH("conv_r3");
+  return 0;
+}
+
+template <int NCC, int N2B, int MATH>
+int launch_r3_skip(const IgemmParams& p, const RegenParams& g, hipStream_t stream) {
+  return p.in2_scale != nullptr ? launch_r3<NCC, N2B, 2, MATH>(p, g, stream)
+                                : launch_r3<NCC, N2B, 1, MATH>(p, g, stream);
+}
+
+template <int MATH>
+int r3_launch_(const IgemmParams& p, const RegenParams& g, hipStream_t stream) {
+  if (g.K1 == 64 && p.N == 64) return launch_r3_skip<2, 2, MATH>(p, g, stream);
+  if (g.K1 == 64 && p.N == 128) return launch_r3_skip<2, 4, MATH>(p, g, stream);
+  if (g.K1 == 128 && p.N == 128) return launch_r3_skip<4, 4, MATH>(p, g, stream);
+  if (g.K1 == 128 && p.N == 256) return launch_r3_skip<4, 8, MATH>(p, g, stream);
+  vlnce_set_error("conv_r3: no instance for %d -> %d -> %d channels", g.K1, p.K, p.N);
+  return 1;
+}
+
+}
+
+int r3_launch(const IgemmParams& p, const RegenParams& g, hipStream_t stream) {
+  note_conv_kernel(VLNCE_CONV_KERNEL(VLNCE_CONV_PATH_P3, p.math, VLNCE_CONV_KERNEL_R3, g.K1, p.N / 32,
+                                     p.in2_scale != nullptr ? 2 : 1));
+  return p.math == MATH_F16X3 ? r3_launch_<MATH_F16X3>(p, g, stream)
+                              : r3_launch_<MATH_BF16X6>(p, g, stream);
+}
+
+}
diff --git a/vln-ce_amd/csrc/conv_s3.hip b/vln-ce_amd/csrc/conv_s3.hip
--- a/vln-ce_amd/csrc/conv_s3.hip
+++ b/vln-ce_amd/csrc/conv_s3.hip
@@ -5,7 +5,7 @@
 namespace vlnce_detail {
 namespace {
 
-template <int NCC, int MATH>
+template <int NCC, int MATH, bool STORE>
 __global__ __launch_bounds__(512) void conv_s3_kernel(IgemmParams p) {
 #if defined(__HIP_DEVICE_COMPILE__)
   typedef Planes<MATH> PL;
@@ -34,7 +34,7 @@
       const_cast<char*>(reinterpret_cast<const char*>(p.Bfrag)), 0, (int)((long)p.N * p.K * 6),
       0x00020000);
   const __amdgpu_buffer_rsrc_t rsrc_c = __builtin_amdgcn_make_buffer_rsrc(
-      reinterpret_cast<char*>(p.C), 0, (int)p.c_bytes, 0x00020000);
+      reinterpret_cast<char*>(p.C), 0, STORE ? (int)p.c_bytes : 0, 0x00020000);
   const float relu_floor = p.in_relu ? 0.f : -__builtin_huge_valf();
   const bool relu_out = p.act == VLNCE_ACT_RELU;
 
@@ -80,9 +80,11 @@
   };
 #pragma unroll
   for (int k = 0; k < RING; ++k) load_raw(raw[k], k);
-  f32x16 acc[2][MT];
-#pragma unroll
-  for (int b = 0; b < 2; ++b)
+  constexpr int NACC = STORE ? 2 : 1;
+  constexpr int B1 = NACC - 1;
+  f32x16 acc[NACC][MT];
+#pragma unroll
+  for (int b = 0; b < NACC; ++b)
 #pragma unroll
     for (int i = 0; i < MT; ++i)
 #pragma unroll
@@ -139,7 +141,8 @@
     load_raw(r, round + RING);
     asm volatile("s_waitcnt lgkmcnt(0)" ::: "memory");
     __builtin_amdgcn_s_barrier();
-    if (has_prev) stats(prv, m0_prev);
+    if constexpr (STORE)
+      if (has_prev) stats(prv, m0_prev);
 #pragma unroll
     for (int c = 0; c < NCC; ++c)
 #pragma unroll
@@ -156,51 +159,62 @@
 #pragma unroll
           for (int i = 0; i < MT; ++i)
             cur[i] = plane_mfma<MATH>(f[i][PL::PA[q]], bres[c * 2 + s2][PL::PB[q]], cur[i]);
-        stores(prv, has_prev ? m0_prev : p.M, (c * 2 + s2) * SPS, SPS);
-        if constexpr (MATH == MATH_F16X3) {
-#pragma unroll
-          for (int g = 0; g < 2; ++g) {
-            if constexpr (SPS == 8) {
-              __builtin_amdgcn_sched_group_barrier(0x008, 1, 0);
-              __builtin_amdgcn_sched_group_barrier(0x040, 1, 0);
-              __builtin_amdgcn_sched_group_barrier(0x008, 1, 0);
-              __builtin_amdgcn_sched_group_barrier(0x040, 2, 0);
-              __builtin_amdgcn_sched_group_barrier(0x008, 1, 0);
-              __builtin_amdgcn_sched_group_barrier(0x040, 1, 0);
-            } else {
-              __builtin_amdgcn_sched_group_barrier(0x008, 3, 0);
-              __builtin_amdgcn_sched_group_barrier(0x040, 2, 0);
+        if constexpr (STORE) {
+          stores(prv, has_prev ? m0_prev : p.M, (c * 2 + s2) * SPS, SPS);
+          if constexpr (MATH == MATH_F16X3) {
+#pragma unroll
+            for (int g = 0; g < 2; ++g) {
+              if constexpr (SPS == 8) {
+                __builtin_amdgcn_sched_group_barrier(0x008, 1, 0);
+                __builtin_amdgcn_sched_group_barrier(0x040, 1, 0);
+                __builtin_amdgcn_sched_group_barrier(0x008, 1, 0);
+                __builtin_amdgcn_sched_group_barrier(0x040, 2, 0);
+                __builtin_amdgcn_sched_group_barrier(0x008, 1, 0);
+                __builtin_amdgcn_sched_group_barrier(0x040, 1, 0);
+              } else {
+                __builtin_amdgcn_sched_group_barrier(0x008, 3, 0);
+                __builtin_amdgcn_sched_group_barrier(0x040, 2, 0);
+              }
             }
-          }
-        } else {
-#pragma unroll
-          for (int g = 0; g < 4; ++g) {
-            if constexpr (SPS == 8) {
-              __builtin_amdgcn_sched_group_barrier(0x008, 2, 0);
-              __builtin_amdgcn_sched_group_barrier(0x040, 1, 0);
-              __builtin_amdgcn_sched_group_barrier(0x008, 1, 0);
-              __builtin_amdgcn_sched_group_barrier(0x040, 1, 0);
-            } else {
-              __builtin_amdgcn_sched_group_barrier(0x008, 3, 0);
-              __builtin_amdgcn_sched_group_barrier(0x040, 1, 0);
+          } else {
+#pragma unroll
+            for (int g = 0; g < 4; ++g) {
+              if constexpr (SPS == 8) {
+                __builtin_amdgcn_sched_group_barrier(0x008, 2, 0);
+                __builtin_amdgcn_sched_group_barrier(0x040, 1, 0);
+                __builtin_amdgcn_sched_group_barrier(0x008, 1, 0);
+                __builtin_amdgcn_sched_group_barrier(0x040, 1, 0);
+              } else {
+                __builtin_amdgcn_sched_group_barrier(0x008, 3, 0);
+                __builtin_amdgcn_sched_group_barrier(0x040, 1, 0);
+              }
             }
           }
         }
       }
+    if constexpr (!STORE) {
+      stats(cur, m0);
+#pragma unroll
+      for (int i = 0; i < MT; ++i)
+#pragma unroll
+        for (int r2 = 0; r2 < 16; ++r2) cur[i][r2] = 0.f;
+    }
   };
   if (my_tiles <= 0) return;
-  tile(0, raw[0], acc[0], acc[1]);
-  if (1 < my_tiles) tile(1, raw[RING - 1], acc[1], acc[0]);
+  tile(0, raw[0], acc[0], acc[B1]);
+  if (1 < my_tiles) tile(1, raw[RING - 1], acc[B1], acc[0]);
   for (int round = 2; round < my_tiles; round += 2) {
-    tile(round, raw[0], acc[0], acc[1]);
-    if (round + 1 < my_tiles) tile(round + 1, raw[RING - 1], acc[1], acc[0]);
-  }
-  {
+    tile(round, raw[0], acc[0], acc[B1]);
+    if (round + 1 < my_tiles) tile(round + 1, raw[RING - 1], acc[B1], acc[0]);
+  }
+  if constexpr (!STORE) {
+    if (p.bn.acc != nullptr) wave_bn_flush(wbn, p.bn.acc, p.N, half, l31);
+  } else {
     const int m0 = (wg + (my_tiles - 1) * nwg) * BM;
     if ((my_tiles - 1) & 1) {
-      stats(acc[1], m0);
+      stats(acc[B1], m0);
       if (p.bn.acc != nullptr) wave_bn_flush(wbn, p.bn.acc, p.N, half, l31);
-      stores(acc[1], m0, 0, 32);
+      stores(acc[B1], m0, 0, 32);
     } else {
       stats(acc[0], m0);
       if (p.bn.acc != nullptr) wave_bn_flush(wbn, p.bn.acc, p.N, half, l31);
@@ -210,10 +224,10 @@
 #endif
 }
 
-template <int NCC, int MATH>
+template <int NCC, int MATH, bool STORE>
 int launch_s3(const IgemmParams& p, hipStream_t stream) {
   constexpr int smem_bytes = 2 * NCC * 64 * Planes<MATH>::ROW + 3 * NCC * 32 * 4;
-  auto kern = conv_s3_kernel<NCC, MATH>;
+  auto kern = conv_s3_kernel<NCC, MATH, STORE>;
   static bool attr_set = false;
   if (!attr_set) {
     hipError_t e = hipFuncSetAttribute(reinterpret_cast<const void*>(kern),
@@ -231,18 +245,37 @@
   const int cus = x3_cus();
   long grid = (long)q.tiles_m * q.tiles_n;
   if (grid > cus) grid = cus - cus % q.tiles_n;
+  if (const int cap = vlnce_opt(VLNCE_OPT_S3_WGS); cap > 0 && grid > cap)
+    grid = cap >= q.tiles_n ? cap - cap % q.tiles_n : q.tiles_n;
   hipLaunchKernelGGL(kern, dim3((unsigned)grid), dim3(512), smem_bytes, stream, q);
   VLNCE_CHECK_LAUNCH("conv_s3");
   return 0;
 }
 
+template <bool STORE>
+int s3_launch_(const IgemmParams& p, hipStream_t stream) {
+  if (p.math == MATH_F16X3)
+    return p.Cin == 64 ? launch_s3<2, MATH_F16X3, STORE>(p, stream)
+                       : launch_s3<4, MATH_F16X3, STORE>(p, stream);
+  return p.Cin == 64 ? launch_s3<2, MATH_BF16X6, STORE>(p, stream)
+                     : launch_s3<4, MATH_BF16X6, STORE>(p, stream);
+}
+
 }
 
 int s3_launch(const IgemmParams& p, hipStream_t stream) {
-  note_conv_kernel(VLNCE_CONV_KERNEL(VLNCE_CONV_PATH_P3, p.math, VLNCE_CONV_KERNEL_S3, p.Cin == 64 ? 64 : 128, 0, 0));
-  if (p.math == MATH_F16X3)
-    return p.Cin == 64 ? launch_s3<2, MATH_F16X3>(p, stream) : launch_s3<4, MATH_F16X3>(p, stream);
-  return p.Cin == 64 ? launch_s3<2, MATH_BF16X6>(p, stream) : launch_s3<4, MATH_BF16X6>(p, stream);
-}
-
-}
+  if (p.stats_only ? p.C != nullptr : p.C == nullptr) {
+    vlnce_set_error("conv_s3: %s", p.stats_only ? "a statistics-only launch takes no output pointer"
+                                                : "null output");
+    return 1;
+  }
+  if (p.stats_only && p.bn.acc == nullptr && p.stat_partial == nullptr) {
+    vlnce_set_error("conv_s3: a statistics-only launch needs bn or stat_partial");
+    return 1;
+  }
+  note_conv_kernel(VLNCE_CONV_KERNEL(VLNCE_CONV_PATH_P3, p.math, VLNCE_CONV_KERNEL_S3,
+                                     p.Cin == 64 ? 64 : 128, p.stats_only ? 1 : 0, 0));
+  return p.stats_only ? s3_launch_<false>(p, stream) : s3_launch_<true>(p, stream);
+}
+
+}
diff --git a/vln-ce_amd/csrc/igemm.hip b/vln-ce_amd/csrc/igemm.hip
--- a/vln-ce_amd/csrc/igemm.hip
+++ b/vln-ce_amd/csrc/igemm.hip
@@ -1120,6 +1120,7 @@
   p.stat_partial = e ? e->stat_partial : nullptr;
   p.bn = vlnce_bn_sums{};
   if (e && e->bn) p.bn = *e->bn;
+  p.stats_only = e ? e->stats_only : 0;
 }
 
 bool aligned16(const void* q) { return (reinterpret_cast<uintptr_t>(q) & 15) == 0; }
@@ -1324,7 +1325,13 @@
 extern "C" int vlnce_conv2d_fwd(const float* x, const float* w, float* y, const vlnce_conv_desc* d,
                                 const vlnce_prologue* pro, const vlnce_epilogue* epi,
                                 vlnce_stream_t stream) {
-  VLNCE_CHECK_ARG(x && w && y && d, "conv2d_fwd: null argument");
+  const vlnce_regen* const regen = pro ? pro->regen : nullptr;
+  VLNCE_CHECK_ARG((regen ? x == nullptr : x != nullptr) && w && d,
+                  "conv2d_fwd: %s", regen ? "a launch that regenerates its input takes no x" : "null argument");
+  const bool stats_only = epi && epi->stats_only;
+  VLNCE_CHECK_ARG(stats_only ? y == nullptr : y != nullptr,
+                  "conv2d_fwd: %s", stats_only ? "a statistics-only launch takes no output (y must be NULL)"
+                                               : "null argument");
   VLNCE_CHECK_ARG(d->N > 0 && d->H > 0 && d->W > 0 && d->Cin > 0 && d->Cout > 0,
                   "conv2d_fwd: bad shape");
   const VlnceOptScope opt_scope(pro ? pro->options : nullptr);
@@ -1404,10 +1411,54 @@
   p.splitk = 1;
   p.a_bytes = (((long)d->N * d->H * d->W - 1) * p.lda + d->Cin) * 4;
   p.b_bytes = (long)d->Cout * p.K * 4;
-  p.c_bytes = ((M - 1) * p.ldc + d->Cout) * 4;
+  p.c_bytes = stats_only ? 0 : ((M - 1) * p.ldc + d->Cout) * 4;
   p.stat_rows = stat_rows_for(d);
   hipStream_t s = reinterpret_cast<hipStream_t>(stream);
   g_last_path = VLNCE_CONV_PATH_F32;
+  if (regen != nullptr) {
+    VLNCE_CHECK_ARG(!stats_only && conv_math() && p.Bfrag && regen->w_frag && regen->x && d->KH == 1 &&
+                        d->KW == 1 && d->stride == 1 && d->pad == 0 && d->Cin == 4 * regen->Cin &&
+                        (regen->Cin == 64 || regen->Cin == 128) && regen->ldx >= regen->Cin &&
+                        regen->ldx % 4 == 0 && p.lda % 4 == 0 && p.A2 && p.side_out && p.in_scale &&
+                        !p.scale && !p.shift && !p.residual && !p.act && !p.accumulate &&
+                        (p.stat_partial == nullptr || p.stat_rows == 32) &&
+                        ((p.in2_scale == nullptr) == (p.in2_shift == nullptr)) &&
+                        (!p.in2_center || p.in2_scale) &&
+                        ((regen->in_scale == nullptr) == (regen->in_shift == nullptr)) &&
+                        (!regen->in_center || regen->in_scale),
+                    "conv2d_fwd: regen needs a stride-1 1x1 launch with Cin = 4 x regen.Cin (64 / 128), "
+                    "w_frag of both convolutions, x2, side_out, in_scale / in_shift and a raw output");
+    RegenParams g{};
+    g.x = regen->x;
+    g.w_frag = regen->w_frag;
+    g.scale = regen->in_scale;
+    g.shift = regen->in_shift;
+    g.center = regen->in_center;
+    g.relu = regen->in_relu;
+    g.K1 = regen->Cin;
+    g.ldx = regen->ldx;
+    g.x_bytes = ((M - 1) * regen->ldx + regen->Cin) * 4;
+    VLNCE_CHECK_ARG(aligned16(g.x) && aligned16(p.A2) && aligned16(p.side_out) && aligned16(y) &&
+                        (!g.scale || (aligned16(g.scale) && aligned16(g.shift))) &&
+                        (!g.center || aligned16(g.center)) && g.x_bytes < 0x7fffffffL &&
+                        p.a_bytes < 0x7fffffffL && p.c_bytes < 0x7fffffffL,
+                    "conv2d_fwd: regen needs 16-byte aligned operands below 2 GiB");
+    g_last_path = VLNCE_CONV_PATH_P3;
+    return r3_launch(p, g, s);
+  }
+  if (stats_only) {
+    VLNCE_CHECK_ARG(p.bn.acc != nullptr || p.stat_partial != nullptr,
+                    "conv2d_fwd: a statistics-only launch needs bn or stat_partial");
+    VLNCE_CHECK_ARG(conv_math() && p.Bfrag && v4 && buf_ok(p) && d->KH == 1 && d->KW == 1 &&
+                        d->stride == 1 && d->pad == 0 && (d->Cin == 64 || d->Cin == 128) &&
+                        d->Cout % 256 == 0 && d->Cout / 256 <= 8 && !p.A2 && !p.side_out &&
+                        !p.scale && !p.shift && !p.residual && !p.act && !p.accumulate &&
+                        (p.stat_partial == nullptr || p.stat_rows == 32),
+                    "conv2d_fwd: no statistics-only kernel for this problem (stride-1 1x1, Cin 64 / 128, "
+                    "Cout %% 256 == 0, w_frag, a plain prologue, no epilogue arithmetic)");
+    g_last_path = VLNCE_CONV_PATH_P3;
+    return s3_launch(p, s);
+  }
   if (p.A2 != nullptr || p.side_out != nullptr) {
     VLNCE_CHECK_ARG(p.A2 && p.in_scale && d->KH == 1 && d->KW == 1 && d->stride == 1 &&
                         d->pad == 0 && v4 && buf_ok(p) && aligned16(p.A2) &&
diff --git a/vln-ce_amd/csrc/igemm_shared.h b/vln-ce_amd/csrc/igemm_shared.h
--- a/vln-ce_amd/csrc/igemm_shared.h
+++ b/vln-ce_amd/csrc/igemm_shared.h
@@ -52,7 +52,19 @@
   int tiles_m, tiles_n;
   int splitk;
   int stat_rows;
+  int stats_only;
   long a_bytes, b_bytes, c_bytes;
+};
+
+struct RegenParams {
+  const float* x;
+  const void* w_frag;
+  const float* scale;
+  const float* shift;
+  const float* center;
+  int relu;
+  int K1, ldx;
+  long x_bytes;
 };
 
 __device__ __forceinline__ f32x4 ldg4(const float* p) { return *reinterpret_cast<const f32x4*>(p); }
@@ -397,6 +409,7 @@
 constexpr int U3_MAX_CIN = 4096;
 int u3_launch(const IgemmParams& p, int bm, int dual_kind, int waves, hipStream_t stream);
 int s3_launch(const IgemmParams& p, hipStream_t stream);
+int r3_launch(const IgemmParams& p, const RegenParams& g, hipStream_t stream);
 int m3_try_launch(const IgemmParams& p, hipStream_t stream);
 int wgrad_x6_try_launch(const float* x, const float* dy, float* dw, const vlnce_conv_desc* d,
                         const float* dy_up, const float* dy_down, int accumulate,
diff --git a/vln-ce_amd/encoders/resnet_encoders.py b/vln-ce_amd/encoders/resnet_encoders.py
--- a/vln-ce_amd/encoders/resnet_encoders.py
+++ b/vln-ce_amd/encoders/resnet_encoders.py
@@ -1,6 +1,6 @@
 import os
 import warnings
-from collections import OrderedDict
+from collections import OrderedDict, namedtuple
 
 import numpy as np
 import torch
@@ -230,6 +230,9 @@
         return [(self.conv1, self.bn1), (self.conv2, self.bn2), (self.conv3, self.bn3)]
 
 
+_Regen = namedtuple("_Regen", "x w pend", defaults=(None,))
+
+
 class _GlobalAvgPool(nn.Module):
     out_hw = (1, 1)
 
@@ -274,10 +277,10 @@
                                act=ops.ACT_RELU if relu else ops.ACT_NONE, **pro)
 
     def _conv_stats(self, x, conv, bn, touched, prologue=None, in_relu=False, s2d=False,
-                    dual=None):
-        pro = {}
+                    dual=None, **extra):
+        pro = dict(extra)
         if prologue is not None:
-            pro = dict(in_scale=prologue[0], in_shift=prologue[1], in_relu=in_relu,
+            pro.update(in_scale=prologue[0], in_shift=prologue[1], in_relu=in_relu,
                        in_center=prologue[2] if len(prologue) > 2 else None)
         if dual is not None:
             x2, p2, side = dual
@@ -288,6 +291,7 @@
                           (self._cache.conv(conv), conv.stride[0], conv.padding[0]))
         assert bn.momentum is not None
         if os.environ.get("VLNCE_BN_FUSED", "1") == "0":
+            assert not extra
             y, stats = ops.conv2d_nhwc(x, w, stride, pad, want_stats=True, **pro)
             pend = ops.bn_finalize(stats, y.numel() // y.size(-1), bn.weight, bn.bias, bn.eps,
                                    bn.momentum, bn.running_mean, bn.running_var)
@@ -307,24 +311,60 @@
                                    act=ops.ACT_RELU, out=raw)
 
     @staticmethod
-    def _takes_pending(blk, pending):
+    def _takes_pending(blk, numel):
         conv = blk.stages()[0][0]
         return (conv.kernel_size == (1, 1) and conv.stride == (1, 1) and conv.padding == (0, 0)
-                and conv.in_channels % 32 == 0 and pending[0].numel() * 4 < (1 << 31)
+                and conv.in_channels % 32 == 0 and numel * 4 < (1 << 31)
                 and os.environ.get("VLNCE_FUSE_BLOCK_END", "1") != "0")
 
-    def _block_train(self, x, pending, blk, touched):
+    _R3_MEASURED_FASTER = frozenset({(64, 64), (64, 128), (128, 128), (128, 256)})
+
+    def _regen_next(self, blk, nxt, raw2):
+        mode = ops.regen_mode()
+        if mode <= 0 or nxt is None or not isinstance(blk, Bottleneck):
+            return None
+        conv3, c1 = blk.conv3, nxt.stages()[0][0]
+        k1, n2 = conv3.in_channels, c1.out_channels
+        if (conv3.kernel_size != (1, 1) or conv3.stride != (1, 1) or conv3.padding != (0, 0)
+                or k1 not in (64, 128) or conv3.out_channels != 4 * k1
+                or c1.in_channels != 4 * k1 or n2 not in ((64, 128) if k1 == 64 else (128, 256))
+                or os.environ.get("VLNCE_BN_FUSED", "1") == "0"
+                or not self._takes_pending(nxt, raw2.numel() * 4)):
+            return None
+        rows = raw2.numel() // k1
+        cus = torch.cuda.get_device_properties(raw2.device).multi_processor_count // 8 * 8
+        if mode == 1 and ((k1, n2) not in self._R3_MEASURED_FASTER or rows < 64 * 4 * cus):
+            return None
+        w3, w1 = self._cache.conv(conv3), self._cache.conv(c1)
+        if ops.plane_format(None, w3) != ops.plane_format(None, w1):
+            return None
+        return _Regen(raw2, w3)
+
+    def _block_train(self, x, pending, blk, touched, nxt=None):
         st = blk.stages()
-        if pending is not None and self._takes_pending(blk, pending):
+        if pending is not None and self._takes_pending(blk, pending[2].numel()):
             raw3, pend3, skip, pskip = pending
-            x = torch.empty_like(raw3)
-            raw, pend = self._conv_stats(raw3, st[0][0], st[0][1], touched, prologue=pend3,
-                                         in_relu=True, dual=(skip, pskip, x))
+            x = torch.empty_like(skip)
+            if isinstance(raw3, _Regen):
+                raw, pend = self._conv_stats(
+                    raw3.x, st[0][0], st[0][1], touched, prologue=pend3, in_relu=True, dual=(skip, pskip, x),
+                    regen=dict(w=raw3.w, in_scale=raw3.pend[0], in_shift=raw3.pend[1], in_center=raw3.pend[2],
+                               in_relu=True))
+            else:
+                raw, pend = self._conv_stats(raw3, st[0][0], st[0][1], touched, prologue=pend3,
+                                             in_relu=True, dual=(skip, pskip, x))
         else:
             if pending is not None:
                 x = self._materialise(pending)
             raw, pend = self._conv_stats(x, st[0][0], st[0][1], touched)
-        for conv, bn in st[1:]:
+        for conv, bn in st[1:-1]:
+            raw, pend = self._conv_stats(raw, conv, bn, touched, prologue=pend, in_relu=True)
+        conv, bn = st[-1]
+        rg = self._regen_next(blk, nxt, raw)
+        if rg is not None:
+            _, pend3 = self._conv_stats(raw, conv, bn, touched, prologue=pend, in_relu=True, stats_only=True)
+            raw, pend = rg._replace(pend=pend), pend3
+        else:
             raw, pend = self._conv_stats(raw, conv, bn, touched, prologue=pend, in_relu=True)
         if blk.downsample is not None:
             rd, pd = self._conv_stats(x, blk.downsample[0], blk.downsample[1], touched)
@@ -356,7 +396,8 @@
             raise NotImplementedError("mixed train/eval BatchNorm modes inside one trunk")
         key = (signature, modes[0], tuple(p._version for p in self._plist(checked=False)),
                id(self.input_scale[0]), len(self._modules),
-               0 if modes[0] else self._bn_gen, ops.plane_format())
+               0 if modes[0] else self._bn_gen, ops.plane_format(),
+               ops.regen_mode() if modes[0] else 0)
         return key, modes[0]
 
     def graph_ready(self, x):
@@ -400,13 +441,13 @@
                     x = self._conv_bn_eval(x, kids[0], kids[1], True, prologue=pro, s2d=s2d)
                     x = ops.maxpool3x3s2(x)
             pending = None
-            for stage in kids[4:8]:
-                for blk in stage:
-                    if train:
-                        pending = self._block_train(x, pending, blk, touched)
-                        x = None
-                    else:
-                        x = self._block_eval(x, blk)
+            blocks = [blk for stage in kids[4:8] for blk in stage]
+            for blk, nxt in zip(blocks, blocks[1:] + [None]):
+                if train:
+                    pending = self._block_train(x, pending, blk, touched, nxt)
+                    x = None
+                else:
+                    x = self._block_eval(x, blk)
             if pending is not None:
                 x = self._materialise(pending)
             for pool in kids[8:]:
diff --git a/vln-ce_amd/ops.py b/vln-ce_amd/ops.py
--- a/vln-ce_amd/ops.py
+++ b/vln-ce_amd/ops.py
@@ -106,12 +106,30 @@
                 Ho=Ho, Wo=Wo, ldx=ldx or Cin, ldy=Cout)
 
 
+def _regen_launch(x, regen, x2, fmt):
+    w3 = regen["w"]
+    assert x2 is not None and x.is_contiguous() and w3.is_contiguous()
+    assert x.shape[:3] == x2.shape[:3] and w3.shape[0] == x2.shape[3] and w3.shape[3] == x.shape[3]
+    frag = pack_weights(w3, fmt)
+    if frag is None:
+        raise RuntimeError("regen: the regenerated convolution has no fragment image")
+    return None, dict(x=x, w_frag=frag, in_scale=regen.get("in_scale"), in_shift=regen.get("in_shift"),
+                      in_center=regen.get("in_center"), in_relu=int(regen.get("in_relu", 0)))
+
+
+def regen_mode():
+    lib = L()
+    if not hasattr(lib, "effective_option") or not lib.effective_option("conv_math"):
+        return 0
+    return lib.effective_option("r3")
+
+
 def conv2d_nhwc(x, w_ohwi, stride, pad, *, in_scale=None, in_shift=None, in_center=None,
                 in_relu=False, scale=None, shift=None, residual=None, act=ACT_NONE,
                 want_stats=False, x2=None, in2_scale=None, in2_shift=None, in2_center=None,
-                side_out=None, w_format=None):
+                side_out=None, w_format=None, regen=None):
     assert x.is_contiguous() and w_ohwi.is_contiguous()
-    g = conv_geometry(x, w_ohwi, stride, pad)
+    g = conv_geometry(x if regen is None else x2, w_ohwi, stride, pad)
     y = torch.empty((g["N"], g["Ho"], g["Wo"], g["Cout"]), device=x.device, dtype=torch.float32)
     stats = None
     partial = None
@@ -123,15 +141,18 @@
         assert residual.is_contiguous() and residual.shape == y.shape
     dual = {}
     if x2 is not None:
-        assert x2.is_contiguous() and x2.shape == x.shape
-        assert side_out is None or (side_out.is_contiguous() and side_out.shape == x.shape)
+        assert x2.is_contiguous() and (regen is not None or x2.shape == x.shape)
+        assert side_out is None or (side_out.is_contiguous() and side_out.shape == x2.shape)
         dual = dict(x2=x2, in2_scale=in2_scale, in2_shift=in2_shift, in2_center=in2_center,
                     side_out=side_out)
     fmt = plane_format(w_format, w_ohwi)
+    more = {}
+    if regen is not None:
+        x, more["regen"] = _regen_launch(x, regen, x2, fmt)
     L().conv2d_fwd(x, w_ohwi, y, g, in_scale=in_scale, in_shift=in_shift, in_center=in_center,
                    in_relu=int(in_relu), **dual, scale=scale, shift=shift, residual=residual, ldr=g["Cout"], act=act,
                    stat_partial=partial, w_split=split_weights(w_ohwi, fmt),
-                   w_frag=pack_weights(w_ohwi, fmt), w_format=fmt)
+                   w_frag=pack_weights(w_ohwi, fmt), w_format=fmt, **more)
     return (y, stats) if want_stats else y
 
 
@@ -147,19 +168,25 @@
     return acc
 
 
-def conv2d_bn_sums(x, w_ohwi, stride, pad, acc, **pro):
+def conv2d_bn_sums(x, w_ohwi, stride, pad, acc, stats_only=False, **pro):
     assert x.is_contiguous() and w_ohwi.is_contiguous()
-    g = conv_geometry(x, w_ohwi, stride, pad)
-    y = torch.empty((g["N"], g["Ho"], g["Wo"], g["Cout"]), device=x.device, dtype=torch.float32)
+    regen = pro.pop("regen", None)
+    g = conv_geometry(x if regen is None else pro.get("x2"), w_ohwi, stride, pad)
+    y = torch.empty((g["N"], g["Ho"], g["Wo"], 0 if stats_only else g["Cout"]), device=x.device,
+                    dtype=torch.float32)
     lib = L()
     ws = torch.empty(max(lib.conv2d_bn_workspace_bytes(g), 16), device=x.device, dtype=torch.uint8)
     if pro.get("x2") is not None:
-        assert pro["x2"].is_contiguous() and pro["x2"].shape == x.shape
+        assert pro["x2"].is_contiguous() and (regen is not None or pro["x2"].shape == x.shape)
     if "in_relu" in pro:
         pro = dict(pro, in_relu=int(pro["in_relu"]))
     fmt = plane_format(None, w_ohwi)
-    lib.conv2d_fwd(x, w_ohwi, y, g, **pro, ldr=g["Cout"], w_split=split_weights(w_ohwi, fmt),
-                   w_frag=pack_weights(w_ohwi, fmt), bn=(acc, ws), w_format=fmt)
+    more = dict(stats_only=True) if stats_only else {}
+    if regen is not None:
+        x, more["regen"] = _regen_launch(x, regen, pro.get("x2"), fmt)
+    lib.conv2d_fwd(x, w_ohwi, None if stats_only else y, g, **pro, ldr=g["Cout"],
+                   w_split=split_weights(w_ohwi, fmt), w_frag=pack_weights(w_ohwi, fmt), bn=(acc, ws),
+                   w_format=fmt, **more)
     return y
 
 
@@ -177,7 +204,7 @@
     acc = _bn_state(bn)
     try:
         y = conv2d_bn_sums(x, w_ohwi, stride, pad, acc, **pro)
-        return y, bn_finalize_sums(acc, y.numel() // y.size(-1), bn)
+        return y, bn_finalize_sums(acc, y.size(0) * y.size(1) * y.size(2), bn)
     except Exception:
         if not (acc.is_cuda and torch.cuda.is_current_stream_capturing()):
             acc.zero_()
```
